# rogerbarton/optix-renderer

Hardware: AMD Instinct MI355X
Metric: Msamples/sec (whole node) + traversal HBM GB/s, cbox 1024x1024 256spp (higher is better)
Workload: dtype f32; 1 GPU; Cornell box (diffuse-only) 1024x1024, 16400 spp, path_mis; config=c2, width=1024, height=1024, spp=16400, mode=wavefront, traversal=ordered, pools=2, gpu_max_hw_queues=8, parallelism=single GPU

## Files before the change

### include/nori_hip.h

```cpp
#ifndef NORI_HIP_H
#define NORI_HIP_H

#include <stddef.h>
#include <stdint.h>

#ifdef __cplusplus
extern "C" {
#endif

#define NH_OK 0
#define NH_ERR_INVALID 1
#define NH_ERR_IO 2
#define NH_ERR_DEVICE 3
#define NH_ERR_UNSUPPORTED 4
#define NH_ERR_STATE 5


enum { NH_SHAPE_MESH = 0, NH_SHAPE_SPHERE = 1 };
enum { NH_BSDF_DIFFUSE = 0, NH_BSDF_MIRROR = 1, NH_BSDF_DIELECTRIC = 2, NH_BSDF_MICROFACET = 3, NH_BSDF_DISNEY = 4 };
enum { NH_EMITTER_AREA = 0, NH_EMITTER_POINT = 1, NH_EMITTER_ENVMAP = 2, NH_EMITTER_SPOT = 3,
       NH_EMITTER_DIRECTIONAL = 4 };
enum { NH_INTEGRATOR_PATH_MIS = 0, NH_INTEGRATOR_PATH_MATS = 1, NH_INTEGRATOR_DIRECT_EMS = 2,
       NH_INTEGRATOR_DIRECT_MATS = 3, NH_INTEGRATOR_DIRECT_MIS = 4, NH_INTEGRATOR_DIRECT = 5,
       NH_INTEGRATOR_NORMALS = 6,
// ... 103 lines not shown
typedef struct nh_envmap {
    int32_t width, height;
    const float *rgba;
    float radiance[3];
    float scale_u, scale_v;
    float offset_u, offset_v;
    int32_t spherical;
    int32_t constant;
    const float *cdf;
    float normalization;
    float rotation[9];
} nh_envmap;

enum { NH_DENOISER_NONE = 0, NH_DENOISER_SIMPLE = 1 };
typedef struct nh_denoiser {
    int32_t type;
    float sigma_d;
    float sigma_vr;
    int32_t range;
    int32_t amount;
} nh_denoiser;

enum { NH_SAMPLER_INDEPENDENT = 0, NH_SAMPLER_ADAPTIVE = 1 };

typedef struct nh_scene_desc {
    nh_camera camera;
    nh_filter filter;
    int32_t integrator;
    int32_t sample_count;
    uint32_t n_shapes;
    const nh_shape *shapes;
    uint32_t n_bsdfs;
    const nh_bsdf *bsdfs;
    uint32_t n_emitters;
    const nh_emitter *emitters;
    const float *emitter_cdf;
    int32_t envmap;
    uint32_t n_vertices;
    const float *V;
    const float *N;
    const float *UV;
    const float *T;
    const float *BT;
    uint32_t n_faces;
    const uint32_t *F;
    uint32_t n_area_cdf;
    const float *area_cdf;
    nh_envmap env;
    nh_denoiser denoiser;
    uint32_t n_textures;
    const nh_texture *textures;
    uint64_t n_texels;
    const float *texels;
    float normals_direction[3];
    const nh_emitter_ext *emitter_ext;
    uint32_t n_media;
    const nh_medium *media;
    const uint32_t *shape_medium;
    uint32_t ambient_medium;
    int32_t sampler;
    int32_t adaptive_initial_uniform;
} nh_scene_desc;


typedef struct nh_bvh_node {
    uint32_t word0;
    uint32_t word1;
    float bbox_min[3];
    float bbox_max[3];
} nh_bvh_node;

typedef struct nh_bvh_desc {
    uint32_t n_nodes;
    const nh_bvh_node *nodes;
    uint32_t n_indices;
    const uint32_t *indices;
    uint32_t n_shapes;
    const uint32_t *shape_offset;
    float bbox_min[3], bbox_max[3];
    uint32_t max_depth;
} nh_bvh_desc;


typedef struct nh_ray_soa {
    const float *ox, *oy, *oz;
    const float *dx, *dy, *dz;
    const float *mint, *maxt;
} nh_ray_soa;

typedef struct nh_hit_soa {
    uint8_t *hit;
    float *t, *u, *v;
    uint32_t *prim;
    uint32_t *shape;
} nh_hit_soa;


enum { NH_MODE_MEGAKERNEL = 0, NH_MODE_WAVEFRONT = 1 };
enum { NH_TRAVERSAL_REFERENCE = 0, NH_TRAVERSAL_ORDERED = 1, NH_TRAVERSAL_WIDE = 2 };

typedef struct nh_render_req {
    int32_t sample_begin;
    int32_t sample_end;
    uint64_t seed;
    int32_t n_blocks;
    const int32_t *blocks;
    int32_t mode;
    int32_t traversal;
    int32_t clear;
    int32_t collect_stats;
} nh_render_req;

#define NH_SMALL_TABLES_BYTES 4096

typedef struct nh_render_stats {
    double kernel_ms_path;
    double kernel_ms_splat;
    double kernel_ms_extend;
    double kernel_ms_shadow;
    double kernel_ms_shade;
    uint64_t launches_path, launches_splat, launches_extend, launches_shadow, launches_shade;
    uint64_t samples;
    uint64_t ray_queries;
    uint64_t nodes_visited;
    uint64_t boxes_tested;
    uint64_t prims_tested;
    uint64_t invalid_samples;
    uint64_t shadow_queries, shadow_nodes_visited, shadow_boxes_tested, shadow_prims_tested;
    uint64_t shade_state_bytes, extend_queue_bytes, shadow_queue_bytes, paths_shaded;
    double kernel_ms_tail;
    uint64_t launches_tail;
    uint64_t node_bytes;
    uint64_t tail_queries, tail_nodes_visited, tail_boxes_tested, tail_prims_tested;
    uint64_t tail_shadow_queries, tail_shadow_nodes_visited, tail_shadow_boxes_tested, tail_shadow_prims_tested;
    uint64_t lds_scene;
    uint64_t fused_bounce;
    uint64_t comm_inits;
    double kernel_ms_denoise;
    uint64_t launches_denoise;
    uint64_t tails_async;
    uint64_t pools_active;
    uint64_t trace_fused;
    uint64_t tail_cycles_body, tail_cycles_shadow, tail_cycles_closest, tail_cycles_head;
    uint64_t tail_bounces, tail_max_bounces;
    uint64_t tail_coop_cycles_body, tail_coop_cycles_shadow, tail_coop_cycles_closest, tail_coop_cycles_head;
    uint64_t tail_coop_bounces;
    uint64_t bounce_cycles_load, bounce_cycles_body, bounce_cycles_shadow, bounce_cycles_closest, bounce_cycles_head;
    uint64_t bounce_cycles_store, bounce_bounces;
    uint64_t bounce_traits;
    uint64_t primary_masks;
    uint64_t pair_kinds;
    uint64_t flat_trace;
    uint64_t shadow_masks;
} nh_render_stats;

typedef struct nh_scene nh_scene;
typedef struct nh_bvh nh_bvh;
typedef struct nh_ctx nh_ctx;

int nh_scene_load_xml(const char *path, nh_scene **out);
int nh_scene_load_xml_index(const char *path, int32_t index, nh_scene **out);
int nh_scene_get_desc(const nh_scene *scene, nh_scene_desc *out);
int nh_scene_set_resolution(nh_scene *scene, int32_t width, int32_t height);
int nh_scene_set_sample_count(nh_scene *scene, int32_t spp);
int nh_scene_set_sampler(nh_scene *scene, int32_t type, int32_t initial_uniform);
int nh_scene_set_bsdf(nh_scene *scene, uint32_t shape, const nh_bsdf *bsdf);
uint32_t nh_scene_add_texture(nh_scene *scene, const nh_texture *tex, const float *texels);
int nh_scene_set_normal_map(nh_scene *scene, uint32_t shape, uint32_t texture);
int nh_scene_set_lens_draw_order(nh_scene *scene, int32_t order);
int nh_texture_decode(const uint8_t *rgba8, uint64_t n, int32_t srgb, float *out);
int nh_scene_set_integrator(nh_scene *scene, int32_t integrator);
typedef struct nh_photon_params {
    int32_t photon_count;
    float photon_radius;
} nh_photon_params;
int nh_scene_get_photon_params(const nh_scene *scene, nh_photon_params *out);
int nh_scene_set_photon_params(nh_scene *scene, const nh_photon_params *params);
typedef struct nh_av_params {
    float length;
} nh_av_params;
int nh_scene_get_av_params(const nh_scene *scene, nh_av_params *out);
int nh_scene_set_av_params(nh_scene *scene, const nh_av_params *params);
int nh_photon_tables(float *cos_theta, float *sin_theta, float *cos_phi, float *sin_phi, float *exp_table);
void nh_scene_free(nh_scene *scene);
const char *nh_host_last_error(void);
int nh_debug_transform(const char *request, float *out, int32_t cap);

int nh_bvh_build(const nh_scene_desc *scene, int32_t n_threads, nh_bvh **out);
int nh_bvh_get_desc(const nh_bvh *bvh, nh_bvh_desc *out);
void nh_bvh_free(nh_bvh *bvh);

int nh_primary_masks(const nh_camera *camera, const float *records, int32_t n_records, const int32_t *blocks,
                     int32_t n_blocks, uint64_t *masks, int32_t *built);
int32_t nh_primary_mask_pad(int32_t width, int32_t height);

int nh_shadow_emitter_faces(const nh_scene_desc *scene, float *faces, int32_t cap_faces, int32_t *n_faces);
int nh_shadow_masks(const nh_camera *camera, const float *records, int32_t n_records, const float *emit_faces,
                    int32_t n_emit_faces, const int32_t *blocks, int32_t n_blocks, uint64_t *emitter_mask,
                    uint64_t *masks, int32_t *built);

int nh_pair_layout(const float *records, int32_t n_records, const int32_t *leaves, int32_t n_leaves, int32_t by_kind,
                   int32_t *slots, int32_t *leaf_pairs);

int nh_flat_image(const float *records, int32_t n_records, const int32_t *leaves, int32_t n_leaves, const float *boxes,
                  int32_t allowed, float *image, int32_t image_cap_f4, int32_t *n_f4, int32_t *box_equal);

int nh_framebuffer_to_rgb(const float *rgbw, int32_t width, int32_t height, int32_t border, float *rgb);
int nh_write_pfm(const char *path, const float *rgb, int32_t width, int32_t height);
int nh_image_load_png(const char *path, uint8_t *rgba, size_t cap, int32_t *width, int32_t *height);
int nh_write_exr(const char *path, const float *rgb, int32_t width, int32_t height);
int nh_rgb_to_ldr(const float *rgb, int32_t width, int32_t height, uint8_t *rgb8);
int nh_write_png(const char *path, const float *rgb, int32_t width, int32_t height);

int nh_get_device_count(int *n);
int nh_create(int device, nh_ctx **out);
void nh_destroy(nh_ctx *ctx);
int nh_upload_scene(nh_ctx *ctx, const nh_scene_desc *scene);
int nh_upload_bvh(nh_ctx *ctx, const nh_bvh_desc *bvh);
int nh_trace_rays(nh_ctx *ctx, const nh_ray_soa *rays, int32_t n, int32_t any_hit, int32_t traversal, nh_hit_soa *out);
#define NH_ADAPTIVE_MAX_SAMPLES 133948
#define NH_ADAPTIVE_STAGING_BYTES ((size_t)4 << 30)
int nh_render(nh_ctx *ctx, const nh_render_req *req);
typedef struct nh_adaptive_stats {
    uint64_t total_samples;
    uint64_t passes;
    uint64_t max_passes;
    uint64_t n_blocks;
} nh_adaptive_stats;
int nh_get_adaptive_stats(nh_ctx *ctx, nh_adaptive_stats *out);
int nh_get_adaptive_variance(nh_ctx *ctx, float *out, size_t n_floats);
int nh_synchronize(nh_ctx *ctx);
int nh_get_framebuffer(nh_ctx *ctx, float *rgbw, size_t n_floats);
int nh_framebuffer_device_ptr(nh_ctx *ctx, void **dptr, size_t *n_floats);
int nh_get_stats(nh_ctx *ctx, nh_render_stats *out);
int nh_reset_stats(nh_ctx *ctx);
int nh_reduce_framebuffers(nh_ctx **ctxs, int32_t n, int32_t root);
int nh_denoise(nh_ctx *ctx, const nh_denoiser *params);
int nh_denoise_image(nh_ctx *ctx, float *rgbw, int32_t width, int32_t height, int32_t border,
                     const nh_denoiser *params);
enum { NH_BSDF_QUERY_EVAL = 0, NH_BSDF_QUERY_SAMPLE = 1 };
int nh_bsdf_query(nh_ctx *ctx, const nh_bsdf *bsdf, const float *albedo, int32_t mode, int32_t n, const float *wi,
                  const float *wo, const float *sample, float *wo_out, float *value, float *pdf, int32_t *measure);
enum { NH_EMITTER_QUERY_SAMPLE = 0, NH_EMITTER_QUERY_EVAL = 1, NH_EMITTER_QUERY_PDF = 2,
       NH_EMITTER_QUERY_SAMPLE_PHOTON = 3 };
#define NH_EMITTER_QUERY_SAMPLE_STRIDE 16
#define NH_EMITTER_QUERY_PHOTON_STRIDE 12
#define NH_EMITTER_QUERY_IN_STRIDE 9
int nh_emitter_query(nh_ctx *ctx, uint32_t emitter, int32_t mode, int32_t n, const float *ref, const float *sample,
                     float *out);
enum { NH_MEDIUM_QUERY_FREE_PATH = 0, NH_MEDIUM_QUERY_TRANSMITTANCE = 1, NH_MEDIUM_QUERY_PHASE_SAMPLE = 2,
       NH_MEDIUM_QUERY_PHASE_PDF = 3 };
int nh_medium_query(nh_ctx *ctx, uint32_t medium, int32_t mode, int32_t n, const float *in, float *out);


enum { NH_TEST_TTEST = 0, NH_TEST_CHI2TEST = 1 };
typedef struct nh_test_desc {
    int32_t type;
    float significance_level;
    int32_t sample_count;
    uint32_t n_angles;
    const float *angles;
    uint32_t n_references;
    const float *references;
    uint32_t n_scenes;
    uint32_t n_bsdfs;
    const nh_bsdf *bsdfs;
} nh_test_desc;
typedef struct nh_test nh_test;
int nh_test_load_xml(const char *path, nh_test **out);
int nh_test_get_desc(const nh_test *test, nh_test_desc *out);
void nh_test_free(nh_test *test);

int nh_students_t_test(double mean, double variance, double reference, int32_t n, double alpha, int32_t num_tests,
                       int32_t *accepted, double *p_value);

#define NH_RADIANCE_QUERY_MAX (1 << 24)
int nh_radiance_query(nh_ctx *ctx, uint64_t seed, int32_t n, const int32_t *pixel, const int32_t *sample,
                      const float *pixel_sample, float *rgb, float *jitter);
int nh_ttest_scene(nh_ctx *ctx, uint64_t seed, int64_t first, int32_t n, double *mean, double *variance,
                   float *luminance);
int nh_ttest_bsdf(nh_ctx *ctx, const nh_bsdf *bsdf, const float *albedo, float angle_deg, uint64_t first_draw,
                  int32_t n, double *mean, double *variance, float *luminance);
typedef struct nh_test_result {
    double mean, variance, reference, p_value;
    int32_t accepted;
    int32_t sample_count;
    float angle;
    int32_t pad;
} nh_test_result;
int nh_test_run(int device, const char *path, uint64_t seed, nh_test_result *results, int32_t cap,
                int32_t *n_results);


#define NH_PHOTON_STREAM ((uint64_t)1 << 32)
#define NH_PHOTON_DEFAULT_BATCH (1 << 18)
int nh_photon_map_build(nh_ctx *ctx, const nh_photon_params *params, uint64_t seed, int32_t batch_paths);
typedef struct nh_photon_stats {
    int32_t stored;
    int32_t emitted;
    float radius;
    float cell_size;
    uint64_t occupied_cells;
} nh_photon_stats;
int nh_get_photon_stats(nh_ctx *ctx, nh_photon_stats *out);
int nh_get_photons(nh_ctx *ctx, int32_t first, int32_t n, float *position, float *direction, float *power,
                   uint8_t *bytes, int32_t *path, int32_t *bounce);
enum { NH_PHOTON_QUERY_CODEC = 0, NH_PHOTON_QUERY_GATHER = 1 };
int nh_photon_query(nh_ctx *ctx, int32_t mode, int32_t n, const float *in, uint8_t *bytes, int32_t *count, float *out);


int nh_set_av_params(nh_ctx *ctx, const nh_av_params *params);

const char *nh_last_error(const nh_ctx *ctx);

#ifdef __cplusplus
}
#endif
#endif
```

### optix-renderer_amd/csrc/nh_ctx.h

```cpp
#pragma once
#include <hip/hip_runtime.h>
#include <rccl/rccl.h>

#include <algorithm>
#include <cstdint>
#include <deque>
#include <memory>
#include <string>
#include <vector>

#include "nh_internal.h"
#include "nori_hip.h"

constexpr int kRing = 4;
constexpr int kPools = 4;
constexpr int kTails = 3;
constexpr int kTailCap = 65536;
#ifndef NH_DEFAULT_POOLS
#define NH_DEFAULT_POOLS 2
#endif

struct WfJob {
    uint64_t seq;
    int s0, rounds;
    uint64_t seed;
    bool ordered, stats;
    bool staged;
    bool jit;
};

struct WfPool {
    hipStream_t stream = nullptr;
    WfState wf{};
    std::vector<void *> bufs;
    size_t cap = 0;
    float *rec = nullptr;
    size_t rec_cap = 0;
    float2 *jit = nullptr;
    size_t jit_cap = 0;
    float4 *staging = nullptr;
    size_t staging_cap = 0;
    uint32_t *spill = nullptr;
    int spill_words = 0;
    unsigned *h_counts = nullptr;
    hipEvent_t copy_ev[kRing] = {};
    std::vector<hipEvent_t> events;
    hipEvent_t ev_begin = nullptr, ev_path = nullptr, ev_splat0 = nullptr, ev_splat = nullptr;
    hipEvent_t ev_handoff = nullptr;
    enum State { IDLE, ENQUEUE, COUNTS, SPLAT, FINISH } state = IDLE;
    WfJob job{};
    WfLaunch L{};
    bool persistent = false, wide = false, trace2 = false, tail = false, draining = false;
    bool fused = false, sorted = false;
    bool rr = false;
    bool trait = false;
    bool shade_sorted = false;
    int64_t tail_at = 0, drain_at = 0;
    int it = 0;
    std::vector<uint64_t> in_e, in_s;
};

struct CommSet {
    std::vector<uint64_t> ids;
    std::vector<int> devices;
    std::vector<ncclComm_t> comms;
    ~CommSet() {
        int cur = 0;
        const bool have = hipGetDevice(&cur) == hipSuccess;
        for (size_t i = 0; i < comms.size(); ++i) {
            (void)hipSetDevice(devices[i]);
            (void)ncclCommDestroy(comms[i]);
        }
        if (have) (void)hipSetDevice(cur);
    }
};

struct DeviceGuard {
    int dev = 0;
    bool ok = false;
    DeviceGuard() { ok = hipGetDevice(&dev) == hipSuccess; }
    ~DeviceGuard() {
        if (ok) (void)hipSetDevice(dev);
    }
};

struct PixelList {
    int *pixel_list = nullptr, *pixel_map = nullptr;
    int *block_ids = nullptr, *block_slot = nullptr;
    int *color_slots = nullptr;
    int n_blocks = 0, n_color0 = 0, n_list = 0;
    std::vector<int32_t> list_key;
    bool have_list = false;
    void release() {
        for (int *p : {pixel_list, pixel_map, block_ids, block_slot, color_slots}) (void)hipFree(p);
        *this = PixelList{};
    }
};

struct AdaptiveState {
    int n_blocks = 0, nbx = 0, nby = 0;
    int next_sample = -1;
    int4 *blocks = nullptr;
    int *block_rank = nullptr, *active_list = nullptr, *next = nullptr;
    AdBlock *state = nullptr;
    unsigned *counts = nullptr, *h_count = nullptr;
    int2 *pos = nullptr;
    float4 *rad = nullptr, *staging = nullptr;
    float2 *jit = nullptr;
    size_t slot_cap = 0;
    unsigned long long *stats = nullptr;
    std::vector<int4> h_blocks;
};

struct PhotonState {
    bool built = false;
    std::vector<void *> bufs;
    const float *tables = nullptr;
    std::vector<float> h_tables;
    float *pos = nullptr;
    uint2 *bytes = nullptr;
    uint32_t *path = nullptr;
    int *bounce = nullptr;
    nh_photon_stats stats{};
};

struct nh_ctx {
    uint64_t id = 0;
    std::shared_ptr<CommSet> comms;
    int device = 0;
    hipStream_t stream = nullptr;
    std::string err;
    std::vector<nh_shape> shapes;
    std::vector<float> V;
    std::vector<uint32_t> F;
    int width = 0, height = 0, border = 0, n_emitters = 0, integrator = 0;
    nh_filter filter{};
    nhd::DScene S{};
    nhd::DScene *d_scene = nullptr;
    nhd::Traversal tv{};
    std::vector<void *> scene_bufs, bvh_bufs;
    bool has_scene = false, has_bvh = false;
    int depth = 0;
    int depth_wide = 0;
    int wide_w = 4;
    int n_node_f4 = 0, n_leaves = 0, n_prim_f4 = 0;
    std::vector<uint32_t> bvh_indices, shape_offset;
    std::vector<int> shape_bsdf_type;
    std::vector<int> shape_bsdf_real;
    int n_bsdf_types = 0;
    bool disney = false;
    bool specular = false;
    bool textured = false;
    bool normal_mapped = false;
    bool diffuse_area = false;
    bool bsdfless = false, has_media = false;
    int sampler = 0, adaptive_initial_uniform = 0;
    AdaptiveState ad;
    PhotonState photon;
    bool av_set = false;
    AvLaunch av{};
    std::vector<void *> av_bufs;
    size_t av_cap = 0;
    int2 *av_spill = nullptr;
    int av_spill_depth = 0;
    std::vector<nhd::DShape> h_shapes;
    std::vector<nhd::DBsdf> h_bsdfs;
    std::vector<nhd::DEmitter> h_emitters;
    std::vector<float> h_area_cdf;
    int n_emit_faces = 0;
    float4 *small_image = nullptr;
    int small_tab[5] = {0, 0, 0, 0, 0};
    bool pair_kinds = false;
    float4 *small_image_ref = nullptr;
    const float4 *flat_image = nullptr;
    nh_camera camera{};
    std::vector<float> h_prims;
    unsigned long long *pmask = nullptr;
    bool pmask_known = false;
    std::vector<float> h_emit_tris;
    unsigned long long *smask = nullptr;
    float *fb = nullptr;
    size_t fb_floats = 0;
    float *rec = nullptr;
    size_t rec_cap = 0;
    int *block_rank = nullptr;
    int nbx = 0, nby = 0;
    PixelList px;
    float4 *staging = nullptr;
    size_t staging_cap = 0;
    unsigned long long *counters = nullptr;
    nh_render_stats stats{};
    WfPool pools[kPools + kTails];
    std::deque<WfJob> jobs;
    uint64_t job_seq = 0, splat_seq = 0;
    hipEvent_t fb_ev = nullptr;
    bool fb_ev_set = false;
    uint64_t stats_comm_inits = 0;
};

inline void drop_primary_masks(nh_ctx *c) {
    (void)hipFree(c->pmask);
    (void)hipFree(c->smask);
    c->pmask = nullptr;
    c->smask = nullptr;
    c->pmask_known = false;
}

#define NH_LAUNCH(c, fn) ((c)->disney ? nh_disney::nh::fn : nh::fn)

void pool_free(WfPool &p);
int pipeline_drain(nh_ctx *c);
int check_device(nh_ctx *c, const char *where);
int render_adaptive(nh_ctx *c, const nh_render_req *q);
void adaptive_release(nh_ctx *c);
void photon_release(nh_ctx *c, bool tables = false);
nhd::DDisney disney_record(const nh_bsdf &b);
void disney_set_record(nhd::DBsdf &o, const nhd::DDisney *rec);
int disney_upload(nh_ctx *c, std::vector<void *> &owner, const std::vector<nhd::DDisney> &recs,
                  const std::vector<float> &albedo, nhd::DDisney **out);

int query_bsdf_record(nh_ctx *c, std::vector<void *> &owner, const nh_bsdf *b, const float *albedo, nhd::DBsdf &o,
                      float alb[3]);

inline bool fail(nh_ctx *c, const std::string &m) {
    if (c) c->err = m;
    return false;
}

#define HIP_TRY(ctx, expr)                                                                               \
    do {                                                                                                 \
        hipError_t e_ = (expr);                                                                          \
        if (e_ != hipSuccess) {                                                                          \
            (ctx)->err = std::string(#expr) + ": " + hipGetErrorString(e_);                              \
            return NH_ERR_DEVICE;                                                                        \
        }                                                                                                \
    } while (0)

template <typename T>
int upload(nh_ctx *c, std::vector<void *> &owner, const T *src, size_t n, const T **dst) {
    void *p = nullptr;
    size_t bytes = (std::max<size_t>(n * sizeof(T), 16) + 15) / 16 * 16;
    HIP_TRY(c, hipMalloc(&p, bytes));
    owner.push_back(p);
    if (n) HIP_TRY(c, hipMemcpyAsync(p, src, n * sizeof(T), hipMemcpyHostToDevice, c->stream));
    *dst = reinterpret_cast<const T *>(p);
    return NH_OK;
}

inline void free_all(std::vector<void *> &v) {
    for (void *p : v) (void)hipFree(p);
    v.clear();
}
```

### optix-renderer_amd/csrc/nh_layout.h

```cpp
#pragma once

namespace nhd {

constexpr int kLensLo = 256, kLensHi = 65536;

constexpr int kPrimSphere = 1, kPrimLeafEnd = 2, kPrimMatShift = 2;
constexpr int kPrimIsolated = 16;

constexpr int kWideF4 = 8;
constexpr int kWideEmpty = (int)0x80000000;

constexpr int kPairF4 = 6;
constexpr int kFlatHeaderF4 = 6, kFlatMaxPairs = 16;
constexpr int kFlatLeftEq = 1, kFlatRightEq = 2;

constexpr int kMaxStack = 128;

}
```

### optix-renderer_amd/csrc/nh_pipeline.hip

```cpp
#include <cmath>
#include <cstdlib>
#include <cstring>
#include <thread>
#include <type_traits>

#include "../host/gpu_layout.h"
#include "nh_ctx.h"


constexpr size_t kWfBytesPerPath = 2 * (16 * 6 + 8 + 1) + 36;

static int pool_alloc(nh_ctx *c, WfPool &p, size_t n, size_t rec_n, size_t staging_f4, bool jit = false) {
    if (!p.stream) {
        if (!p.h_counts && hipHostMalloc(reinterpret_cast<void **>(&p.h_counts),
                                         (kRing * 2 * kCountGroup + kCountSlot) * sizeof(unsigned)) != hipSuccess) {
            p.h_counts = nullptr;
            return fail(c, "hipHostMalloc failed"), NH_ERR_DEVICE;
        }
        for (hipEvent_t &e : p.copy_ev)
            if (!e) HIP_TRY(c, hipEventCreateWithFlags(&e, hipEventDisableTiming));
        for (hipEvent_t *e : {&p.ev_begin, &p.ev_path, &p.ev_splat0, &p.ev_splat})
            if (!*e) HIP_TRY(c, hipEventCreate(e));
        if (!p.ev_handoff) HIP_TRY(c, hipEventCreateWithFlags(&p.ev_handoff, hipEventDisableTiming));
        HIP_TRY(c, hipStreamCreateWithFlags(&p.stream, hipStreamNonBlocking));
// ... 49 lines not shown

void pool_free(WfPool &p) {
    free_all(p.bufs);
    (void)hipFree(p.rec);
    (void)hipFree(p.jit);
    (void)hipFree(p.staging);
    (void)hipFree(p.spill);
    if (p.h_counts) (void)hipHostFree(p.h_counts);
    for (hipEvent_t e : p.events) (void)hipEventDestroy(e);
    for (hipEvent_t e : p.copy_ev)
        if (e) (void)hipEventDestroy(e);
    for (hipEvent_t e : {p.ev_begin, p.ev_path, p.ev_splat0, p.ev_splat, p.ev_handoff})
        if (e) (void)hipEventDestroy(e);
    if (p.stream) (void)hipStreamDestroy(p.stream);
    p = WfPool{};
}

static SplatLaunch make_splat(const nh_ctx *c, const float *rec, uint64_t seed, int s0, float4 *staging, int rounds,
                              bool staged) {
    SplatLaunch P{};
    P.staged = staged ? 1 : 0;
    P.fb = c->fb;
    P.width = c->width;
    P.height = c->height;
    P.border = c->border;
    P.reach = (int)std::floor(c->filter.radius + 0.5f);
    P.nbx = c->nbx;
    P.n_rounds = rounds;
    P.n_list = c->px.n_list;
    P.pixel_map = c->px.pixel_map;
    P.block_rank = c->block_rank;
    P.rec = rec;
    P.seed = seed;
    P.s0 = s0;
    P.radius = c->filter.radius;
    P.lookup = c->filter.lookup_factor;
    std::memcpy(P.table, c->filter.table, sizeof(P.table));
    P.blocks = c->px.block_ids;
    P.block_slot = c->px.block_slot;
    P.n_blocks = c->px.n_blocks;
    P.color_slots = c->px.color_slots;
    P.n_color0 = c->px.n_color0;
    P.staging = staging;
    return P;
}

static bool splat_staged(const nh_ctx *c) {
    return nh::splat_uses_staging(c->border, (int)std::floor(c->filter.radius + 0.5f));
}
static size_t block_px(const nh_ctx *c, bool staged) {
    if (!staged) return 0;
    return (size_t)(32 + 2 * c->border) * (size_t)stage_pitch(32 + 2 * c->border);
}

static int active_pools(const nh_ctx *c) {
    const char *np = std::getenv("NH_POOLS");
    const int def = c->specular ? NH_DEFAULT_POOLS + 1 : NH_DEFAULT_POOLS;
    return std::max(1, std::min(kPools, np ? std::atoi(np) : def));
}

static bool tail_async_enabled() {
    const char *e = std::getenv("NH_TAIL_ASYNC");
    return e && e[0] == '1';
}

static int pool_start(nh_ctx *c, WfPool &p, const WfJob &job) {
    WfJob j = job;
    j.staged = splat_staged(c);
    const char *jv = std::getenv("NH_SPLAT_JITTER");
    j.jit = jv && std::strcmp(jv, "stored") == 0;
    const int n_paths = j.rounds * c->px.n_list;
    const size_t staging_f4 = (size_t)j.rounds * c->px.n_blocks * block_px(c, j.staged);
    int rc = pool_alloc(c, p, (size_t)n_paths, (size_t)n_paths, staging_f4, j.jit);
    if (rc) return rc;
    for (int i = 0; i < active_pools(c); ++i) {
        WfPool &o = c->pools[i];
        if (&o == &p || o.state != WfPool::IDLE) continue;
        if ((rc = pool_alloc(c, o, (size_t)n_paths, (size_t)n_paths, staging_f4, j.jit))) return rc;
    }
    if (active_pools(c) > 1 && tail_async_enabled())
        for (int i = kPools; i < kPools + kTails; ++i) {
            WfPool &o = c->pools[i];
            if (o.state != WfPool::IDLE) continue;
            if ((rc = pool_alloc(c, o, (size_t)kTailCap, (size_t)n_paths, staging_f4, j.jit))) return rc;
        }
    p.job = j;
    WfLaunch &L = p.L;
    L = WfLaunch{};
    L.st = p.wf;
    L.n_paths = n_paths;
    L.n_list = c->px.n_list;
    L.s0 = j.s0;
    L.seed = j.seed;
    L.pixel_list = c->px.pixel_list;
    L.rec = p.rec;
    L.jit = j.jit ? p.jit : nullptr;
    L.counters = c->counters;
    const size_t scene_bytes = 16 * (size_t)(c->n_node_f4 + c->n_prim_f4) + 8 * (size_t)c->n_leaves;
    bool small = scene_bytes <= kSmallSceneBytes;
    if (const char *e = std::getenv("NH_LDS_SCENE")) small = small && e[0] != '0';
    if (small) {
        L.small_nodes = c->n_node_f4;
        L.small_leaves = c->n_leaves;
        L.small_prims = c->n_prim_f4;
        L.small_frames = c->n_prim_f4 / 3 <= kSmallFramesMaxPrims;
        if (const char *e = std::getenv("NH_LDS_FRAMES")) L.small_frames = L.small_frames && e[0] != '0';
        L.small_image = j.stats && c->small_image_ref ? c->small_image_ref : c->small_image;
        for (int i = 0; i < 5; ++i) L.small_tab[i] = c->small_tab[i];
    }
    const int per_chunk = 256;
    const int max_chunks = (n_paths + per_chunk - 1) / per_chunk;
    L.seg_cap = (max_chunks + kQueueShards - 1) / kQueueShards * per_chunk;
    p.persistent = c->depth > 20;
    if (const char *e = std::getenv("NH_PERSISTENT")) p.persistent = e[0] == '1';
    p.wide = p.persistent && j.ordered && c->tv.wnodes != nullptr;
    if (const char *e = std::getenv("NH_WIDE")) p.wide = p.wide && e[0] != '0';
    if (p.wide && !j.ordered) return fail(c, "wavefront pool: the wide traversal needs an ordered job"), NH_ERR_STATE;
    p.trace2 = p.wide && scene_bytes <= (size_t)256 << 20;
    if (const char *e = std::getenv("NH_TRACE2")) p.trace2 = p.wide && e[0] != '0';
    c->stats.trace_fused = p.trace2 ? 1 : 0;
    const int spill_words = p.wide ? 2 * c->depth_wide : (c->depth + 1) / 2 * 2;
    if (p.persistent && p.spill_words < spill_words) {
        HIP_TRY(c, hipStreamSynchronize(p.stream));
        (void)hipFree(p.spill);
        p.spill = nullptr;
        p.spill_words = 0;
        HIP_TRY(c, hipMalloc(&p.spill, (size_t)kPersistentBlocks * 128 * spill_words * sizeof(uint32_t)));
        p.spill_words = spill_words;
    }
    p.fused = small && !p.persistent && c->depth <= 16;
    if (const char *e = std::getenv("NH_FUSED")) p.fused = p.fused && e[0] != '0';
    p.sorted = p.fused && c->n_bsdf_types > 1;
    p.rr = p.fused;
    if (const char *e = std::getenv("NH_RR_AHEAD")) p.rr = p.fused && e[0] != '0';
    p.shade_sorted = false;
    if (const char *e = std::getenv("NH_SORT_SHADE")) p.shade_sorted = !p.fused && e[0] == '1';
    if (const char *e = std::getenv("NH_SORT")) p.sorted = p.fused && e[0] == '1';
    p.trait = p.rr && c->diffuse_area && c->small_tab[0] > 0 && j.ordered && !p.sorted;
    if (const char *e = std::getenv("NH_BOUNCE_TRAITS")) p.trait = p.trait && e[0] != '0';
    c->stats.bounce_traits = p.rr ? (p.trait ? 2 : 1) : 0;
    const char *pm = std::getenv("NH_PRIMARY_MASKS");
    const bool masks = p.rr && c->pmask && !j.stats && !(pm && pm[0] == '0');
    L.pmask = masks ? c->pmask : nullptr;
    L.pmask_nbx = c->nbx;
    c->stats.primary_masks = masks ? 1 : 0;
    const char *sm = std::getenv("NH_SHADOW_MASKS");
    const bool shadow = p.rr && c->smask && !j.stats && !(sm && (sm[0] == '0' || sm[0] == '1'));
    L.smask = shadow ? c->smask : nullptr;
    c->stats.shadow_masks = shadow ? 2 : 0;
    c->stats.pair_kinds = p.fused && c->pair_kinds && !j.stats ? 1 : 0;
    const bool flat = p.rr && c->flat_image && c->pair_kinds && !j.stats && !c->disney;
    L.flat = flat ? c->flat_image : nullptr;
    c->stats.flat_trace = flat ? 1 : 0;
    c->stats.fused_bounce = p.fused ? 1 : 0;
    c->stats.node_bytes = p.wide ? 16 * nhd::kWideF4 * (c->wide_w / 4) : 64;
    c->stats.lds_scene = small && !p.persistent && c->depth <= 16 ? 1 : 0;
    L.trav_spill = p.spill;
    L.spill_depth = p.spill_words;
    p.tail_at = p.fused ? std::min<int64_t>(std::max<int64_t>(n_paths / 1024, 8192), 16384)
                        : std::min<int64_t>(std::max<int64_t>(n_paths / 64, 8192), 262144);
    if (const char *e = std::getenv("NH_TAIL")) p.tail_at = std::atoll(e);
    p.drain_at = std::max<int64_t>(n_paths / 8, p.tail_at);
    HIP_TRY(c, hipEventRecord(p.ev_begin, p.stream));
    unsigned *h_init = p.h_counts + kRing * 2 * kCountGroup;
    std::memset(h_init, 0, kCountSlot * sizeof(unsigned));
    h_init[0] = (unsigned)n_paths;
    HIP_TRY(c, hipMemcpyAsync(p.wf.counts, h_init, kCountSlot * sizeof(unsigned), hipMemcpyHostToDevice, p.stream));
    p.in_e.assign(1, (uint64_t)n_paths);
    p.in_s.assign(1, 0);
    p.it = 0;
    p.tail = false;
    p.draining = false;
    p.state = WfPool::ENQUEUE;
    return NH_OK;
}

static void chunk_swap(WfPool &a, WfPool &b) {
    std::swap(a.h_counts, b.h_counts);
    std::swap(a.copy_ev, b.copy_ev);
    std::swap(a.events, b.events);
    std::swap(a.ev_begin, b.ev_begin);
    std::swap(a.ev_path, b.ev_path);
    std::swap(a.ev_splat0, b.ev_splat0);
    std::swap(a.ev_splat, b.ev_splat);
    std::swap(a.job, b.job);
    std::swap(a.L, b.L);
    std::swap(a.persistent, b.persistent);
    std::swap(a.wide, b.wide);
    std::swap(a.trace2, b.trace2);
    std::swap(a.tail, b.tail);
    std::swap(a.draining, b.draining);
    std::swap(a.fused, b.fused);
    std::swap(a.sorted, b.sorted);
    std::swap(a.rr, b.rr);
    std::swap(a.trait, b.trait);
    std::swap(a.shade_sorted, b.shade_sorted);
    std::swap(a.tail_at, b.tail_at);
    std::swap(a.drain_at, b.drain_at);
    std::swap(a.it, b.it);
    std::swap(a.in_e, b.in_e);
    std::swap(a.in_s, b.in_s);
    std::swap(a.rec, b.rec);
    std::swap(a.rec_cap, b.rec_cap);
    std::swap(a.jit, b.jit);
    std::swap(a.jit_cap, b.jit_cap);
    std::swap(a.staging, b.staging);
    std::swap(a.staging_cap, b.staging_cap);
}

static WfPool *free_tail_slot(nh_ctx *c, const WfPool &p, int bound) {
    if (!p.rr || bound > kTailCap || active_pools(c) < 2) return nullptr;
    if (!tail_async_enabled()) return nullptr;
    for (int i = kPools; i < kPools + kTails; ++i)
        if (c->pools[i].state == WfPool::IDLE) return &c->pools[i];
    return nullptr;
}

static int pool_handoff(nh_ctx *c, WfPool &p, WfPool &T, int bound, hipEvent_t *ev) {
    int rc = pool_alloc(c, T, (size_t)kTailCap, 0, 0);
    if (rc) return rc;
    HIP_TRY(c, hipMemsetAsync(T.wf.counts, 0, kCountSlot * sizeof(unsigned), p.stream));
    nh::launch_wf_pack_rr(p.L, T.wf.buf[0], T.wf.counts, bound, p.stream);
    HIP_TRY(c, hipGetLastError());
    HIP_TRY(c, hipEventRecord(p.ev_handoff, p.stream));
    chunk_swap(p, T);
    WfLaunch &L = T.L;
    L.st = T.wf;
    L.in_q = 0;
    L.cnt_in = T.wf.counts;
    HIP_TRY(c, hipStreamWaitEvent(T.stream, p.ev_handoff, 0));
    HIP_TRY(c, hipEventRecord(ev[1], T.stream));
    HIP_TRY(c, hipEventRecord(ev[2], T.stream));
    NH_LAUNCH(c, launch_wf_tail_rr)(c->d_scene, c->tv, L, T.job.ordered, T.job.stats, bound, c->specular,
                          !c->specular && !c->textured, c->normal_mapped, T.trait, T.stream);
    HIP_TRY(c, hipGetLastError());
    HIP_TRY(c, hipEventRecord(ev[3], T.stream));
    T.tail = true;
    T.draining = true;
    T.state = WfPool::SPLAT;
    p.state = WfPool::IDLE;
    c->stats.tails_async++;
    return NH_OK;
}

static bool count_kernel() {
    static const bool on = [] {
        const char *e = std::getenv("NH_COUNT_KERNEL");
        return !(e && e[0] == '0');
    }();
    return on;
}

static int count_service(nh_ctx *c, WfPool &p, unsigned *out, unsigned *in_slot, int it) {
    unsigned *h = p.h_counts + (size_t)(it % kRing) * 2 * kCountGroup;
    if (count_kernel()) {
        nh::launch_wf_counts(out, h, 2 * kCountGroup, in_slot, kCountSlot, p.stream);
        HIP_TRY(c, hipGetLastError());
    } else {
        HIP_TRY(c, hipMemcpyAsync(h, out, 2 * kCountGroup * sizeof(unsigned), hipMemcpyDeviceToHost, p.stream));
    }
    HIP_TRY(c, hipEventRecord(p.copy_ev[it % kRing], p.stream));
    return NH_OK;
}

static int pool_enqueue(nh_ctx *c, WfPool &p) {
    WfLaunch &L = p.L;
    const int it = p.it, in = it & 1;
    unsigned *slot[2] = {p.wf.counts, p.wf.counts + kCountSlot};
    L.in_q = in;
    L.first = it == 0;
    L.cam_rays = it == 0 && p.persistent && c->S.dof ? 1 : 0;
    L.cnt_in = slot[in];
    L.cnt_out = slot[in ^ 1];
    while ((size_t)(it + 1) * 4 > p.events.size()) {
        hipEvent_t e;
        HIP_TRY(c, hipEventCreate(&e));
        p.events.push_back(e);
    }
    hipEvent_t *ev = &p.events[(size_t)it * 4];
    const int bound = (int)p.in_e[it == 0 ? 0 : it - 1];
    const bool ordered = p.job.ordered, stats = p.job.stats;
    if (it == 0 || !count_kernel()) HIP_TRY(c, hipMemsetAsync(slot[in ^ 1], 0, kCountSlot * sizeof(unsigned), p.stream));
    HIP_TRY(c, hipEventRecord(ev[0], p.stream));
    if (p.fused) {
        if (it > 0 && (int64_t)bound <= p.tail_at)
            if (WfPool *T = free_tail_slot(c, p, bound)) return pool_handoff(c, p, *T, bound, ev);
        HIP_TRY(c, hipEventRecord(ev[1], p.stream));
        HIP_TRY(c, hipEventRecord(ev[2], p.stream));
        if (it > 0 && (int64_t)bound <= p.tail_at) {
            if (p.rr)
                NH_LAUNCH(c, launch_wf_tail_rr)(c->d_scene, c->tv, L, ordered, stats, bound, c->specular,
                                                !c->specular && !c->textured, c->normal_mapped, p.trait, p.stream);
            else NH_LAUNCH(c, launch_wf_tail)(c->d_scene, c->tv, L, ordered, stats, false, bound, c->depth, p.stream);
            HIP_TRY(c, hipGetLastError());
            HIP_TRY(c, hipEventRecord(ev[3], p.stream));
            p.tail = true;
            p.draining = true;
            p.state = WfPool::SPLAT;
            return NH_OK;
        }
        if (p.rr) NH_LAUNCH(c, launch_wf_bounce_rr)(c->d_scene, c->tv, L, ordered, stats, p.sorted,
                                                    !c->specular && !c->textured, c->normal_mapped, p.trait, bound,
                                                    p.stream);
        else NH_LAUNCH(c, launch_wf_bounce)(c->d_scene, c->tv, L, ordered, stats, p.sorted, bound, p.stream);
        HIP_TRY(c, hipGetLastError());
        HIP_TRY(c, hipEventRecord(ev[3], p.stream));
// ... 309 lines not shown
    if (blocks.empty())
        for (int i = 0; i < c->nbx * c->nby; ++i) blocks.push_back(i);
    std::vector<uint64_t> m;
    if (!nh::primary_masks(c->camera, reinterpret_cast<const nh::f4 *>(c->h_prims.data()), (int)(c->h_prims.size() / 12),
                           blocks.data(), (int)blocks.size(), m))
        return NH_OK;
    std::vector<unsigned long long> grid((size_t)c->nbx * c->nby, 0ull);
    for (size_t i = 0; i < blocks.size(); ++i) grid[(size_t)blocks[i]] = m[i];
    unsigned long long *d = nullptr;
    HIP_TRY(c, hipMalloc(&d, std::max<size_t>(grid.size(), 1) * sizeof(unsigned long long)));
    const hipError_t e = hipMemcpy(d, grid.data(), grid.size() * sizeof(unsigned long long), hipMemcpyHostToDevice);
    if (e != hipSuccess) {
        (void)hipFree(d);
        HIP_TRY(c, e);
    }
    c->pmask = d;
    const int n_faces = (int)(c->h_emit_tris.size() / 9);
    const nh::f4 *recs = reinterpret_cast<const nh::f4 *>(c->h_prims.data());
    const int n_recs = (int)(c->h_prims.size() / 12);
    if (n_faces == 0 ||
        !nh::shadow_block_masks(c->camera, recs, n_recs, c->h_emit_tris.data(), n_faces, blocks.data(), (int)blocks.size(), m))
        return NH_OK;
    for (size_t i = 0; i < blocks.size(); ++i) grid[(size_t)blocks[i]] = m[i];
    HIP_TRY(c, hipMalloc(&d, std::max<size_t>(grid.size(), 1) * sizeof(unsigned long long)));
    const hipError_t e2 = hipMemcpy(d, grid.data(), grid.size() * sizeof(unsigned long long), hipMemcpyHostToDevice);
    if (e2 != hipSuccess) {
        (void)hipFree(d);
        HIP_TRY(c, e2);
    }
    c->smask = d;
    return NH_OK;
}

constexpr size_t kAvBytesPerPath = 94;

static bool av_wide(const nh_ctx *c, const nh_render_req *q) {
    return q->traversal != NH_TRAVERSAL_REFERENCE && c->depth > 20 && c->tv.wnodes != nullptr;
}
static size_t av_bytes_per_path(const nh_ctx *c, const nh_render_req *q) {
    return kAvBytesPerPath + (av_wide(c, q) ? (size_t)c->depth_wide * sizeof(int2) : 0);
}

static int av_reserve(nh_ctx *c, size_t paths, bool wide) {
    const int spill_depth = wide ? c->depth_wide : 0;
    if (c->av_cap >= paths && c->av_spill_depth >= spill_depth) return NH_OK;
    free_all(c->av_bufs);
    c->av_cap = 0;
    c->av_spill_depth = 0;
    c->av_spill = nullptr;
    AvLaunch &L = c->av;
    L = AvLaunch{};
    const auto get = [&](auto **p, size_t n) -> int {
        void *d = nullptr;
        HIP_TRY(c, hipMalloc(&d, std::max<size_t>(n, 1) * sizeof(**p)));
        c->av_bufs.push_back(d);
        *p = static_cast<std::remove_reference_t<decltype(*p)>>(d);
        return NH_OK;
    };
    int rc = NH_OK;
    for (int i = 0; i < 8 && !rc; ++i)
        if (!(rc = get(&L.ray[i], paths))) rc = get(&L.q_ray[i], paths);
    if (rc || (rc = get(&L.hit.hit, paths)) || (rc = get(&L.hit.t, paths)) || (rc = get(&L.hit.u, paths)) ||
        (rc = get(&L.hit.v, paths)) || (rc = get(&L.hit.k, paths)) || (rc = get(&L.rng, paths)) ||
        (rc = get(&L.q_path, paths)) || (rc = get(&L.q_hit, paths)) || (rc = get(&L.q_count, 1)) ||
        (spill_depth && (rc = get(&c->av_spill, paths * (size_t)spill_depth)))) {
        free_all(c->av_bufs);
        return rc;
    }
    c->av_cap = paths;
    c->av_spill_depth = spill_depth;
    return NH_OK;
}

static int av_chunk(nh_ctx *c, const nh_render_req *q, const PathLaunch &P) {
    AvLaunch L = c->av;
    L.n_paths = P.n_paths;
    L.n_list = P.n_list;
    L.s0 = P.s0;
    L.seed = P.seed;
    L.pixel_list = P.pixel_list;
    L.rec = P.rec;
    const bool wide = av_wide(c, q), ordered = q->traversal != NH_TRAVERSAL_REFERENCE, stats = q->collect_stats != 0;
    const auto batch = [&](float *const r[8], const HitBatch &hb, int n, bool any) {
        const RayBatch rb{r[0], r[1], r[2], r[3], r[4], r[5], r[6], r[7]};
        unsigned long long *ctr = c->counters + (any ? kStatAny : 0);
        if (wide) nh::launch_trace_wide(c->d_scene, c->tv, rb, hb, n, any, true, stats, c->av_spill, c->av_spill_depth, ctr,
                                        c->stream, c->wide_w);
        else nh::launch_trace(c->d_scene, c->tv, rb, hb, n, any, ordered, stats, c->depth, ctr, c->stream);
    };
    HIP_TRY(c, hipMemsetAsync(L.q_count, 0, sizeof(unsigned), c->stream));
    nh::launch_av_primary(c->d_scene, L, c->stream);
    batch(L.ray, L.hit, L.n_paths, false);
    nh::launch_av_shade(c->d_scene, c->tv, L, c->stream);
    HIP_TRY(c, hipGetLastError());
    int n_queue = L.n_paths;
    if (stats) {
        unsigned n = 0;
        HIP_TRY(c, hipMemcpyAsync(&n, L.q_count, sizeof(n), hipMemcpyDeviceToHost, c->stream));
        HIP_TRY(c, hipStreamSynchronize(c->stream));
        n_queue = (int)n;
    }
    HitBatch occl{};
    occl.hit = L.q_hit;
    batch(L.q_ray, occl, n_queue, true);
    nh::launch_av_resolve(L, n_queue, c->stream);
    return NH_OK;
}

extern "C" {

int nh_render(nh_ctx *c, const nh_render_req *q) {
    if (!c || !q) return NH_ERR_INVALID;
    if (!c->has_scene || !c->has_bvh) return fail(c, "nh_render: scene and BVH must be uploaded"), NH_ERR_STATE;
    if (q->sample_end < q->sample_begin || q->sample_begin < 0) return fail(c, "invalid sample range"), NH_ERR_INVALID;
    if (c->S.dof && q->sample_end > nhd::kLensLo * nhd::kLensHi)
        return fail(c, "depth of field: sample rounds beyond 2^24"), NH_ERR_UNSUPPORTED;
    if ((c->integrator == NH_INTEGRATOR_PATH_MIS || c->integrator == NH_INTEGRATOR_DIRECT_MIS) && c->n_emitters == 0)
        return fail(c, "No Emitter in scene!"), NH_ERR_INVALID;
    if (q->mode != NH_MODE_MEGAKERNEL && q->mode != NH_MODE_WAVEFRONT) return fail(c, "unknown render mode"), NH_ERR_INVALID;
    const bool volumetric = c->integrator == NH_INTEGRATOR_PATH_VOL_MATS || c->integrator == NH_INTEGRATOR_PATH_VOL_MIS;
    if (!volumetric && (c->bsdfless || c->has_media))
        return fail(c, "the scene has a participating medium or a shape without a BSDF: only the path_vol_mats and "
                       "path_vol_mis integrators render it"), NH_ERR_UNSUPPORTED;
    if (c->integrator == NH_INTEGRATOR_PATH_VOL_MIS && c->n_emitters == 0)
        return fail(c, "No Emitter in scene!"), NH_ERR_INVALID;
    const bool photon = c->integrator == NH_INTEGRATOR_PHOTONMAPPER;
    if (photon && !c->photon.built)
        return fail(c, "nh_render: the photon mapper needs a photon map (nh_photon_map_build)"), NH_ERR_STATE;
    if (photon && c->sampler == NH_SAMPLER_ADAPTIVE)
        return fail(c, "photonmapper: the adaptive sampler is not supported"), NH_ERR_UNSUPPORTED;
    if (c->integrator == NH_INTEGRATOR_AV && !c->av_set)
        return fail(c, "nh_render: the av integrator needs its length (nh_set_av_params)"), NH_ERR_STATE;
    if (c->integrator == NH_INTEGRATOR_ENVMAPTESTER && c->S.envmap < 0)
        return fail(c, "This integrator requires an env map."), NH_ERR_INVALID;
    const bool av_split = q->mode == NH_MODE_WAVEFRONT && c->integrator == NH_INTEGRATOR_AV;
    const bool wavefront = q->mode == NH_MODE_WAVEFRONT && c->integrator <= NH_INTEGRATOR_PATH_MATS;
    if (q->traversal < NH_TRAVERSAL_REFERENCE || q->traversal > NH_TRAVERSAL_WIDE)
        return fail(c, "unknown traversal"), NH_ERR_INVALID;
    if (c->border > 4) return fail(c, "reconstruction filters wider than border 4 are not supported"), NH_ERR_UNSUPPORTED;
    HIP_TRY(c, hipSetDevice(c->device));
    int rc = NH_OK;
    if (!wavefront || q->collect_stats || q->clear || c->sampler == NH_SAMPLER_ADAPTIVE) rc = pipeline_drain(c);
    if (rc) return rc;
    if (c->sampler == NH_SAMPLER_ADAPTIVE) return render_adaptive(c, q);
    rc = ensure_pixel_list(c, q);
    if (rc) return rc;
    if (wavefront && (rc = ensure_primary_masks(c))) return rc;
    c->stats.node_bytes = 64;
    if (av_split && av_wide(c, q)) c->stats.node_bytes = 16 * nhd::kWideF4 * (c->wide_w / 4);
    c->stats.primary_masks = 0;
    c->stats.shadow_masks = 0;
    c->stats.pair_kinds = 0;
    c->stats.flat_trace = 0;
    c->stats.trace_fused = 0;
    c->stats.lds_scene = 0;
    c->stats.fused_bounce = 0;
    if (q->clear) {
        HIP_TRY(c, hipMemsetAsync(c->fb, 0, c->fb_floats * sizeof(float), c->stream));
        HIP_TRY(c, hipEventRecord(c->fb_ev, c->stream));
        c->fb_ev_set = true;
    }
    const int rounds = q->sample_end - q->sample_begin;
    if (rounds == 0 || c->px.n_list == 0) return NH_OK;
    if (q->collect_stats)
        HIP_TRY(c, hipMemsetAsync(c->counters, 0, kStatShards * kStatStride * sizeof(unsigned long long), c->stream));
    const size_t per_round = (size_t)c->px.n_list;
    const char *jv = std::getenv("NH_SPLAT_JITTER");
    const size_t rec_bytes = kRecFloats * 4 + (wavefront && jv && std::strcmp(jv, "stored") == 0 ? 8 : 0);
    const size_t per_round_bytes = per_round * rec_bytes + (size_t)c->px.n_blocks * block_px(c, splat_staged(c)) * 16 +
                                   (wavefront ? per_round * kWfBytesPerPath : 0) +
                                   (av_split ? per_round * av_bytes_per_path(c, q) : 0);
    size_t budget = wavefront ? (size_t)24 << 30 : (size_t)1 << 30;
    if (const char *e = std::getenv(wavefront ? "NH_WF_BUDGET_MB" : "NH_RECORD_BUDGET_MB"))
        budget = (size_t)std::max(1L, std::atol(e)) << 20;
    if (wavefront) {
        size_t free_b = 0, total_b = 0;
        if (hipMemGetInfo(&free_b, &total_b) == hipSuccess) {
            size_t held = 0;
            for (const WfPool &p : c->pools)
                held += p.cap * kWfBytesPerPath + p.rec_cap * kRecFloats * 4 + p.jit_cap * 8 + p.staging_cap * sizeof(float4);
            const int shares = active_pools(c) + (active_pools(c) > 1 && tail_async_enabled() ? kTails : 0);
            const size_t avail = (size_t)((double)(free_b + held) * 0.85) / (size_t)shares;
            budget = std::min(budget, std::max(avail, per_round_bytes));
        }
    }
    int chunk = (int)std::max<size_t>(1, std::min<size_t>((size_t)rounds, budget / per_round_bytes));
    while ((size_t)chunk * per_round > (size_t)0x7fffffff) chunk = std::max(1, chunk / 2);
    if (wavefront) {
        if (per_round > ((size_t)1 << 26))
            return fail(c, "wavefront mode renders at most 2^26 pixels per context"), NH_ERR_UNSUPPORTED;
        chunk = std::min(chunk, (int)(((size_t)1 << 26) / per_round));
    }

    if (wavefront) {
        HIP_TRY(c, hipStreamSynchronize(c->stream));
        for (int s = q->sample_begin; s < q->sample_end; s += chunk)
            c->jobs.push_back(WfJob{c->job_seq++, s, std::min(chunk, q->sample_end - s), q->seed,
                                    q->traversal != NH_TRAVERSAL_REFERENCE, q->collect_stats != 0});
        rc = q->collect_stats ? pipeline_drain(c) : pipeline_run(c, false);
        if (rc) return rc;
        if (int e = check_device(c, "nh_render")) return e;
    } else {
        if (c->rec_cap < (size_t)chunk * per_round) {
            (void)hipFree(c->rec);
            c->rec = nullptr;
            c->rec_cap = 0;
            const size_t cap = (size_t)chunk * per_round;
            HIP_TRY(c, hipMalloc(&c->rec, cap * kRecFloats * sizeof(float)));
            c->rec_cap = cap;
        }
        if (av_split && (rc = av_reserve(c, (size_t)chunk * per_round, av_wide(c, q)))) return rc;
        const bool staged = splat_staged(c);
        if (c->staging_cap < (size_t)chunk * c->px.n_blocks * block_px(c, staged)) {
            (void)hipFree(c->staging);
            c->staging = nullptr;
            c->staging_cap = 0;
            const size_t cap = (size_t)chunk * c->px.n_blocks * block_px(c, staged);
            HIP_TRY(c, hipMalloc(&c->staging, cap * sizeof(float4)));
            c->staging_cap = cap;
        }
        struct Ev {
            hipEvent_t a, b, d;
        };
        std::vector<Ev> evs;
        for (int s = q->sample_begin; s < q->sample_end; s += chunk) {
            const int k = std::min(chunk, q->sample_end - s);
            PathLaunch L{};
            L.n_paths = k * c->px.n_list;
            L.n_list = c->px.n_list;
            L.s0 = s;
            L.seed = q->seed;
            L.pixel_list = c->px.pixel_list;
            L.rec = c->rec;
            L.counters = c->counters;
            Ev ev;
            HIP_TRY(c, hipEventCreate(&ev.a));
            HIP_TRY(c, hipEventCreate(&ev.b));
            HIP_TRY(c, hipEventCreate(&ev.d));
            HIP_TRY(c, hipEventRecord(ev.a, c->stream));
            if (av_split) {
                if ((rc = av_chunk(c, q, L))) return rc;
            } else if (photon)
                nh_disney::nh::launch_photon_path(c->d_scene, c->tv, L, q->collect_stats != 0, c->depth, c->stream);
            else if (volumetric)
                nh_disney::nh::launch_vol_path(c->d_scene, c->tv, L, c->integrator == NH_INTEGRATOR_PATH_VOL_MIS,
                                               q->collect_stats != 0, c->depth, c->stream);
            else
                NH_LAUNCH(c, launch_path)(c->d_scene, c->tv, L, q->traversal != NH_TRAVERSAL_REFERENCE, q->collect_stats != 0,
                            c->depth, c->integrator == NH_INTEGRATOR_PATH_MIS && !c->normal_mapped, c->stream);
            HIP_TRY(c, hipGetLastError());
            HIP_TRY(c, hipEventRecord(ev.b, c->stream));
            if (q->collect_stats) nh::launch_count_invalid(c->rec, (size_t)L.n_paths, c->counters, c->stream);
            nh::launch_splat(make_splat(c, c->rec, q->seed, s, c->staging, k, staged), c->stream);
            HIP_TRY(c, hipGetLastError());
            HIP_TRY(c, hipEventRecord(ev.d, c->stream));
            evs.push_back(ev);
        }
        HIP_TRY(c, hipStreamSynchronize(c->stream));
        for (auto &ev : evs) {
            float a = 0, b = 0;
            (void)hipEventElapsedTime(&a, ev.a, ev.b);
            (void)hipEventElapsedTime(&b, ev.b, ev.d);
            c->stats.kernel_ms_path += a;
            c->stats.kernel_ms_splat += b;
            c->stats.launches_path++;
            c->stats.launches_splat++;
            (void)hipEventDestroy(ev.a);
            (void)hipEventDestroy(ev.b);
            (void)hipEventDestroy(ev.d);
        }
        c->stats.samples += (uint64_t)rounds * (uint64_t)c->px.n_list;
    }
    if (q->collect_stats) {
        unsigned long long hs[kStatShards * kStatStride], h[kStatStride] = {};
        HIP_TRY(c, hipMemcpy(hs, c->counters, sizeof(hs), hipMemcpyDeviceToHost));
        for (int sh = 0; sh < kStatShards; ++sh)
            for (int j = 0; j < kStatStride; ++j) h[j] += hs[sh * kStatStride + j];
        h[kStatTailClk + 5] = 0;
        for (int sh = 0; sh < kStatShards; ++sh)
            h[kStatTailClk + 5] = std::max(h[kStatTailClk + 5], hs[sh * kStatStride + kStatTailClk + 5]);
        c->stats.tail_cycles_body += h[kStatTailClk];
        c->stats.tail_cycles_shadow += h[kStatTailClk + 1];
        c->stats.tail_cycles_closest += h[kStatTailClk + 2];
        c->stats.tail_cycles_head += h[kStatTailClk + 3];
        c->stats.tail_bounces += h[kStatTailClk + 4];
        c->stats.tail_max_bounces = std::max<uint64_t>(c->stats.tail_max_bounces, h[kStatTailClk + 5]);
        c->stats.tail_coop_cycles_body += h[kStatTailCoopClk];
        c->stats.tail_coop_cycles_shadow += h[kStatTailCoopClk + 1];
        c->stats.tail_coop_cycles_closest += h[kStatTailCoopClk + 2];
        c->stats.tail_coop_cycles_head += h[kStatTailCoopClk + 3];
        c->stats.tail_coop_bounces += h[kStatTailCoopClk + 4];
        c->stats.bounce_cycles_load += h[kStatBounceClk];
        c->stats.bounce_cycles_body += h[kStatBounceClk + 1];
        c->stats.bounce_cycles_shadow += h[kStatBounceClk + 2];
        c->stats.bounce_cycles_closest += h[kStatBounceClk + 3];
        c->stats.bounce_cycles_head += h[kStatBounceClk + 4];
        c->stats.bounce_cycles_store += h[kStatBounceClk + 5];
        c->stats.bounce_bounces += h[kStatBounceClk + 6];
        const unsigned long long *cl = h, *an = h + kStatAny, *tc = h + kStatTail, *ta = h + kStatTailAny;
        c->stats.ray_queries += cl[0] + an[0] + tc[0] + ta[0];
        c->stats.nodes_visited += cl[1] + an[1] + tc[1] + ta[1];
        c->stats.boxes_tested += cl[2] + an[2] + tc[2] + ta[2];
        c->stats.prims_tested += cl[3] + an[3] + tc[3] + ta[3];
        c->stats.invalid_samples += h[4];
        c->stats.shadow_queries += an[0] + ta[0];
        c->stats.shadow_nodes_visited += an[1] + ta[1];
// ... 16 lines not shown
```

### optix-renderer_amd/csrc/nh_traverse.h

```cpp
#pragma once
#include "nh_device.h"
#include "nh_flat_combine.h"

namespace nhd {

struct Hit {
    float t, u, v;
    int k;
};

struct TravStats {
    uint32_t nodes, boxes, prims;
};

NHD bool box_test(float mnx, float mny, float mnz, float mxx, float mxy, float mxz, F3 o, F3 d, F3 r, float mint,
                  float maxt, float &near_out) {
    float near_t = -INFINITY, far_t = INFINITY;
    if (d.x == 0) {
        if (o.x < mnx || o.x > mxx) return false;
    } else {
        float t1 = (mnx - o.x) * r.x, t2 = (mxx - o.x) * r.x;
        if (t1 > t2) { float tmp = t1; t1 = t2; t2 = tmp; }
        near_t = e_max(t1, near_t);
        far_t = e_min(t2, far_t);
// ... 411 lines not shown
}

NHD void node_box_tests(const float *nf, F3 o, F3 d, F3 r, float mint, float maxt, bool fin, bool &hl, bool &hr,
                        float &nl, float &nr) {
    const float l0 = nf[0], l1 = nf[1], l2 = nf[2], l3 = nf[3], l4 = nf[4], l5 = nf[5];
    const float r0 = nf[6], r1 = nf[7], r2 = nf[8], r3 = nf[9], r4 = nf[10], r5 = nf[11];
    if (fin) {
        box_test_finite_pair(f2{l0, r0}, f2{l1, r1}, f2{l2, r2}, f2{l3, r3}, f2{l4, r4}, f2{l5, r5}, o.x, o.y, o.z, r.x,
                             r.y, r.z, mint, maxt, hl, hr, nl, nr);
    } else {
        hl = box_test(l0, l1, l2, l3, l4, l5, o, d, r, mint, maxt, nl);
        hr = box_test(r0, r1, r2, r3, r4, r5, o, d, r, mint, maxt, nr);
    }
}

template <int DEPTH, bool ORDERED, bool ANY, bool STATS, bool PAIRS = false, int G = 1, bool RCP = false,
          bool MASKED = false>
NHD bool trace(const Traversal &tv, const DScene &S, F3 o, F3 d, float mint, float maxt, Hit &best, uint32_t *stk,
               int stride, TravStats &st, unsigned long long cand = ~0ull) {
    if (mint == kEps) mint = e_max(mint, mint * e_max(fabsf(o.x), e_max(fabsf(o.y), fabsf(o.z))));
    const bool lead = G == 1 || (threadIdx.x & (G - 1)) == 0;
    best.k = -1;
    best.t = INFINITY;
    if (S.root_kind == 0 || maxt < mint) return false;
    const F3 r = RCP ? f3(dir_rcp(d.x), dir_rcp(d.y), dir_rcp(d.z)) : f3(1.0f / d.x, 1.0f / d.y, 1.0f / d.z);
    const bool fin = isfinite(r.x) & isfinite(r.y) & isfinite(r.z);
    bool found = false;
    float near_t;
    if (STATS && lead) st.boxes++;
    if (fin ? !box_test_finite(S.root_min[0], S.root_min[1], S.root_min[2], S.root_max[0], S.root_max[1],
                               S.root_max[2], o, r, mint, maxt, near_t)
            : !box_test(S.root_min[0], S.root_min[1], S.root_min[2], S.root_max[0], S.root_max[1], S.root_max[2], o,
                        d, r, mint, maxt, near_t))
        return false;
    if (S.root_kind == 2) {
        bool any = leaf_any<ANY, STATS, PAIRS, G, MASKED>(tv, 0, o, d, mint, maxt, best, found, st, cand);
        return ANY ? any : found;
    }
    int sp = 0;
    int cur = 0;
    for (;;) {
        while (cur >= 0) {
            const float *nf = node_f(tv, cur);
            const int ref_l = node_ref(nf, 0), ref_r = node_ref(nf, 1);
            if (STATS && lead) { st.nodes++; st.boxes += 2; }
            float nl, nr;
            bool hl, hr;
            node_box_tests(nf, o, d, r, mint, maxt, fin, hl, hr, nl, nr);
            int next;
            if (hl && hr) {
                const bool right_first = ORDERED && nr < nl;
                stk[sp * stride] = ((uint32_t)cur << 1) | (right_first ? 0u : 1u);
                ++sp;
                next = right_first ? ref_r : ref_l;
            } else if (hl) {
                next = ref_l;
            } else if (hr) {
                next = ref_r;
            } else {
                break;
            }
            if (next >= 0) {
                cur = next;
                continue;
            }
            if (leaf_any<ANY, STATS, PAIRS, G, MASKED>(tv, ~next, o, d, mint, maxt, best, found, st, cand)) return true;
            break;
        }
        cur = -1;
        while (sp > 0) {
            --sp;
            const uint32_t e = stk[sp * stride];
            const int parent = (int)(e >> 1), side = (int)(e & 1u);
            const float *nf = node_f(tv, parent);
            if (STATS && lead) st.boxes++;
            if (!child_box_test(nf, side, o, d, r, mint, maxt, near_t, fin)) continue;
            const int ref = node_ref(nf, side);
            if (ref >= 0) {
                cur = ref;
                break;
            }
            if (leaf_any<ANY, STATS, PAIRS, G, MASKED>(tv, ~ref, o, d, mint, maxt, best, found, st, cand)) return true;
        }
        if (cur < 0) break;
    }
    (void)DEPTH;
    return ANY ? false : found;
}

template <bool ANY, bool MASKED>
NHD bool flat_leaf(const float4 *__restrict__ pp, int n_tri, int n_sph, F3 o, F3 d, float mint, float maxt, Hit &best,
                   bool &found, unsigned long long cand) {
    bool any = false;
    for (int i = 0; i < n_tri; ++i, pp += kPairF4) {
        const float4 q5 = pp[5];
        const int k0 = __float_as_int(q5.z), k1 = __float_as_int(q5.w);
        if constexpr (MASKED)
            if (!(((cand >> (k0 & 63)) | (cand >> (k1 & 63))) & 1ull)) continue;
        const float4 q0 = pp[0], q1 = pp[1], q2 = pp[2], q3 = pp[3], q4 = pp[4];
        const P3 p0{f2{q0.x, q0.y}, f2{q0.z, q0.w}, f2{q1.x, q1.y}};
        const P3 e1{f2{q2.x, q2.y}, f2{q2.z, q2.w}, f2{q3.x, q3.y}};
        const P3 e2{f2{q3.z, q3.w}, f2{q4.x, q4.y}, f2{q4.z, q4.w}};
        f2 pt, pu, pv;
        bool ok0, ok1;
        tri_test_pair_e(p0, e1, e2, o, d, mint, pt, pu, pv, ok0, ok1);
        if (ANY) {
            any = any || (ok0 && pt.x <= maxt) || (ok1 && pt.y <= maxt);
            continue;
        }
        accept_hit(ok0 && pt.x <= maxt, pt.x, pu.x, pv.x, k0, maxt, best, found);
        accept_hit(ok1 && pt.y <= maxt, pt.y, pu.y, pv.y, k1, maxt, best, found);
    }
    for (int i = 0; i < n_sph; ++i, pp += kPairF4) {
        const float4 q5 = pp[5];
        const int k0 = __float_as_int(q5.z), k1 = __float_as_int(q5.w);
        if constexpr (MASKED)
            if (!(((cand >> (k0 & 63)) | (cand >> (k1 & 63))) & 1ull)) continue;
        const float4 q0 = pp[0], q1 = pp[1];
        f2 tmin, tmax;
        bool ok0, ok1;
        sphere_test_pair(f2{q0.x, q0.y}, f2{q0.z, q0.w}, f2{q1.x, q1.y}, f2{q1.z, q1.w}, o, d, tmin, tmax, ok0, ok1);
        if (!(ok0 | ok1)) continue;
        float t0, t1;
        const bool h0 = sphere_in_range(tmin.x, tmax.x, mint, maxt, t0) && ok0;
        if (ANY) {
            any = any || h0 || (sphere_in_range(tmin.y, tmax.y, mint, maxt, t1) && ok1);
            continue;
        }
        accept_hit(h0, t0, 0.f, 0.f, k0, maxt, best, found);
        const bool h1 = sphere_in_range(tmin.y, tmax.y, mint, maxt, t1) && ok1;
        accept_hit(h1, t1, 0.f, 0.f, k1, maxt, best, found);
    }
    return any;
}

template <bool ORDERED, bool ANY, bool RCP, bool MASKED = false>
NHD bool trace_flat(const float4 *__restrict__ fl, const DScene &S, F3 o, F3 d, float mint, float maxt, Hit &best,
                    unsigned long long cand = ~0ull) {
    if (mint == kEps) mint = e_max(mint, mint * e_max(fabsf(o.x), e_max(fabsf(o.y), fabsf(o.z))));
    best.k = -1;
    best.t = INFINITY;
    if (S.root_kind == 0 || maxt < mint) return false;
    const F3 r = RCP ? f3(dir_rcp(d.x), dir_rcp(d.y), dir_rcp(d.z)) : f3(1.0f / d.x, 1.0f / d.y, 1.0f / d.z);
    const bool fin = isfinite(r.x) & isfinite(r.y) & isfinite(r.z);
    const float4 h0 = fl[0], h1 = fl[1], h2 = fl[2], h3 = fl[3], h4 = fl[4], h5 = fl[5];
    const auto box = [&](float4 mn, float4 mx, float &near_t) {
        return fin ? box_test_finite(mn.x, mn.y, mn.z, mx.x, mx.y, mx.z, o, r, mint, maxt, near_t)
                   : box_test(mn.x, mn.y, mn.z, mx.x, mx.y, mx.z, o, d, r, mint, maxt, near_t);
    };
    float near_root;
    if (!box(h0, h1, near_root)) return false;
    const int eq = __float_as_int(h0.w);
    const bool two = __float_as_int(h1.w) == 2;
    bool hl = true, hr = false;
    float nl = near_root, nr = near_root;
    if (!(eq & kFlatLeftEq)) hl = box(h2, h3, nl);
    if (two) {
        hr = true;
        if (!(eq & kFlatRightEq)) hr = box(h4, h5, nr);
    }
    const int cl = __float_as_int(h2.w), cr = __float_as_int(h4.w);
    const float4 *pl = fl + kFlatHeaderF4, *pr = pl + kPairF4 * ((cl & 0xffff) + (cl >> 16));
    Hit bl{INFINITY, 0.f, 0.f, -1}, br{INFINITY, 0.f, 0.f, -1};
    bool fl_found = false, fr_found = false, any_l = false, any_r = false;
    if (hl) any_l = flat_leaf<ANY, MASKED>(pl, cl & 0xffff, cl >> 16, o, d, mint, maxt, bl, fl_found, cand);
    if constexpr (ANY) {
        if (hr && !any_l) any_r = flat_leaf<ANY, MASKED>(pr, cr & 0xffff, cr >> 16, o, d, mint, maxt, br, fr_found, cand);
        return flat_combine_any(hl, hr, any_l, any_r);
    } else {
        const bool left_first = hl && !(hr && ORDERED && nr < nl);
        const float maxt_l = fl_found ? bl.t : maxt;
        if (hr && !(left_first && !(nr <= maxt_l)))
            flat_leaf<ANY, MASKED>(pr, cr & 0xffff, cr >> 16, o, d, mint, maxt, br, fr_found, cand);
        FlatBest out;
        flat_combine<ORDERED>(hl, hr, nl, nr, maxt, FlatBest{bl.t, bl.u, bl.v, bl.k, fl_found},
                              FlatBest{br.t, br.u, br.v, br.k, fr_found}, out);
        best.t = out.found ? out.t : INFINITY;
        best.u = out.u;
        best.v = out.v;
        best.k = out.k;
        return out.found;
    }
}

template <bool STATS, int G = 1>
NHD bool iso_sphere_hit(const Traversal &tv, int k_prev, F3 o, F3 d, float mint, float maxt, Hit &best,
                        TravStats &st) {
    if (k_prev < 0) return false;
    const float4 c = tv.prims[3 * k_prev + 2];
    if (!(__float_as_int(c.w) & kPrimIsolated)) return false;
    if (mint == kEps) mint = e_max(mint, mint * e_max(fabsf(o.x), e_max(fabsf(o.y), fabsf(o.z))));
    if (maxt < mint) return false;
    const float4 a = tv.prims[3 * k_prev];
    const float lim = a.w + tv.prims[3 * k_prev + 1].x;
    if (!(fabsf(o.x - a.x) <= lim && fabsf(o.y - a.y) <= lim && fabsf(o.z - a.z) <= lim)) return false;
    float t;
    if (!sphere_test(a, o, d, mint, maxt, t) || !(t >= 2.f * mint)) return false;
    best.t = t;
    best.u = 0.f;
    best.v = 0.f;
    best.k = k_prev;
    if (STATS && (G == 1 || (threadIdx.x & (G - 1)) == 0)) st.prims++;
    return true;
}

template <int DEPTH, bool ORDERED, bool STATS, bool PAIRS = false, int G = 1, bool ISO = true, bool RCP = false>
NHD bool trace_next(const Traversal &tv, const DScene &S, int k_prev, F3 o, F3 d, float mint, float maxt, Hit &best,
                    uint32_t *stk, int stride, TravStats &st) {
#ifndef NH_AB_NO_ISO
    if (ISO && S.iso_spheres && S.root_kind != 0 && iso_sphere_hit<STATS, G>(tv, k_prev, o, d, mint, maxt, best, st))
        return true;
#endif
    return trace<DEPTH, ORDERED, false, STATS, PAIRS, G, RCP>(tv, S, o, d, mint, maxt, best, stk, stride, st);
}
template <bool ORDERED, bool ISO = true, bool RCP = false>
NHD bool trace_next_flat(const float4 *__restrict__ fl, const Traversal &tv, const DScene &S, int k_prev, F3 o, F3 d,
                         float mint, float maxt, Hit &best) {
#ifndef NH_AB_NO_ISO
    TravStats none{0, 0, 0};
    if (ISO && S.iso_spheres && S.root_kind != 0 && iso_sphere_hit<false, 1>(tv, k_prev, o, d, mint, maxt, best, none))
        return true;
#endif
    return trace_flat<ORDERED, false, RCP>(fl, S, o, d, mint, maxt, best);
}



template <int K>
struct RingStack {
    static_assert((K & (K - 1)) == 0, "K must be a power of two");
    uint32_t *lds;
    int stride;
    uint32_t *glob;
    NHD void push(int i, uint32_t e) {
        uint32_t *slot = lds + (i & (K - 1)) * stride;
        if (i >= K) glob[i - K] = *slot;
        *slot = e;
    }
    NHD uint32_t pop(int i) {
        uint32_t *slot = lds + (i & (K - 1)) * stride;
        const uint32_t e = *slot;
        if (i >= K) *slot = glob[i - K];
        return e;
    }
};

template <bool ORDERED, bool ANY, bool STATS, class Stack>
struct Tracer {
    F3 o, d, r;
    float mint, maxt;
    int cur;
    int k, kend;
    int sp;
    bool found, done;
    bool fin;
    Hit best;

    NHD void begin(const DScene &S, const Traversal &tv, F3 o_, F3 d_, float mint_, float maxt_, TravStats &st) {
        o = o_;
        d = d_;
        mint = mint_;
        maxt = maxt_;
        if (mint == kEps) mint = e_max(mint, mint * e_max(fabsf(o.x), e_max(fabsf(o.y), fabsf(o.z))));
        best.k = -1;
        best.t = INFINITY;
        found = false;
        done = true;
        sp = 0;
        cur = -1;
        k = kend = 0;
        if (S.root_kind == 0 || maxt < mint) return;
        r = f3(1.0f / d.x, 1.0f / d.y, 1.0f / d.z);
        fin = isfinite(r.x) & isfinite(r.y) & isfinite(r.z);
        float near_t;
        if (STATS) st.boxes++;
        if (fin ? !box_test_finite(S.root_min[0], S.root_min[1], S.root_min[2], S.root_max[0], S.root_max[1],
                                   S.root_max[2], o, r, mint, maxt, near_t)
                : !box_test(S.root_min[0], S.root_min[1], S.root_min[2], S.root_max[0], S.root_max[1], S.root_max[2],
                            o, d, r, mint, maxt, near_t))
            return;
        done = false;
        if (S.root_kind == 2) {
            const int2 lf = tv.leaves[0];
            k = lf.x;
            kend = lf.x + lf.y;
        } else {
            cur = 0;
        }
    }

    NHD void step(const Traversal &tv, Stack &stk, TravStats &st) {
        if (k < kend) {
            const float4 a = tv.prims[3 * k], b = tv.prims[3 * k + 1], c = tv.prims[3 * k + 2];
            if (STATS) st.prims++;
            float t, u = 0.f, v = 0.f;
            const bool hit = prim_is_tri(c) ? tri_test(a, b, c, o, d, mint, maxt, t, u, v)
                                                        : sphere_test(a, o, d, mint, maxt, t);
            if (hit) {
                if (ANY) {
                    found = true;
                    done = true;
                    return;
                }
                if (t < maxt || k > best.k) {
                    found = true;
                    maxt = t;
                    best.t = t;
                    best.u = u;
                    best.v = v;
                    best.k = k;
                }
            }
            ++k;
            return;
        }
// ... 477 lines not shown
```

### optix-renderer_amd/csrc/nh_upload.hip

```cpp
#include <cmath>
#include <cstdlib>
#include <cstring>

#include "../host/gpu_layout.h"
#include "nh_ctx.h"

using nhd::DBsdf;
using nhd::DEmitter;
using nhd::DShape;

static_assert(sizeof(nh::f4) == sizeof(float4) && alignof(float4) % alignof(nh::f4) == 0, "nh::f4 is float4's layout");
static_assert(sizeof(nh::i2) == sizeof(int2) && alignof(int2) % alignof(nh::i2) == 0, "nh::i2 is int2's layout");
static_assert(sizeof(nh::u64x2) == sizeof(ulonglong2) && alignof(ulonglong2) % alignof(nh::u64x2) == 0,
              "nh::u64x2 is ulonglong2's layout");
static_assert((int)nhd::BSDF_DIELECTRIC == (int)NH_BSDF_DIELECTRIC, "the isolated-sphere marking reads NH_BSDF_*");

nhd::DDisney disney_record(const nh_bsdf &b) {
    nhd::DDisney o;
    std::memset(&o, 0, sizeof(o));
    o.metallic = b.metallic; o.subsurface = b.subsurface; o.specular = b.specular; o.roughness = b.roughness;
    o.specular_tint = b.specular_tint; o.anisotropic = b.anisotropic; o.sheen = b.sheen; o.sheen_tint = b.sheen_tint;
    o.clearcoat = b.clearcoat; o.clearcoat_gloss = b.clearcoat_gloss;
    return o;
}
// ... 213 lines not shown
        const uint4 *tri = nullptr;
        if ((rc = upload(c, c->scene_bufs, ef_tri.data(), ef_tri.size(), &tri))) return rc;
        float4 *faces = nullptr;
        HIP_TRY(c, hipMalloc(&faces, 3 * ef_tri.size() * sizeof(float4)));
        c->scene_bufs.push_back(faces);
        const int n = (int)ef_tri.size();
        hipLaunchKernelGGL(emit_face_kernel, dim3((n + 255) / 256), dim3(256), 0, c->stream, S.V, tri, n, faces);
        HIP_TRY(c, hipGetLastError());
        S.emit_faces = faces;
    }
    if ((rc = upload(c, c->scene_bufs, d->area_cdf, (size_t)d->n_area_cdf, &S.area_cdf))) return rc;
    if (!dt.empty() && (rc = upload(c, c->scene_bufs, dt.data(), dt.size(), &S.texs))) return rc;
    if (d->n_texels) {
        const float *tx = nullptr;
        if ((rc = upload(c, c->scene_bufs, d->texels, 4 * (size_t)d->n_texels, &tx))) return rc;
        S.texels = reinterpret_cast<const float4 *>(tx);
    }
    S.envmap = d->envmap;
    if (d->envmap >= 0) {
        const nh_envmap &e = d->env;
        const size_t texels = (size_t)e.width * (size_t)e.height;
        const float *rgba = nullptr;
        if ((rc = upload(c, c->scene_bufs, e.rgba, 4 * texels, &rgba))) return rc;
        S.env_rgba = reinterpret_cast<const float4 *>(rgba);
        if ((rc = upload(c, c->scene_bufs, e.cdf, texels + 1, &S.env_cdf))) return rc;
        S.env_guide = nullptr;
        S.env_guide_bits = 0;
        bool monotone = true;
        for (size_t i = 0; i <= texels && monotone; ++i)
            monotone = !std::isnan(e.cdf[i]) && (i == 0 || !(e.cdf[i] < e.cdf[i - 1]));
        if (monotone && texels >= 64 && !(std::getenv("NH_ENV_GUIDE") && std::getenv("NH_ENV_GUIDE")[0] == '0')) {
            int bits = 0;
            while (bits < 20 && ((size_t)1 << (bits + 2)) < texels) ++bits;
            const size_t M = (size_t)1 << bits;
            std::vector<int> guide(M + 1);
            size_t i = 0;
            for (size_t j = 0; j <= M; ++j) {
                const float t = (float)((double)j / (double)M);
                while (i <= texels && e.cdf[i] < t) ++i;
                guide[j] = (int)i;
            }
            const int *g = nullptr;
            if ((rc = upload(c, c->scene_bufs, guide.data(), guide.size(), &g))) return rc;
            HIP_TRY(c, hipStreamSynchronize(c->stream));
            S.env_guide = g;
            S.env_guide_bits = bits;
        }
        S.env_w = e.width;
        S.env_h = e.height;
        S.env_spherical = e.spherical;
        std::memcpy(S.env_rot, e.rotation, sizeof(S.env_rot));
        S.env_constant = e.constant;
        S.env_norm = e.normalization;
        S.env_su = e.scale_u;
        S.env_sv = e.scale_v;
        S.env_ou = e.offset_u;
        S.env_ov = e.offset_v;
        S.env_r = e.radiance[0];
        S.env_g = e.radiance[1];
        S.env_b = e.radiance[2];
    }
    S.n_emitters = (int)d->n_emitters;
    S.nee_finite = nh::nee_finite(d) ? 1 : 0;
    if (d->integrator < NH_INTEGRATOR_PATH_MIS || d->integrator > NH_INTEGRATOR_ENVMAPTESTER)
        return fail(c, "unknown integrator"), NH_ERR_INVALID;
    S.integrator = d->integrator;
    S.av_length = 0.f;
    for (int i = 0; i < 3; ++i) S.ndir[i] = d->normals_direction[i];
    std::memcpy(S.s2c, d->camera.sample_to_camera, sizeof(S.s2c));
    std::memcpy(S.c2w, d->camera.camera_to_world, sizeof(S.c2w));
    {
        float ow[4];
        const float z = 0.0f;
        for (int i = 0; i < 4; ++i) {
            float acc = S.c2w[4 * i] * z;
            acc = acc + S.c2w[4 * i + 1] * z;
            acc = acc + S.c2w[4 * i + 2] * z;
            acc = acc + S.c2w[4 * i + 3] * 1.0f;
            ow[i] = acc;
        }
        for (int i = 0; i < 3; ++i) S.cam_o[i] = ow[i] / ow[3];
    }
    S.inv_w = d->camera.inv_output_size[0];
    S.inv_h = d->camera.inv_output_size[1];
    S.near_clip = d->camera.near_clip;
    S.far_clip = d->camera.far_clip;
    S.width = d->camera.width;
    S.height = d->camera.height;
    S.dof = d->camera.lens_radius > 1e-4f ? 1 : 0;
    S.lens_radius = d->camera.lens_radius;
    S.focal_distance = d->camera.focal_distance;
    S.lens_rtl = d->camera.lens_draw_order == NH_LENS_DRAWS_RTL ? 1 : 0;
    S.lens_pix = S.lens_lo = nullptr;
    S.lens_hi = nullptr;
    if (S.dof) {
        const nh::LensTables lt = nh::lens_tables(S.width, S.height);
        const nh::u64x2 *pix = nullptr, *lo = nullptr;
        if ((rc = upload(c, c->scene_bufs, lt.pix.data(), lt.pix.size(), &pix))) return rc;
        if ((rc = upload(c, c->scene_bufs, lt.lo.data(), lt.lo.size(), &lo))) return rc;
        if ((rc = upload(c, c->scene_bufs, lt.hi.data(), lt.hi.size(), &S.lens_hi))) return rc;
        S.lens_pix = reinterpret_cast<const ulonglong2 *>(pix);
        S.lens_lo = reinterpret_cast<const ulonglong2 *>(lo);
        HIP_TRY(c, hipStreamSynchronize(c->stream));
    }
    S.filter_radius = d->filter.radius;
    S.lookup = d->filter.lookup_factor;
    S.border = d->filter.border;
    std::memcpy(S.table, d->filter.table, sizeof(S.table));

    c->shapes.assign(d->shapes, d->shapes + d->n_shapes);
    c->shape_bsdf_type.clear();
    c->shape_bsdf_real.clear();
    unsigned types = 0;
    for (uint32_t i = 0; i < d->n_shapes; ++i) {
        const int t = d->shapes[i].bsdf < 0 ? NH_BSDF_DIFFUSE : d->bsdfs[d->shapes[i].bsdf].type;
        c->shape_bsdf_real.push_back(t);
        types |= 1u << t;
    }
    int disney_key = 0;
    for (int k : {NH_BSDF_MICROFACET, NH_BSDF_MIRROR, NH_BSDF_DIELECTRIC, NH_BSDF_DIFFUSE})
        if (!(types & (1u << k))) {
            disney_key = k;
            break;
        }
    for (int t : c->shape_bsdf_real) c->shape_bsdf_type.push_back(t == NH_BSDF_DISNEY ? disney_key : t);
    c->disney = (types & (1u << NH_BSDF_DISNEY)) != 0;
    c->disney = c->disney || !dx.empty();
    c->n_bsdf_types = __builtin_popcount(types);
    c->specular = (types & ((1u << NH_BSDF_MIRROR) | (1u << NH_BSDF_DIELECTRIC))) != 0;
    c->textured = false;
    for (uint32_t i = 0; i < d->n_bsdfs; ++i) c->textured = c->textured || d->bsdfs[i].albedo_texture != 0;
    c->normal_mapped = false;
    for (uint32_t i = 0; i < d->n_shapes; ++i) c->normal_mapped = c->normal_mapped || d->shapes[i].normal_map != 0;
    c->textured = c->textured || c->normal_mapped;
    c->diffuse_area = S.integrator == NH_INTEGRATOR_PATH_MIS && !c->textured && !S.dof && d->envmap < 0 &&
                      d->n_emitters > 0;
    for (uint32_t i = 0; i < d->n_bsdfs; ++i) c->diffuse_area = c->diffuse_area && d->bsdfs[i].type == NH_BSDF_DIFFUSE;
    for (uint32_t i = 0; i < d->n_emitters; ++i) {
        const nh_emitter &e = d->emitters[i];
        c->diffuse_area = c->diffuse_area && e.type == NH_EMITTER_AREA && e.shape >= 0 &&
                          (uint32_t)e.shape < d->n_shapes && ds[e.shape].ef_off >= 0;
    }
    for (uint32_t i = 0; i < d->n_shapes; ++i)
        c->diffuse_area = c->diffuse_area && d->shapes[i].emitter < (int32_t)d->n_emitters;
    c->h_shapes = ds;
    c->h_bsdfs = db;
    c->h_emitters = de;
    c->h_area_cdf.assign(d->area_cdf, d->area_cdf + d->n_area_cdf);
    c->n_emit_faces = (int)ef_tri.size();
    c->h_emit_tris = nh::shadow_emitter_faces(*d);
    if (c->h_emit_tris.size() != 9 * ef_tri.size()) c->h_emit_tris.clear();
    c->small_image = c->small_image_ref = nullptr;
    c->flat_image = nullptr;
    c->pair_kinds = false;
    c->V.assign(d->V, d->V + 3 * nv);
    c->F.assign(d->F, d->F + 3 * (size_t)d->n_faces);
    c->width = d->camera.width;
    c->height = d->camera.height;
    c->border = d->filter.border;
    c->filter = d->filter;
    c->n_emitters = (int)d->n_emitters;
    c->integrator = S.integrator;
    if (d->sampler != NH_SAMPLER_INDEPENDENT && d->sampler != NH_SAMPLER_ADAPTIVE)
        return fail(c, "unknown sampler"), NH_ERR_INVALID;
    c->sampler = d->sampler;
    c->adaptive_initial_uniform = std::max(1, (int)d->adaptive_initial_uniform);
    adaptive_release(c);
    photon_release(c);
    c->av_set = false;

    (void)hipFree(c->fb);
    c->fb = nullptr;
    c->fb_floats = 4 * (size_t)(c->width + 2 * c->border) * (size_t)(c->height + 2 * c->border);
    HIP_TRY(c, hipMalloc(&c->fb, c->fb_floats * sizeof(float)));
    HIP_TRY(c, hipMemsetAsync(c->fb, 0, c->fb_floats * sizeof(float), c->stream));
    auto rank = nh::spiral_rank(c->width, c->height, 32, c->nbx, c->nby);
    (void)hipFree(c->block_rank);
    HIP_TRY(c, hipMalloc(&c->block_rank, rank.size() * sizeof(int)));
    HIP_TRY(c, hipMemcpyAsync(c->block_rank, rank.data(), rank.size() * sizeof(int), hipMemcpyHostToDevice, c->stream));
    HIP_TRY(c, hipStreamSynchronize(c->stream));
    c->has_scene = true;
    return NH_OK;
}

static int build_small_image(nh_ctx *c, const nh::GpuBvh &g) {
    c->small_image = c->small_image_ref = nullptr;
    c->flat_image = nullptr;
    c->pair_kinds = false;
    for (int &v : c->small_tab) v = 0;
    const size_t scene_bytes = 16 * (size_t)(c->n_node_f4 + c->n_prim_f4) + 8 * (size_t)c->n_leaves;
    if (scene_bytes > kSmallSceneBytes) return NH_OK;
    const int n = c->n_prim_f4 / 3;
    const int leaves_f4 = (c->n_leaves + 1) / 2;
    const int pairs_off = c->n_node_f4 + c->n_prim_f4 + leaves_f4;
    const bool frames = n <= kSmallFramesMaxPrims;
    std::vector<float4> tab;
    if (c->diffuse_area) {
        std::vector<nhd::DShape> sh = c->h_shapes;
        std::vector<float> cdf;
        for (const nhd::DEmitter &e : c->h_emitters) {
            nhd::DShape &s = sh[e.shape];
            if ((size_t)s.pdf_off + s.n_faces + 1 > c->h_area_cdf.size()) return fail(c, "area CDF out of range"), NH_ERR_INVALID;
            const int off = (int)cdf.size();
            cdf.insert(cdf.end(), c->h_area_cdf.begin() + s.pdf_off, c->h_area_cdf.begin() + s.pdf_off + s.n_faces + 1);
            s.pdf_off = off;
        }
        cdf.resize((cdf.size() + 3) / 4 * 4, 0.f);
        const size_t bytes = sh.size() * sizeof(nhd::DShape) + c->h_bsdfs.size() * sizeof(nhd::DBsdf) +
                             c->h_emitters.size() * sizeof(nhd::DEmitter) + cdf.size() * sizeof(float) +
                             3 * (size_t)c->n_emit_faces * sizeof(float4);
        if (bytes <= kSmallTablesBytes) {
            static_assert(sizeof(nhd::DShape) % 16 == 0 && sizeof(nhd::DBsdf) % 16 == 0 && sizeof(nhd::DEmitter) % 16 == 0,
                          "table records are whole float4s");
            c->small_tab[0] = (int)(sh.size() * sizeof(nhd::DShape) / 16);
            c->small_tab[1] = (int)(c->h_bsdfs.size() * sizeof(nhd::DBsdf) / 16);
            c->small_tab[2] = (int)(c->h_emitters.size() * sizeof(nhd::DEmitter) / 16);
            c->small_tab[3] = (int)(cdf.size() / 4);
            c->small_tab[4] = 3 * c->n_emit_faces;
            tab.resize((size_t)c->small_tab[0] + c->small_tab[1] + c->small_tab[2] + c->small_tab[3]);
            char *w = reinterpret_cast<char *>(tab.data());
            std::memcpy(w, sh.data(), sh.size() * sizeof(nhd::DShape));
            w += sh.size() * sizeof(nhd::DShape);
            std::memcpy(w, c->h_bsdfs.data(), c->h_bsdfs.size() * sizeof(nhd::DBsdf));
            w += c->h_bsdfs.size() * sizeof(nhd::DBsdf);
            std::memcpy(w, c->h_emitters.data(), c->h_emitters.size() * sizeof(nhd::DEmitter));
            w += c->h_emitters.size() * sizeof(nhd::DEmitter);
            std::memcpy(w, cdf.data(), cdf.size() * sizeof(float));
        }
    }
    const int tab_f4 = (int)tab.size() + c->small_tab[4];
    const int pleaves_off = pairs_off + nhd::kPairF4 * n, tab_off = pleaves_off + leaves_f4;
    const int frames_off = tab_off + tab_f4;
    const size_t total = (size_t)frames_off + (frames ? 3 * (size_t)n : 0);
    const auto d2d = [&](float4 *dst, const void *src, size_t bytes) {
        return bytes ? hipMemcpyAsync(dst, src, bytes, hipMemcpyDeviceToDevice, c->stream) : hipSuccess;
    };
    const char *pk = std::getenv("NH_PAIR_KINDS");
    c->pair_kinds = n > 0 && !(pk && pk[0] == '0');
    for (int pass = 0; pass < (c->pair_kinds ? 2 : 1); ++pass) {
        const bool by_kind = c->pair_kinds && pass == 0;
        const nh::PairLayout pl = nh::pair_layout(g.leaves.data(), c->n_leaves, g.prims.data(), n, by_kind);
        float4 *img = nullptr;
        HIP_TRY(c, hipMalloc(&img, std::max<size_t>(total, 1) * sizeof(float4)));
        c->bvh_bufs.push_back(img);
        HIP_TRY(c, hipMemsetAsync(img, 0, std::max<size_t>(total, 1) * sizeof(float4), c->stream));
        HIP_TRY(c, d2d(img, c->tv.nodes, 16 * (size_t)c->n_node_f4));
        HIP_TRY(c, d2d(img + c->n_node_f4, c->tv.prims, 16 * (size_t)c->n_prim_f4));
        HIP_TRY(c, d2d(img + c->n_node_f4 + c->n_prim_f4, c->tv.leaves, 8 * (size_t)c->n_leaves));
        if (n > 0) {
            const nh::i2 *slots = nullptr;
            if (int rc = upload(c, c->bvh_bufs, pl.slots.data(), pl.slots.size(), &slots)) return rc;
            nh::launch_small_image(c->tv, c->n_prim_f4, reinterpret_cast<const int2 *>(slots), pairs_off,
                                   frames ? frames_off : -1, img, c->stream);
            HIP_TRY(c, hipGetLastError());
        }
        if (c->n_leaves > 0)
            HIP_TRY(c, hipMemcpyAsync(img + pleaves_off, pl.leaves.data(), 8 * (size_t)c->n_leaves, hipMemcpyHostToDevice,
                                      c->stream));
        if (!tab.empty()) {
            float4 *t = img + tab_off;
            HIP_TRY(c, hipMemcpyAsync(t, tab.data(), tab.size() * sizeof(float4), hipMemcpyHostToDevice, c->stream));
            HIP_TRY(c, d2d(t + tab.size(), c->S.emit_faces, 16 * (size_t)c->small_tab[4]));
        }
        HIP_TRY(c, hipStreamSynchronize(c->stream));
        (pass == 0 ? c->small_image : c->small_image_ref) = img;
    }
    const bool one_leaf = g.root_kind == 2 && c->n_leaves == 1;
    bool two_leaves = g.root_kind == 1 && c->n_node_f4 == 4 && c->n_leaves == 2;
    if (two_leaves) {
        int refs[2];
        std::memcpy(refs, &g.nodes[3].x, sizeof(refs));
        two_leaves = refs[0] == ~0 && refs[1] == ~1;
    }
    if (c->pair_kinds && (one_leaf || two_leaves)) {
        float boxes[18];
        for (int i = 0; i < 3; ++i) {
            boxes[i] = g.root_min[i];
            boxes[3 + i] = g.root_max[i];
        }
        if (two_leaves) {
            const nh::f4 n0 = g.nodes[0], n1 = g.nodes[1], n2 = g.nodes[2];
            const float lr[12] = {n0.x, n0.y, n0.z, n0.w, n1.x, n1.y, n1.z, n1.w, n2.x, n2.y, n2.z, n2.w};
            std::memcpy(boxes + 6, lr, sizeof(lr));
        } else {
            std::memcpy(boxes + 6, boxes, 6 * sizeof(float));
            std::memcpy(boxes + 12, boxes, 6 * sizeof(float));
        }
        const nh::PairLayout pl = nh::pair_layout(g.leaves.data(), c->n_leaves, g.prims.data(), n, true);
        const nh::FlatImage fi = nh::flat_image(boxes, g.leaves.data(), c->n_leaves, g.prims.data(), n, pl, nh::flat_trace_knob());
        if (fi.flat) {
            const nh::f4 *dev = nullptr;
            if (int rc = upload(c, c->bvh_bufs, fi.data.data(), fi.data.size(), &dev)) return rc;
            HIP_TRY(c, hipStreamSynchronize(c->stream));
            c->flat_image = reinterpret_cast<const float4 *>(dev);
        }
    }
    return NH_OK;
}

int nh_set_av_params(nh_ctx *c, const nh_av_params *params) {
    if (!c) return NH_ERR_INVALID;
    if (!params || std::isnan(params->length)) return fail(c, "nh_set_av_params: invalid av parameters"), NH_ERR_INVALID;
    if (!c->has_scene) return fail(c, "nh_set_av_params: no scene uploaded"), NH_ERR_STATE;
    HIP_TRY(c, hipSetDevice(c->device));
    if (int rc = pipeline_drain(c)) return rc;
    HIP_TRY(c, hipStreamSynchronize(c->stream));
    c->S.av_length = params->length;
    if (c->d_scene && c->has_bvh)
        HIP_TRY(c, hipMemcpy(reinterpret_cast<char *>(c->d_scene) + offsetof(nhd::DScene, av_length), &c->S.av_length,
                             sizeof(float), hipMemcpyHostToDevice));
    c->av_set = true;
    return NH_OK;
}

int nh_upload_bvh(nh_ctx *c, const nh_bvh_desc *b) {
    if (!c || !b) return NH_ERR_INVALID;
    if (!c->has_scene) return fail(c, "nh_upload_bvh: upload the scene first"), NH_ERR_STATE;
    HIP_TRY(c, hipSetDevice(c->device));
    if (int rc_ = pipeline_drain(c)) return rc_;
    HIP_TRY(c, hipStreamSynchronize(c->stream));
    free_all(c->bvh_bufs);
    c->has_bvh = false;
    photon_release(c);
    c->wide_w = std::getenv("NH_WIDE8") && std::getenv("NH_WIDE8")[0] == '1' ? 8 : 4;
    int top_k = nh::tree_top_nodes() * 4 / c->wide_w;
    if (const char *e = std::getenv("NH_TREE_TOP")) top_k = std::min(std::max(0, std::atoi(e)), top_k);
    nh::GpuBvh g;
    if (int rc_ = nh::build_gpu_bvh(*b, c->shapes, c->V, c->F, c->shape_bsdf_type, c->shape_bsdf_real, c->wide_w, top_k,
                                    g, c->err))
        return rc_;
    nhd::DScene &S = c->S;
    S.root_kind = g.root_kind;
    for (int i = 0; i < 3; ++i) { S.root_min[i] = g.root_min[i]; S.root_max[i] = g.root_max[i]; }
    S.iso_spheres = g.iso_spheres;
    c->tv.n_top = g.n_top;
    int rc;
    c->n_node_f4 = (int)g.nodes.size();
    c->n_leaves = (int)g.leaves.size();
    c->n_prim_f4 = (int)g.prims.size() - 3;
    drop_primary_masks(c);
    c->h_prims.clear();
    if (c->n_prim_f4 > 0 && c->n_prim_f4 / 3 <= 64)
        c->h_prims.assign(&g.prims[0].x, &g.prims[0].x + 4 * (size_t)c->n_prim_f4);
    const nh::f4 *nodes = nullptr, *prims = nullptr, *wide = nullptr;
    const nh::i2 *leaves = nullptr;
    if ((rc = upload(c, c->bvh_bufs, g.nodes.data(), g.nodes.size(), &nodes))) return rc;
    if ((rc = upload(c, c->bvh_bufs, g.leaves.data(), g.leaves.size(), &leaves))) return rc;
    if ((rc = upload(c, c->bvh_bufs, g.prims.data(), g.prims.size(), &prims))) return rc;
    if (!g.wide.empty() && (rc = upload(c, c->bvh_bufs, g.wide.data(), g.wide.size(), &wide))) return rc;
    c->tv.nodes = reinterpret_cast<const float4 *>(nodes);
    c->tv.leaves = reinterpret_cast<const int2 *>(leaves);
    c->tv.prims = reinterpret_cast<const float4 *>(prims);
    c->tv.wnodes = reinterpret_cast<const float4 *>(wide);
    c->depth_wide = g.depth_wide;
    S.nodes = c->tv.nodes;
    S.prims = c->tv.prims;
    c->bvh_indices.assign(b->indices, b->indices + b->n_indices);
    c->shape_offset = g.shape_offset;
    c->depth = (int)g.tree_depth + 2;
    if (!c->d_scene) HIP_TRY(c, hipMalloc(&c->d_scene, sizeof(nhd::DScene)));
    HIP_TRY(c, hipMemcpyAsync(c->d_scene, &c->S, sizeof(nhd::DScene), hipMemcpyHostToDevice, c->stream));
    if ((rc = build_small_image(c, g))) return rc;
    HIP_TRY(c, hipStreamSynchronize(c->stream));
    c->has_bvh = true;
    return NH_OK;
}

}
```

### optix-renderer_amd/host/gpu_layout.cpp

```cpp
#include "gpu_layout.h"

#include <algorithm>
#include <cmath>
#include <cstdlib>
#include <cstring>
#include <functional>

#include "../csrc/nh_layout.h"
#include "nh_host.h"

namespace nh {

namespace {
using float4 = f4;
using int2 = i2;
struct int4 {
    int x, y, z, w;
};
inline float4 make_float4(float x, float y, float z, float w) { return float4{x, y, z, w}; }
inline int2 make_int2(int x, int y) { return int2{x, y}; }
inline int4 make_int4(int x, int y, int z, int w) { return int4{x, y, z, w}; }
inline u64x2 make_ulonglong2(uint64_t x, uint64_t y) { return u64x2{x, y}; }
}

// ... 374 lines not shown
}

int build_gpu_bvh(const nh_bvh_desc &desc, const std::vector<nh_shape> &shapes, const std::vector<float> &V,
                  const std::vector<uint32_t> &F, const std::vector<int> &shape_mat_key,
                  const std::vector<int> &shape_bsdf_real, int wide_w, int top_k, GpuBvh &S, std::string &err) {
    const nh_bvh_desc *b = &desc;
    auto fail = [&](const std::string &m) {
        err = m;
        return false;
    };
    S = GpuBvh{};
    std::vector<uint32_t> &off = S.shape_offset;
    off.assign(1, 0u);
    for (auto &s : shapes) off.push_back(off.back() + (s.type == NH_SHAPE_MESH ? s.n_faces : 1u));
    if (b->n_indices != off.back()) return fail("BVH primitive count does not match the scene"), NH_ERR_INVALID;
    if (b->n_indices > 0 && b->n_nodes == 0) return fail("empty BVH for a non-empty scene"), NH_ERR_INVALID;

    std::vector<float4> &nodes = S.nodes;
    std::vector<int2> &leaves = S.leaves;
    uint32_t &tree_depth = S.tree_depth;
    if (b->n_nodes == 0) {
        S.root_kind = 0;
    } else {
        const nh_bvh_node *N = b->nodes;
        for (int i = 0; i < 3; ++i) { S.root_min[i] = N[0].bbox_min[i]; S.root_max[i] = N[0].bbox_max[i]; }
        if (N[0].word0 & 1u) {
            S.root_kind = 2;
            leaves.push_back(make_int2((int)N[0].word1, (int)(N[0].word0 >> 1)));
        } else {
            S.root_kind = 1;
            std::vector<int> gid(b->n_nodes, -1);
            std::vector<uint32_t> order;
            std::vector<std::pair<uint32_t, uint32_t>> st{{0u, 0u}};
            while (!st.empty()) {
                const uint32_t i = st.back().first, lvl = st.back().second;
                st.pop_back();
                tree_depth = std::max(tree_depth, lvl);
                if (N[i].word0 & 1u) continue;
                if (gid[i] >= 0) return fail("corrupt BVH: node reached twice"), NH_ERR_INVALID;
                gid[i] = (int)order.size();
                order.push_back(i);
                if (N[i].word1 >= b->n_nodes || i + 1 >= b->n_nodes)
                    return fail("corrupt BVH child index"), NH_ERR_INVALID;
                st.push_back({N[i].word1, lvl + 1});
                st.push_back({i + 1, lvl + 1});
            }
            nodes.resize(4 * order.size());
            auto child_ref = [&](uint32_t ch) -> int {
                if (N[ch].word0 & 1u) {
                    leaves.push_back(make_int2((int)N[ch].word1, (int)(N[ch].word0 >> 1)));
                    return ~(int)(leaves.size() - 1);
                }
                return gid[ch];
            };
            for (size_t g = 0; g < order.size(); ++g) {
                uint32_t i = order[g];
                const nh_bvh_node &L = N[i + 1], &R = N[N[i].word1];
                int lr = child_ref(i + 1), rr = child_ref(N[i].word1);
                nodes[4 * g] = make_float4(L.bbox_min[0], L.bbox_min[1], L.bbox_min[2], L.bbox_max[0]);
                nodes[4 * g + 1] = make_float4(L.bbox_max[1], L.bbox_max[2], R.bbox_min[0], R.bbox_min[1]);
                nodes[4 * g + 2] = make_float4(R.bbox_min[2], R.bbox_max[0], R.bbox_max[1], R.bbox_max[2]);
                int4 r4 = make_int4(lr, rr, 0, 0);
                std::memcpy(&nodes[4 * g + 3], &r4, sizeof(int4));
            }
        }
    }
    std::vector<float4> &prims = S.prims;
    prims.resize(3 * (size_t)b->n_indices);
    for (uint32_t k = 0; k < b->n_indices; ++k) {
        uint32_t g = b->indices[k];
        if (g >= off.back()) return fail("BVH index out of range"), NH_ERR_INVALID;
        uint32_t s = (uint32_t)(std::upper_bound(off.begin(), off.end(), g) - off.begin()) - 1;
        uint32_t local = g - off[s];
        const nh_shape &sh = shapes[s];
        float4 *p = &prims[3 * (size_t)k];
        int si = (int)s, one = 1, zero = 0;
        float fs, f1, f0;
        std::memcpy(&fs, &si, 4);
        std::memcpy(&f1, &one, 4);
        std::memcpy(&f0, &zero, 4);
        const int mat = shape_mat_key[s] << nhd::kPrimMatShift;
        if (sh.type == NH_SHAPE_SPHERE) {
            const int flags = 1 | mat;
            std::memcpy(&f1, &flags, 4);
            p[0] = make_float4(sh.center[0], sh.center[1], sh.center[2], sh.radius);
            p[1] = make_float4(0, 0, 0, fs);
            p[2] = make_float4(0, 0, 0, f1);
        } else {
            std::memcpy(&f0, &mat, 4);
            const uint32_t *f = &F[3 * ((size_t)sh.f_offset + local)];
            const float *p0 = &V[3 * ((size_t)sh.v_offset + f[0])], *p1 = &V[3 * ((size_t)sh.v_offset + f[1])],
                        *p2 = &V[3 * ((size_t)sh.v_offset + f[2])];
            int li = (int)local;
            float fl;
            std::memcpy(&fl, &li, 4);
            p[0] = make_float4(p0[0], p0[1], p0[2], fl);
            p[1] = make_float4(p1[0], p1[1], p1[2], fs);
            p[2] = make_float4(p2[0], p2[1], p2[2], f0);
        }
    }
    S.iso_spheres = mark_isolated_spheres(prims, nodes, leaves, S.root_kind, shape_bsdf_real);
    for (const int2 &lf : leaves)
        if (lf.y > 0) {
            float4 &w = prims[3 * ((size_t)lf.x + lf.y - 1) + 2];
            int bits;
            std::memcpy(&bits, &w.w, 4);
            bits |= nhd::kPrimLeafEnd;
            std::memcpy(&w.w, &bits, 4);
        }
    if (tree_depth + 2 > (uint32_t)nhd::kMaxStack)
        return fail("BVH deeper than " + std::to_string(nhd::kMaxStack - 2) + " levels is not supported"), NH_ERR_UNSUPPORTED;
    int depth4 = 0;
    S.wide = collapse_wide(nodes, leaves, depth4, wide_w);
    S.n_top = S.root_kind == 1 ? number_top_first(S.wide, S.root_min, S.root_max, top_k, wide_w) : 0;
    S.depth_wide = (wide_w - 1) * depth4 + 1;
    prims.resize(prims.size() + 3, make_float4(0.f, 0.f, 0.f, 0.f));
    return NH_OK;
}

PairLayout pair_layout(const i2 *leaves, int n_leaves, const f4 *prims, int n_records, bool by_kind) {
    PairLayout out;
    out.slots.assign((size_t)n_records, make_int2(-1, -1));
    out.leaves.resize((size_t)n_leaves);
    if (!by_kind) {
        for (int p = 0; p < n_records; ++p) out.slots[(size_t)p] = make_int2(p, p + 1 < n_records ? p + 1 : -1);
        for (int l = 0; l < n_leaves; ++l) out.leaves[(size_t)l] = make_int2(leaves[l].x, 0);
        return out;
    }
    std::vector<int> kind[2];
    for (int l = 0; l < n_leaves; ++l) {
        const int2 lf = leaves[l];
        kind[0].clear();
        kind[1].clear();
        for (int k = lf.x; k < lf.x + lf.y; ++k) {
            int bits;
            std::memcpy(&bits, &prims[3 * (size_t)k + 2].w, 4);
            kind[bits & nhd::kPrimSphere ? 1 : 0].push_back(k);
        }
        int p = lf.x;
        for (const std::vector<int> &v : kind)
            for (size_t i = 0; i < v.size(); i += 2) out.slots[(size_t)p++] = make_int2(v[i], i + 1 < v.size() ? v[i + 1] : -1);
        const int n_tri = ((int)kind[0].size() + 1) / 2, n_sph = ((int)kind[1].size() + 1) / 2;
        out.leaves[(size_t)l] = make_int2(lf.x, n_tri | (n_sph << 16));
    }
    return out;
}

bool flat_trace_knob() {
    const char *e = std::getenv("NH_FLAT_TRACE");
    return !(e && e[0] == '0');
}

FlatImage flat_image(const float boxes[18], const i2 *leaves, int n_leaves, const f4 *prims, int n_records,
                     const PairLayout &pl, bool allowed) {
    FlatImage out;
    if (!allowed || n_leaves < 1 || n_leaves > 2 || n_records < 1 || (int)pl.leaves.size() != n_leaves) return out;
    int n_pairs = 0;
    for (int l = 0; l < n_leaves; ++l) {
        const int2 p = pl.leaves[(size_t)l];
        if (p.y == 0 && leaves[l].y > 0) return out;
        n_pairs += (p.y & 0xffff) + (p.y >> 16);
    }
    if (n_pairs < 1 || n_pairs > nhd::kFlatMaxPairs) return out;
    const auto same_bits = [](const float *a, const float *b) { return std::memcmp(a, b, 6 * sizeof(float)) == 0; };
    const auto as_float = [](int v) {
        float f;
        std::memcpy(&f, &v, 4);
        return f;
    };
    const float *root = boxes, *lb = n_leaves == 2 ? boxes + 6 : boxes, *rb = n_leaves == 2 ? boxes + 12 : boxes;
    out.box_equal = n_leaves == 1 ? nhd::kFlatLeftEq
                                  : (same_bits(lb, root) ? nhd::kFlatLeftEq : 0) | (same_bits(rb, root) ? nhd::kFlatRightEq : 0);
    out.data.reserve((size_t)nhd::kFlatHeaderF4 + (size_t)nhd::kPairF4 * n_pairs);
    out.data.push_back(make_float4(root[0], root[1], root[2], as_float(out.box_equal)));
    out.data.push_back(make_float4(root[3], root[4], root[5], as_float(n_leaves)));
    out.data.push_back(make_float4(lb[0], lb[1], lb[2], as_float(pl.leaves[0].y)));
    out.data.push_back(make_float4(lb[3], lb[4], lb[5], 0.f));
    out.data.push_back(make_float4(rb[0], rb[1], rb[2], as_float(n_leaves == 2 ? pl.leaves[1].y : 0)));
    out.data.push_back(make_float4(rb[3], rb[4], rb[5], 0.f));
    for (int l = 0; l < n_leaves; ++l) {
        const int2 p = pl.leaves[(size_t)l];
        for (int i = 0, n = (p.y & 0xffff) + (p.y >> 16); i < n; ++i) {
            const int2 s = pl.slots[(size_t)(p.x + i)];
            const int k = s.x, k1 = s.y < 0 ? k : s.y;
            if (k < 0 || k >= n_records || k1 >= n_records) return FlatImage{};
            const float4 a = prims[3 * (size_t)k], b = prims[3 * (size_t)k + 1], c = prims[3 * (size_t)k + 2];
            const float4 a1 = prims[3 * (size_t)k1], b1 = prims[3 * (size_t)k1 + 1], c1 = prims[3 * (size_t)k1 + 2];
            out.data.push_back(make_float4(a.x, a1.x, a.y, a1.y));
            out.data.push_back(make_float4(a.z, a1.z, a.w, a1.w));
            out.data.push_back(make_float4(b.x - a.x, b1.x - a1.x, b.y - a.y, b1.y - a1.y));
            out.data.push_back(make_float4(b.z - a.z, b1.z - a1.z, c.x - a.x, c1.x - a1.x));
            out.data.push_back(make_float4(c.y - a.y, c1.y - a1.y, c.z - a.z, c1.z - a1.z));
            out.data.push_back(make_float4(c.w, c1.w, as_float(k), as_float(k1)));
        }
    }
    out.flat = true;
    return out;
}

}

extern "C" {

int nh_flat_image(const float *records, int32_t n_records, const int32_t *leaves, int32_t n_leaves, const float *boxes,
                  int32_t allowed, float *image, int32_t image_cap_f4, int32_t *n_f4, int32_t *box_equal) {
    bool ok = n_records >= 0 && n_leaves >= 0 && (n_records == 0 || records) && (n_leaves == 0 || leaves) && boxes &&
              n_f4 && box_equal && image_cap_f4 >= 0 && (image_cap_f4 == 0 || image);
    std::vector<char> used((size_t)std::max(n_records, 0), 0);
    for (int l = 0; ok && l < n_leaves; ++l) {
        const int64_t s = leaves[2 * l], n = leaves[2 * l + 1];
        ok = s >= 0 && n >= 0 && n < 65535 && s + n <= n_records;
        for (int64_t k = s; ok && k < s + n; ++k) {
            ok = !used[(size_t)k];
            used[(size_t)k] = 1;
        }
    }
    if (!ok) {
        nh::set_host_error("nh_flat_image: invalid argument");
        return NH_ERR_INVALID;
    }
    const nh::i2 *lv = reinterpret_cast<const nh::i2 *>(leaves);
    const nh::f4 *rec = reinterpret_cast<const nh::f4 *>(records);
    const nh::PairLayout pl = nh::pair_layout(lv, n_leaves, rec, n_records, true);
    const nh::FlatImage fi = nh::flat_image(boxes, lv, n_leaves, rec, n_records, pl, allowed != 0 && nh::flat_trace_knob());
    *n_f4 = fi.flat ? (int32_t)fi.data.size() : 0;
    *box_equal = fi.box_equal;
    if (fi.flat) {
        if ((size_t)image_cap_f4 < fi.data.size()) {
            nh::set_host_error("nh_flat_image: image buffer too small");
            return NH_ERR_INVALID;
        }
        std::memcpy(image, fi.data.data(), fi.data.size() * sizeof(nh::f4));
    }
    return NH_OK;
}

int nh_pair_layout(const float *records, int32_t n_records, const int32_t *leaves, int32_t n_leaves, int32_t by_kind,
                   int32_t *slots, int32_t *leaf_pairs) {
    bool ok = n_records >= 0 && n_leaves >= 0 && (n_records == 0 || (records && slots)) &&
              (n_leaves == 0 || (leaves && leaf_pairs));
    std::vector<char> used((size_t)std::max(n_records, 0), 0);
    for (int l = 0; ok && l < n_leaves; ++l) {
        const int64_t s = leaves[2 * l], n = leaves[2 * l + 1];
        ok = s >= 0 && n >= 0 && n < 65535 && s + n <= n_records;
        for (int64_t k = s; ok && k < s + n; ++k) {
            ok = !used[(size_t)k];
            used[(size_t)k] = 1;
        }
    }
    if (!ok) {
        nh::set_host_error("nh_pair_layout: invalid argument");
        return NH_ERR_INVALID;
    }
    static_assert(sizeof(nh::f4) == 4 * sizeof(float) && sizeof(nh::i2) == 2 * sizeof(int32_t), "plain arrays");
    const nh::PairLayout pl = nh::pair_layout(reinterpret_cast<const nh::i2 *>(leaves), n_leaves,
                                              reinterpret_cast<const nh::f4 *>(records), n_records, by_kind != 0);
    if (n_records > 0) std::memcpy(slots, pl.slots.data(), (size_t)n_records * sizeof(nh::i2));
    for (int l = 0; l < n_leaves; ++l) {
        leaf_pairs[3 * l] = pl.leaves[(size_t)l].x;
        leaf_pairs[3 * l + 1] = pl.leaves[(size_t)l].y & 0xffff;
        leaf_pairs[3 * l + 2] = pl.leaves[(size_t)l].y >> 16;
    }
    return NH_OK;
}

}
```

### optix-renderer_amd/host/gpu_layout.h

```cpp
#pragma once
#include <cstdint>
#include <string>
#include <vector>

#include "nori_hip.h"

namespace nh {

struct f4 {
    float x, y, z, w;
};
struct i2 {
    int x, y;
};
struct u64x2 {
    uint64_t x, y;
};

struct GpuBvh {
    std::vector<f4> nodes;
    std::vector<i2> leaves;
    std::vector<f4> prims;
    std::vector<f4> wide;
    std::vector<uint32_t> shape_offset;
    int root_kind = 0;
    float root_min[3] = {0.f, 0.f, 0.f}, root_max[3] = {0.f, 0.f, 0.f};
    uint32_t tree_depth = 0;
    int depth_wide = 1;
    int n_top = 0;
    int iso_spheres = 0;
};

int build_gpu_bvh(const nh_bvh_desc &b, const std::vector<nh_shape> &shapes, const std::vector<float> &V,
                  const std::vector<uint32_t> &F, const std::vector<int> &shape_mat_key,
                  const std::vector<int> &shape_bsdf_real, int wide_w, int top_k, GpuBvh &out, std::string &err);

std::vector<f4> collapse_wide(const std::vector<f4> &nodes, const std::vector<i2> &leaves, int &depth_out, int W = 4);
int number_top_first(std::vector<f4> &wide, const float root_min[3], const float root_max[3], int K, int W = 4);

std::vector<int> spiral_rank(int w, int h, int bs, int &nbx, int &nby);
std::vector<uint32_t> serial_ray_index(int w, int h, int bs);

struct LensTables {
    std::vector<u64x2> pix, lo;
    std::vector<uint64_t> hi;
};
LensTables lens_tables(int w, int h);

bool nee_finite(const nh_scene_desc *d);

bool primary_masks(const nh_camera &cam, const f4 *prims, int n_records, const int32_t *blocks, int n_blocks,
                   std::vector<uint64_t> &masks);
int primary_mask_pad(int width, int height);
bool primary_mask_in_front(const nh_camera &cam, const f4 *prims, int n_records, std::vector<char> &in_front);

uint64_t shadow_emitter_mask(const f4 *prims, int n_records, const float *emit_faces, int n_faces);
std::vector<float> shadow_emitter_faces(const nh_scene_desc &d);
bool shadow_block_masks(const nh_camera &cam, const f4 *prims, int n_records, const float *emit_faces, int n_faces,
                        const int32_t *blocks, int n_blocks, std::vector<uint64_t> &masks);

struct PairLayout {
    std::vector<i2> slots, leaves;
};
PairLayout pair_layout(const i2 *leaves, int n_leaves, const f4 *prims, int n_records, bool by_kind);

struct FlatImage {
    bool flat = false;
    int box_equal = 0;
    std::vector<f4> data;
};
FlatImage flat_image(const float boxes[18], const i2 *leaves, int n_leaves, const f4 *prims, int n_records,
                     const PairLayout &pl, bool allowed);
bool flat_trace_knob();

}
```

### optix-renderer_amd/host/shadow_masks.cpp

```cpp
#include <algorithm>
#include <cmath>
#include <cstring>

#include "gpu_layout.h"
#include "nh_host.h"

#include "../csrc/nh_layout.h"

namespace nh {

namespace {

struct V3 {
    double x, y, z;
};
V3 operator-(V3 a, V3 b) { return V3{a.x - b.x, a.y - b.y, a.z - b.z}; }
V3 operator+(V3 a, V3 b) { return V3{a.x + b.x, a.y + b.y, a.z + b.z}; }
V3 operator*(double s, V3 a) { return V3{s * a.x, s * a.y, s * a.z}; }
double dot(V3 a, V3 b) { return a.x * b.x + a.y * b.y + a.z * b.z; }
V3 cross(V3 a, V3 b) { return V3{a.y * b.z - a.z * b.y, a.z * b.x - a.x * b.z, a.x * b.y - a.y * b.x}; }
double norm(V3 a) { return std::sqrt(dot(a, a)); }

const double kU = std::ldexp(1.0, -24);

struct AABB {
    V3 lo{INFINITY, INFINITY, INFINITY}, hi{-INFINITY, -INFINITY, -INFINITY};
    void add(V3 p) {
        lo = V3{std::min(lo.x, p.x), std::min(lo.y, p.y), std::min(lo.z, p.z)};
        hi = V3{std::max(hi.x, p.x), std::max(hi.y, p.y), std::max(hi.z, p.z)};
    }
    bool empty() const { return !(lo.x <= hi.x); }
    bool meets(const AABB &o, double g) const {
        return lo.x - g <= o.hi.x && o.lo.x <= hi.x + g && lo.y - g <= o.hi.y && o.lo.y <= hi.y + g &&
               lo.z - g <= o.hi.z && o.lo.z <= hi.z + g;
    }
};

struct Face {
    V3 p[3], n;
};

struct Record {
    bool sphere;
    V3 p[3];
    double r;
    V3 n;
    double sin_t;
    double len;
    double rho;
    double grown;
    AABB box;
};

double sphere_grown(double r, double far_d) {
    const double g = r + 1e-3 * r + 64.0 * kU * far_d * far_d / std::max(r, 1e-300);
    return 1.5 * g;
}

struct Analysis {
    bool ok = false;
    std::vector<Face> faces;
    std::vector<Record> rec;
    AABB scene, emit;
    double eps_o = 0, eta = 0, d_e = 0, m = 0;
    uint64_t emitter_word = ~(uint64_t)0;
};

Analysis analyse(const f4 *prims, int n_records, const float *emit_faces, int n_faces) {
    Analysis A;
    if (n_records <= 0 || n_records > 64 || n_faces <= 0 || !emit_faces) return A;
    double min_sin = 1.0, max_abs = 0.0;
    for (int f = 0; f < n_faces; ++f) {
        Face F;
        for (int j = 0; j < 3; ++j) {
            F.p[j] = V3{emit_faces[9 * f + 3 * j], emit_faces[9 * f + 3 * j + 1], emit_faces[9 * f + 3 * j + 2]};
            A.emit.add(F.p[j]);
            max_abs = std::max({max_abs, std::fabs(F.p[j].x), std::fabs(F.p[j].y), std::fabs(F.p[j].z)});
        }
        const V3 e1 = F.p[1] - F.p[0], e2 = F.p[2] - F.p[0], c = cross(e1, e2);
        const double a2 = norm(c), l = norm(e1) * norm(e2);
        if (!(a2 > 0.0) || !std::isfinite(a2) || !(l > 0.0)) return A;
        min_sin = std::min(min_sin, a2 / l);
        F.n = (1.0 / a2) * c;
        A.faces.push_back(F);
    }
    if (!(min_sin >= 1.0 / 16)) return A;
    A.rec.resize((size_t)n_records);
    for (int k = 0; k < n_records; ++k) {
        const f4 a = prims[3 * k], b = prims[3 * k + 1], c = prims[3 * k + 2];
        int bits;
        std::memcpy(&bits, &c.w, sizeof(bits));
        Record &R = A.rec[(size_t)k];
        R.sphere = (bits & nhd::kPrimSphere) != 0;
        R.p[0] = V3{a.x, a.y, a.z};
        R.rho = INFINITY;
        if (R.sphere) {
            R.r = std::fabs((double)a.w);
            R.box.add(V3{a.x - R.r, a.y - R.r, a.z - R.r});
            R.box.add(V3{a.x + R.r, a.y + R.r, a.z + R.r});
        } else {
            R.p[1] = V3{b.x, b.y, b.z};
            R.p[2] = V3{c.x, c.y, c.z};
            for (int j = 0; j < 3; ++j) R.box.add(R.p[j]);
        }
        A.scene.add(R.box.lo);
        A.scene.add(R.box.hi);
    }
    if (!std::isfinite(A.scene.lo.x + A.scene.lo.y + A.scene.lo.z + A.scene.hi.x + A.scene.hi.y + A.scene.hi.z)) return A;
    const V3 ext = A.scene.hi - A.scene.lo;
    A.m = 1e-4 * std::max({ext.x, ext.y, ext.z});
    for (const Face &F : A.faces)
        for (int j = 0; j < 3; ++j)
            for (int i = 0; i < 8; ++i) {
                const V3 q{i & 1 ? A.scene.hi.x : A.scene.lo.x, i & 2 ? A.scene.hi.y : A.scene.lo.y,
                           i & 4 ? A.scene.hi.z : A.scene.lo.z};
                A.d_e = std::max(A.d_e, norm(q - F.p[j]));
            }
    A.eps_o = 8.0 * kU * max_abs;
    A.eta = 32.0 * kU / min_sin;
    for (Record &R : A.rec) {
        if (R.sphere) {
            double far_d = 0;
            for (const Face &F : A.faces)
                for (int j = 0; j < 3; ++j) far_d = std::max(far_d, norm(F.p[j] - R.p[0]) + R.r);
            R.grown = sphere_grown(R.r, far_d);
            R.rho = R.grown - R.r;
            continue;
        }
        const V3 e1 = R.p[1] - R.p[0], e2 = R.p[2] - R.p[0], c = cross(e1, e2);
        const double a2 = norm(c), l1 = norm(e1), l2 = norm(e2);
        R.n = V3{0, 0, 0};
        R.sin_t = 0;
        R.len = std::max(l1, l2);
        if (!(a2 > 0.0) || !(l1 * l2 > 0.0)) continue;
        R.n = (1.0 / a2) * c;
        R.sin_t = a2 / (l1 * l2);
        double s = INFINITY, reach = 0;
        int side = 0;
        bool one_side = true;
        for (const Face &F : A.faces)
            for (int j = 0; j < 3; ++j) {
                const double h = dot(R.n, F.p[j] - R.p[0]);
                const int sg = h > 0 ? 1 : h < 0 ? -1 : 0;
                if (sg == 0 || (side && sg != side)) one_side = false;
                side = sg;
                s = std::min(s, std::fabs(h));
                for (int i = 0; i < 3; ++i) reach = std::max(reach, norm(F.p[j] - R.p[i]));
            }
        s -= A.eps_o;
        if (!one_side || !(s > 0.0) || !(32.0 * kU * reach <= s * R.sin_t)) continue;
        R.rho = 64.0 * kU * (reach + R.len + A.d_e) * A.d_e / (s * R.sin_t);
    }
    A.ok = true;
    uint64_t word = n_records < 64 ? ~(uint64_t)0 << n_records : 0;
    for (int k = 0; k < n_records; ++k) {
        const Record &R = A.rec[(size_t)k];
        bool behind = std::isfinite(R.rho);
        const double delta = A.eps_o + 1.01 * A.d_e * A.eta + (R.sphere ? 0.0 : R.rho);
        for (size_t f = 0; f < A.faces.size() && behind; ++f) {
            const Face &F = A.faces[f];
            if (R.sphere) {
                for (int i = 0; i < 8 && behind; ++i) {
                    const V3 q{R.p[0].x + (i & 1 ? R.grown : -R.grown), R.p[0].y + (i & 2 ? R.grown : -R.grown),
                               R.p[0].z + (i & 4 ? R.grown : -R.grown)};
                    behind = dot(F.n, q - F.p[0]) <= -delta;
                }
            } else {
                for (int j = 0; j < 3 && behind; ++j) behind = dot(F.n, R.p[j] - F.p[0]) <= -delta;
            }
        }
        if (!behind) word |= (uint64_t)1 << k;
    }
    A.emitter_word = word;
    return A;
}

void clip(const std::vector<V3> &in, V3 org, V3 n, std::vector<V3> &out) {
    out.clear();
    const size_t k = in.size();
    for (size_t i = 0; i < k; ++i) {
        const V3 a = in[i], b = in[(i + 1) % k];
        const double da = dot(n, a - org), db = dot(n, b - org);
        if (da >= 0) out.push_back(a);
        if ((da >= 0) != (db >= 0)) out.push_back(a + (da / (da - db)) * (b - a));
    }
}

}

std::vector<float> shadow_emitter_faces(const nh_scene_desc &d) {
    std::vector<float> out;
    if (d.n_emitters == 0) return out;
    for (uint32_t i = 0; i < d.n_emitters; ++i) {
        const nh_emitter &e = d.emitters[i];
        if (e.type != NH_EMITTER_AREA || e.shape < 0 || (uint32_t)e.shape >= d.n_shapes) return out;
        const nh_shape &s = d.shapes[e.shape];
        if (s.type != NH_SHAPE_MESH || s.has_normals || s.emitter < 0) return out;
    }
    for (uint32_t i = 0; i < d.n_shapes; ++i) {
        const nh_shape &s = d.shapes[i];
        if (s.emitter < 0) continue;
        if (s.type != NH_SHAPE_MESH || s.has_normals || (uint64_t)s.f_offset + s.n_faces > d.n_faces) return {};
        for (uint32_t f = 0; f < s.n_faces; ++f)
            for (int j = 0; j < 3; ++j) {
                const uint64_t v = (uint64_t)s.v_offset + d.F[3 * ((size_t)s.f_offset + f) + j];
                if (v >= d.n_vertices) return {};
                out.insert(out.end(), d.V + 3 * v, d.V + 3 * v + 3);
            }
    }
    return out;
}

uint64_t shadow_emitter_mask(const f4 *prims, int n_records, const float *emit_faces, int n_faces) {
    return analyse(prims, n_records, emit_faces, n_faces).emitter_word;
}

bool shadow_block_masks(const nh_camera &cam, const f4 *prims, int n_records, const float *emit_faces, int n_faces,
                        const int32_t *blocks, int n_blocks, std::vector<uint64_t> &masks) {
    masks.clear();
    std::vector<uint64_t> pm;
    std::vector<char> in_front;
    if (!primary_masks(cam, prims, n_records, blocks, n_blocks, pm) ||
        !primary_mask_in_front(cam, prims, n_records, in_front))
        return false;
    const Analysis A = analyse(prims, n_records, emit_faces, n_faces);
    masks.assign((size_t)std::max(n_blocks, 0), 0);
    bool all_in_front = true;
    for (char c : in_front) all_in_front = all_in_front && c;
    const int nbx = (cam.width + 31) / 32, nby = (cam.height + 31) / 32;
    const double pad = primary_mask_pad(cam.width, cam.height);
    const float *cw = cam.camera_to_world;
    const V3 org{(double)cw[3] / cw[15], (double)cw[7] / cw[15], (double)cw[11] / cw[15]};
    const auto direction = [&](double x, double y, V3 &d) {
        const float *m = cam.sample_to_camera;
        const double sx = x / cam.width, sy = y / cam.height;
        double r[4];
        for (int i = 0; i < 4; ++i) r[i] = m[4 * i] * sx + m[4 * i + 1] * sy + m[4 * i + 3];
        const V3 l{r[0] / r[3], r[1] / r[3], r[2] / r[3]};
        d = V3{cw[0] * l.x + cw[1] * l.y + cw[2] * l.z, cw[4] * l.x + cw[5] * l.y + cw[6] * l.z,
               cw[8] * l.x + cw[9] * l.y + cw[10] * l.z};
        const double len = norm(d);
        if (!(len > 0.0) || !std::isfinite(len)) return false;
        d = (1.0 / len) * d;
        return true;
    };
    std::vector<V3> poly, tmp;
    for (int i = 0; i < n_blocks; ++i) {
        const uint64_t p = pm[(size_t)i];
        if (!p) continue;
        masks[(size_t)i] = A.emitter_word;
        const int bid = blocks[i];
        if (!A.ok || !all_in_front || bid < 0 || bid >= nbx * nby) continue;
        const int bx = bid % nbx, by = bid / nbx;
        const double x0 = 32.0 * bx - pad, x1 = std::min(32.0 * bx + 32.0, (double)cam.width) + pad;
        const double y0 = 32.0 * by - pad, y1 = std::min(32.0 * by + 32.0, (double)cam.height) + pad;
        V3 d[4], mid;
        if (!direction(x0, y0, d[0]) || !direction(x1, y0, d[1]) || !direction(x1, y1, d[2]) ||
            !direction(x0, y1, d[3]) || !direction(0.5 * (x0 + x1), 0.5 * (y0 + y1), mid))
            continue;
        V3 pn[4];
        bool planes_ok = true;
        double cone_cos = 1.0;
        for (int e = 0; e < 4; ++e) {
            pn[e] = cross(d[e], d[(e + 1) & 3]);
            const double s = dot(pn[e], mid);
            if (s < 0) pn[e] = -1.0 * pn[e];
            planes_ok = planes_ok && s != 0.0;
            for (int j = 0; j < 4; ++j) cone_cos = std::min(cone_cos, dot(d[e], d[j]));
        }
        if (!planes_ok || !(cone_cos > 0.5)) continue;
        AABB region;
        double w = 0;
        bool grazing = false;
        for (int k = 0; k < n_records && !grazing; ++k) {
            if (!((p >> k) & 1)) continue;
            const Record &R = A.rec[(size_t)k];
            if (R.sphere) {
                double dist = norm(R.p[0] - org);
                const double G = sphere_grown(R.r, dist + R.r), reach = std::sqrt(3.0) * G;
                const double t0 = std::max(dist - reach, 0.0), t1 = (dist + reach) / cone_cos;
                AABB fr, sb;
                for (int e = 0; e < 4; ++e) {
                    fr.add(org + t0 * d[e]);
                    fr.add(org + t1 * d[e]);
                }
                sb.add(V3{R.p[0].x - G, R.p[0].y - G, R.p[0].z - G});
                sb.add(V3{R.p[0].x + G, R.p[0].y + G, R.p[0].z + G});
                if (!fr.meets(sb, 0.0)) continue;
                region.add(V3{std::max(fr.lo.x, sb.lo.x), std::max(fr.lo.y, sb.lo.y), std::max(fr.lo.z, sb.lo.z)});
                region.add(V3{std::min(fr.hi.x, sb.hi.x), std::min(fr.hi.y, sb.hi.y), std::min(fr.hi.z, sb.hi.z)});
                continue;
            }
            double c_min = INFINITY, reach = 0;
            int side = 0;
            for (int e = 0; e < 4; ++e) {
                const double c = dot(R.n, d[e]);
                const int sg = c > 0 ? 1 : c < 0 ? -1 : 0;
                if (sg == 0 || (side && sg != side)) grazing = true;
                side = sg;
                c_min = std::min(c_min, std::fabs(c));
            }
            for (int j = 0; j < 3; ++j) reach = std::max(reach, norm(R.p[j] - org));
            if (grazing || !(R.sin_t > 0.0)) {
                grazing = true;
                break;
            }
            w = std::max(w, 64.0 * kU * (reach + R.len) / (R.sin_t * c_min));
            poly.assign(R.p, R.p + 3);
            for (int e = 0; e < 4 && !poly.empty(); ++e) {
                clip(poly, org, pn[e], tmp);
                poly.swap(tmp);
            }
            for (const V3 &q : poly) region.add(q);
        }
        if (grazing || !std::isfinite(w)) continue;
        AABB target = A.emit;
        if (!region.empty()) {
            target.add(region.lo);
            target.add(region.hi);
        }
        uint64_t keep = 0;
        for (int k = 0; k < n_records; ++k) {
            const Record &R = A.rec[(size_t)k];
            if (!std::isfinite(R.rho) || R.box.meets(target, A.m + A.eps_o + w + R.rho)) keep |= (uint64_t)1 << k;
        }
        if (n_records < 64) keep |= ~(uint64_t)0 << n_records;
        masks[(size_t)i] = keep & A.emitter_word;
    }
    return true;
}

}

extern "C" {

int nh_shadow_emitter_faces(const nh_scene_desc *scene, float *faces, int32_t cap_faces, int32_t *n_faces) {
    if (!scene || !n_faces || cap_faces < 0 || (cap_faces > 0 && !faces)) {
        nh::set_host_error("nh_shadow_emitter_faces: invalid argument");
        return NH_ERR_INVALID;
    }
    const std::vector<float> f = nh::shadow_emitter_faces(*scene);
    *n_faces = (int32_t)(f.size() / 9);
    if (*n_faces > cap_faces) {
        nh::set_host_error("nh_shadow_emitter_faces: more faces than the caller has room for");
        return NH_ERR_INVALID;
    }
    if (!f.empty()) std::memcpy(faces, f.data(), f.size() * sizeof(float));
    return NH_OK;
}

int nh_shadow_masks(const nh_camera *camera, const float *records, int32_t n_records, const float *emit_faces,
                    int32_t n_emit_faces, const int32_t *blocks, int32_t n_blocks, uint64_t *emitter_mask,
                    uint64_t *masks, int32_t *built) {
    if (!camera || !built || !emitter_mask || n_records < 0 || n_blocks < 0 || (n_records > 0 && !records) ||
        (n_emit_faces > 0 && !emit_faces) || (n_blocks > 0 && (!blocks || !masks))) {
        nh::set_host_error("nh_shadow_masks: invalid argument");
        return NH_ERR_INVALID;
    }
    const nh::f4 *prims = reinterpret_cast<const nh::f4 *>(records);
    *emitter_mask = nh::shadow_emitter_mask(prims, n_records, emit_faces, n_emit_faces);
    std::vector<uint64_t> m;
    *built = nh::shadow_block_masks(*camera, prims, n_records, emit_faces, n_emit_faces, blocks, n_blocks, m) ? 1 : 0;
    if (*built && n_blocks > 0) std::memcpy(masks, m.data(), (size_t)n_blocks * sizeof(uint64_t));
    return NH_OK;
}

}
```

### optix-renderer_amd/nori_hip.py

```python
from __future__ import annotations

import ctypes as C
import os

import numpy as np

_HERE = os.path.dirname(os.path.abspath(__file__))
LIB_PATH = os.environ.get("NH_LIB_PATH") or os.path.join(_HERE, "lib", "libnori_hip.so")

from nh_env import raise_hw_queues

if not os.path.exists(LIB_PATH):
    raise ImportError(f"nori_hip: HIP library not built ({LIB_PATH}); run `make` or __graft_entry__.build()")
_lib = C.CDLL(LIB_PATH)

NH_OK = 0
SHAPE_MESH, SHAPE_SPHERE = 0, 1
BSDF_DIFFUSE, BSDF_MIRROR, BSDF_DIELECTRIC, BSDF_MICROFACET = 0, 1, 2, 3
BSDF_DISNEY = 4
BSDF_QUERY_EVAL, BSDF_QUERY_SAMPLE = 0, 1
EMITTER_AREA, EMITTER_POINT, EMITTER_ENVMAP = 0, 1, 2
EMITTER_SPOT, EMITTER_DIRECTIONAL = 3, 4
EMITTER_QUERY_SAMPLE, EMITTER_QUERY_EVAL, EMITTER_QUERY_PDF = 0, 1, 2
EMITTER_QUERY_SAMPLE_STRIDE, EMITTER_QUERY_IN_STRIDE = 16, 9
# ... 12 lines not shown
ADAPTIVE_MAX_SAMPLES = 133948
LENS_DRAWS_LTR, LENS_DRAWS_RTL = 0, 1

_f = C.c_float
_i32 = C.c_int32
_u32 = C.c_uint32
_fp = C.POINTER(C.c_float)
_u32p = C.POINTER(C.c_uint32)


class nh_shape(C.Structure):
    _fields_ = [("type", _i32), ("bsdf", _i32), ("emitter", _i32), ("v_offset", _u32), ("n_vertices", _u32),
                ("f_offset", _u32), ("n_faces", _u32), ("has_normals", _i32), ("has_uvs", _i32),
                ("center", _f * 3), ("radius", _f), ("bbox_min", _f * 3), ("bbox_max", _f * 3),
                ("pdf_offset", _u32), ("pdf_normalization", _f), ("normal_map", _u32)]


DISNEY_PARAMS = ("metallic", "subsurface", "specular", "roughness", "specular_tint", "anisotropic", "sheen",
                 "sheen_tint", "clearcoat", "clearcoat_gloss")
DISNEY_DEFAULTS = dict(zip(DISNEY_PARAMS, (0.0, 0.0, 0.5, 0.5, 0.0, 0.0, 0.0, 0.5, 0.0, 1.0)))


class nh_bsdf(C.Structure):
    _fields_ = [("type", _i32), ("albedo", _f * 3), ("alpha", _f), ("int_ior", _f), ("ext_ior", _f),
                ("kd", _f * 3), ("ks", _f), ("albedo_texture", _u32)] + [(n, _f) for n in DISNEY_PARAMS]


TEXTURE_CONSTANT, TEXTURE_CHECKERBOARD, TEXTURE_PNG = 0, 1, 2


class nh_texture(C.Structure):
    _fields_ = [("type", _i32), ("value1", _f * 3), ("value2", _f * 3), ("delta", _f * 2), ("scale", _f * 2),
                ("width", _i32), ("height", _i32), ("texel_offset", C.c_uint64), ("scale_u", _f), ("scale_v", _f),
                ("offset_u", _f), ("offset_v", _f), ("spherical", _i32), ("rotation", _f * 9), ("linear", _i32),
                ("intensity", _f), ("pad", _i32)]


class nh_emitter(C.Structure):
    _fields_ = [("type", _i32), ("shape", _i32), ("radiance", _f * 3), ("light_prob", _f),
                ("position", _f * 3), ("pad", _f)]


class nh_emitter_ext(C.Structure):
    _fields_ = [("direction", _f * 3), ("cos_total_width", _f), ("frame_s", _f * 3), ("cos_falloff_start", _f),
                ("frame_t", _f * 3), ("cos_theta_max", _f), ("frame_n", _f * 3), ("pad", _f)]


class nh_medium(C.Structure):
    _fields_ = [("type", _i32), ("mu_a", _f * 3), ("mu_s", _f * 3), ("mu_t", _f * 3), ("density", _f),
                ("phase", _i32), ("g", _f)]


class nh_camera(C.Structure):
    _fields_ = [("width", _i32), ("height", _i32), ("sample_to_camera", _f * 16), ("camera_to_world", _f * 16),
                ("inv_output_size", _f * 2), ("near_clip", _f), ("far_clip", _f), ("lens_radius", _f),
                ("focal_distance", _f), ("lens_draw_order", _i32)]


class nh_filter(C.Structure):
    _fields_ = [("radius", _f), ("border", _i32), ("lookup_factor", _f), ("table", _f * 33)]


class nh_envmap(C.Structure):
    _fields_ = [("width", _i32), ("height", _i32), ("rgba", _fp), ("radiance", _f * 3), ("scale_u", _f),
                ("scale_v", _f), ("offset_u", _f), ("offset_v", _f), ("spherical", _i32), ("constant", _i32),
                ("cdf", _fp), ("normalization", _f), ("rotation", _f * 9)]


class nh_denoiser(C.Structure):
    _fields_ = [("type", _i32), ("sigma_d", _f), ("sigma_vr", _f), ("range", _i32), ("amount", _i32)]


def simple_denoiser(sigma_d: float = 0.0, sigma_vr: float = 0.6, range: int = 1, amount: int = 1) -> nh_denoiser:
    eps = np.float32(1e-4)

    def clampf(v, lo, hi):
        v = np.float32(v)
        return float(lo if v < lo else (hi if v > hi else v))
    d = nh_denoiser()
    d.type = DENOISER_SIMPLE
    d.sigma_d = clampf(sigma_d, eps, np.float32(10))
    d.sigma_vr = clampf(sigma_vr, eps, np.float32(10))
    d.range = int(min(max(range, 0), 50))
    d.amount = int(min(max(amount, 1), 10))
    return d


class nh_scene_desc(C.Structure):
    _fields_ = [("camera", nh_camera), ("filter", nh_filter), ("integrator", _i32), ("sample_count", _i32),
                ("n_shapes", _u32), ("shapes", C.POINTER(nh_shape)), ("n_bsdfs", _u32),
                ("bsdfs", C.POINTER(nh_bsdf)), ("n_emitters", _u32), ("emitters", C.POINTER(nh_emitter)),
                ("emitter_cdf", _fp), ("envmap", _i32), ("n_vertices", _u32), ("V", _fp), ("N", _fp),
                ("UV", _fp), ("T", _fp), ("BT", _fp), ("n_faces", _u32), ("F", _u32p), ("n_area_cdf", _u32),
                ("area_cdf", _fp), ("env", nh_envmap), ("denoiser", nh_denoiser), ("n_textures", _u32),
                ("textures", C.POINTER(nh_texture)), ("n_texels", C.c_uint64), ("texels", _fp),
                ("normals_direction", _f * 3), ("emitter_ext", C.POINTER(nh_emitter_ext)),
                ("n_media", _u32), ("media", C.POINTER(nh_medium)), ("shape_medium", _u32p),
                ("ambient_medium", _u32), ("sampler", _i32), ("adaptive_initial_uniform", _i32)]


class nh_bvh_node(C.Structure):
    _fields_ = [("word0", _u32), ("word1", _u32), ("bbox_min", _f * 3), ("bbox_max", _f * 3)]


class nh_bvh_desc(C.Structure):
    _fields_ = [("n_nodes", _u32), ("nodes", C.POINTER(nh_bvh_node)), ("n_indices", _u32), ("indices", _u32p),
                ("n_shapes", _u32), ("shape_offset", _u32p), ("bbox_min", _f * 3), ("bbox_max", _f * 3),
                ("max_depth", _u32)]


class nh_ray_soa(C.Structure):
    _fields_ = [(n, _fp) for n in ("ox", "oy", "oz", "dx", "dy", "dz", "mint", "maxt")]


class nh_hit_soa(C.Structure):
    _fields_ = [("hit", C.POINTER(C.c_uint8)), ("t", _fp), ("u", _fp), ("v", _fp), ("prim", _u32p),
                ("shape", _u32p)]


class nh_render_req(C.Structure):
    _fields_ = [("sample_begin", _i32), ("sample_end", _i32), ("seed", C.c_uint64), ("n_blocks", _i32),
                ("blocks", C.POINTER(_i32)), ("mode", _i32), ("traversal", _i32), ("clear", _i32),
                ("collect_stats", _i32)]


class nh_adaptive_stats(C.Structure):
    _fields_ = [("total_samples", C.c_uint64), ("passes", C.c_uint64), ("max_passes", C.c_uint64),
                ("n_blocks", C.c_uint64)]


class nh_render_stats(C.Structure):
    _fields_ = [("kernel_ms_path", C.c_double), ("kernel_ms_splat", C.c_double), ("kernel_ms_extend", C.c_double),
                ("kernel_ms_shadow", C.c_double), ("kernel_ms_shade", C.c_double), ("launches_path", C.c_uint64),
                ("launches_splat", C.c_uint64), ("launches_extend", C.c_uint64), ("launches_shadow", C.c_uint64),
                ("launches_shade", C.c_uint64), ("samples", C.c_uint64), ("ray_queries", C.c_uint64),
                ("nodes_visited", C.c_uint64), ("boxes_tested", C.c_uint64), ("prims_tested", C.c_uint64),
                ("invalid_samples", C.c_uint64), ("shadow_queries", C.c_uint64),
                ("shadow_nodes_visited", C.c_uint64), ("shadow_boxes_tested", C.c_uint64),
                ("shadow_prims_tested", C.c_uint64), ("shade_state_bytes", C.c_uint64),
                ("extend_queue_bytes", C.c_uint64), ("shadow_queue_bytes", C.c_uint64),
                ("paths_shaded", C.c_uint64), ("kernel_ms_tail", C.c_double), ("launches_tail", C.c_uint64),
                ("node_bytes", C.c_uint64)] + [
        (n, C.c_uint64) for n in ("tail_queries", "tail_nodes_visited", "tail_boxes_tested", "tail_prims_tested",
                                  "tail_shadow_queries", "tail_shadow_nodes_visited", "tail_shadow_boxes_tested",
                                  "tail_shadow_prims_tested", "lds_scene", "fused_bounce", "comm_inits")] + [
        ("kernel_ms_denoise", C.c_double), ("launches_denoise", C.c_uint64), ("tails_async", C.c_uint64),
        ("pools_active", C.c_uint64), ("trace_fused", C.c_uint64)] + [
        (n, C.c_uint64) for n in ("tail_cycles_body", "tail_cycles_shadow", "tail_cycles_closest", "tail_cycles_head",
                                  "tail_bounces", "tail_max_bounces", "tail_coop_cycles_body",
                                  "tail_coop_cycles_shadow", "tail_coop_cycles_closest", "tail_coop_cycles_head",
                                  "tail_coop_bounces", "bounce_cycles_load", "bounce_cycles_body",
                                  "bounce_cycles_shadow", "bounce_cycles_closest", "bounce_cycles_head",
                                  "bounce_cycles_store", "bounce_bounces", "bounce_traits", "primary_masks",
                                  "pair_kinds", "flat_trace", "shadow_masks")]


def _sig(name, res, *args):
    fn = getattr(_lib, name)
    fn.restype = res
    fn.argtypes = list(args)
    return fn


_vp = C.c_void_p
_sig("nh_scene_load_xml", _i32, C.c_char_p, C.POINTER(_vp))
_sig("nh_scene_load_xml_index", _i32, C.c_char_p, _i32, C.POINTER(_vp))
_sig("nh_scene_get_desc", _i32, _vp, C.POINTER(nh_scene_desc))
_sig("nh_scene_set_resolution", _i32, _vp, _i32, _i32)
_sig("nh_scene_set_sample_count", _i32, _vp, _i32)
_sig("nh_scene_set_sampler", _i32, _vp, _i32, _i32)
_sig("nh_scene_set_bsdf", _i32, _vp, _u32, C.POINTER(nh_bsdf))
_sig("nh_scene_set_integrator", _i32, _vp, _i32)
_sig("nh_scene_add_texture", _u32, _vp, C.POINTER(nh_texture), _fp)
_sig("nh_scene_set_normal_map", _i32, _vp, _u32, _u32)
_sig("nh_scene_set_lens_draw_order", _i32, _vp, _i32)
_sig("nh_texture_decode", _i32, C.POINTER(C.c_uint8), C.c_uint64, _i32, _fp)
_sig("nh_scene_free", None, _vp)
_sig("nh_host_last_error", C.c_char_p)
_sig("nh_debug_transform", _i32, C.c_char_p, _fp, _i32)
_sig("nh_bvh_build", _i32, C.POINTER(nh_scene_desc), _i32, C.POINTER(_vp))
_sig("nh_bvh_get_desc", _i32, _vp, C.POINTER(nh_bvh_desc))
_sig("nh_bvh_free", None, _vp)
_sig("nh_primary_masks", _i32, C.POINTER(nh_camera), _fp, _i32, C.POINTER(_i32), _i32, C.POINTER(C.c_uint64),
     C.POINTER(_i32))
_sig("nh_primary_mask_pad", _i32, _i32, _i32)
_sig("nh_shadow_emitter_faces", _i32, C.POINTER(nh_scene_desc), _fp, _i32, C.POINTER(_i32))
_sig("nh_shadow_masks", _i32, C.POINTER(nh_camera), _fp, _i32, _fp, _i32, C.POINTER(_i32), _i32, C.POINTER(C.c_uint64),
     C.POINTER(C.c_uint64), C.POINTER(_i32))
_sig("nh_pair_layout", _i32, _fp, _i32, C.POINTER(_i32), _i32, _i32, C.POINTER(_i32), C.POINTER(_i32))
_sig("nh_flat_image", _i32, _fp, _i32, C.POINTER(_i32), _i32, _fp, _i32, _fp, _i32, C.POINTER(_i32), C.POINTER(_i32))
_sig("nh_framebuffer_to_rgb", _i32, _fp, _i32, _i32, _i32, _fp)
_sig("nh_write_pfm", _i32, C.c_char_p, _fp, _i32, _i32)
_sig("nh_image_load_png", _i32, C.c_char_p, C.POINTER(C.c_uint8), C.c_size_t, C.POINTER(_i32), C.POINTER(_i32))
_sig("nh_write_exr", _i32, C.c_char_p, _fp, _i32, _i32)
_sig("nh_write_png", _i32, C.c_char_p, _fp, _i32, _i32)
_sig("nh_rgb_to_ldr", _i32, _fp, _i32, _i32, C.POINTER(C.c_uint8))
_sig("nh_get_device_count", _i32, C.POINTER(C.c_int))
_sig("nh_create", _i32, C.c_int, C.POINTER(_vp))
_sig("nh_destroy", None, _vp)
_sig("nh_upload_scene", _i32, _vp, C.POINTER(nh_scene_desc))
_sig("nh_upload_bvh", _i32, _vp, C.POINTER(nh_bvh_desc))
_sig("nh_trace_rays", _i32, _vp, C.POINTER(nh_ray_soa), _i32, _i32, _i32, C.POINTER(nh_hit_soa))
_sig("nh_render", _i32, _vp, C.POINTER(nh_render_req))
_sig("nh_synchronize", _i32, _vp)
_sig("nh_get_framebuffer", _i32, _vp, _fp, C.c_size_t)
_sig("nh_framebuffer_device_ptr", _i32, _vp, C.POINTER(_vp), C.POINTER(C.c_size_t))
_sig("nh_get_stats", _i32, _vp, C.POINTER(nh_render_stats))
_sig("nh_reset_stats", _i32, _vp)
_sig("nh_get_adaptive_stats", _i32, _vp, C.POINTER(nh_adaptive_stats))
_sig("nh_get_adaptive_variance", _i32, _vp, _fp, C.c_size_t)
_sig("nh_reduce_framebuffers", _i32, C.POINTER(_vp), _i32, _i32)
_sig("nh_denoise", _i32, _vp, C.POINTER(nh_denoiser))
_sig("nh_denoise_image", _i32, _vp, _fp, _i32, _i32, _i32, C.POINTER(nh_denoiser))
_sig("nh_bsdf_query", _i32, _vp, C.POINTER(nh_bsdf), _fp, _i32, _i32, _fp, _fp, _fp, _fp, _fp, _fp, C.POINTER(_i32))
_sig("nh_emitter_query", _i32, _vp, _u32, _i32, _i32, _fp, _fp, _fp)
_sig("nh_medium_query", _i32, _vp, _u32, _i32, _i32, _fp, _fp)
_sig("nh_last_error", C.c_char_p, _vp)


class nh_test_desc(C.Structure):
    _fields_ = [("type", _i32), ("significance_level", _f), ("sample_count", _i32), ("n_angles", _u32),
                ("angles", _fp), ("n_references", _u32), ("references", _fp), ("n_scenes", _u32), ("n_bsdfs", _u32),
                ("bsdfs", C.POINTER(nh_bsdf))]


class nh_test_result(C.Structure):
    _fields_ = [("mean", C.c_double), ("variance", C.c_double), ("reference", C.c_double), ("p_value", C.c_double),
                ("accepted", _i32), ("sample_count", _i32), ("angle", _f), ("pad", _i32)]


TEST_TTEST, TEST_CHI2TEST = 0, 1
RADIANCE_QUERY_MAX = 1 << 24
_dp = C.POINTER(C.c_double)
_i32p = C.POINTER(_i32)
_sig("nh_test_load_xml", _i32, C.c_char_p, C.POINTER(_vp))
_sig("nh_test_get_desc", _i32, _vp, C.POINTER(nh_test_desc))
_sig("nh_test_free", None, _vp)
_sig("nh_students_t_test", _i32, C.c_double, C.c_double, C.c_double, _i32, C.c_double, _i32, _i32p, _dp)
_sig("nh_radiance_query", _i32, _vp, C.c_uint64, _i32, _i32p, _i32p, _fp, _fp, _fp)
_sig("nh_ttest_scene", _i32, _vp, C.c_uint64, C.c_int64, _i32, _dp, _dp, _fp)
_sig("nh_ttest_bsdf", _i32, _vp, C.POINTER(nh_bsdf), _fp, _f, C.c_uint64, _i32, _dp, _dp, _fp)
_sig("nh_test_run", _i32, C.c_int, C.c_char_p, C.c_uint64, C.POINTER(nh_test_result), _i32, _i32p)


INTEGRATOR_PHOTONMAPPER = 9
EMITTER_QUERY_SAMPLE_PHOTON, EMITTER_QUERY_PHOTON_STRIDE = 3, 12
PHOTON_QUERY_CODEC, PHOTON_QUERY_GATHER = 0, 1
PHOTON_STREAM = 1 << 32
PHOTON_DEFAULT_BATCH = 1 << 18


class nh_photon_params(C.Structure):
    _fields_ = [("photon_count", _i32), ("photon_radius", _f)]


class nh_photon_stats(C.Structure):
    _fields_ = [("stored", _i32), ("emitted", _i32), ("radius", _f), ("cell_size", _f),
                ("occupied_cells", C.c_uint64)]


_u8p = C.POINTER(C.c_uint8)
_sig("nh_scene_get_photon_params", _i32, _vp, C.POINTER(nh_photon_params))
_sig("nh_scene_set_photon_params", _i32, _vp, C.POINTER(nh_photon_params))
_sig("nh_photon_tables", _i32, _fp, _fp, _fp, _fp, _fp)
_sig("nh_photon_map_build", _i32, _vp, C.POINTER(nh_photon_params), C.c_uint64, _i32)
_sig("nh_get_photon_stats", _i32, _vp, C.POINTER(nh_photon_stats))
_sig("nh_get_photons", _i32, _vp, _i32, _i32, _fp, _fp, _fp, _u8p, _i32p, _i32p)
_sig("nh_photon_query", _i32, _vp, _i32, _i32, _fp, _u8p, _i32p, _fp)


INTEGRATOR_AV, INTEGRATOR_ENVMAPTESTER = 10, 11


class nh_av_params(C.Structure):
    _fields_ = [("length", _f)]


_sig("nh_scene_get_av_params", _i32, _vp, C.POINTER(nh_av_params))
_sig("nh_scene_set_av_params", _i32, _vp, C.POINTER(nh_av_params))
_sig("nh_set_av_params", _i32, _vp, C.POINTER(nh_av_params))


def photon_tables() -> dict:
    t = {k: np.zeros(256, np.float32) for k in ("cos_theta", "sin_theta", "cos_phi", "sin_phi", "exp")}
    _host_check(_lib.nh_photon_tables(*[_fptr(t[k]) for k in ("cos_theta", "sin_theta", "cos_phi", "sin_phi", "exp")]),
                "photon_tables")
    return t


lib = _lib
_hip_used = False


def configure_runtime(min_hw_queues: int = 8) -> int:
    if _hip_used:
        raise RuntimeError("configure_runtime: the HIP runtime is already initialised in this process")
    return raise_hw_queues(min_hw_queues)


class NoriError(RuntimeError):
    pass


def _fptr(a):
    return a.ctypes.data_as(_fp)


def _host_check(rc, what):
    if rc != NH_OK:
        raise NoriError(f"{what}: {_lib.nh_host_last_error().decode()}")


class Scene:

    def __init__(self, path: str, index: int = 0):
        h = _vp()
        _host_check(_lib.nh_scene_load_xml_index(path.encode(), index, C.byref(h)), f"load {path}")
        self._h = h
        self.path = path

    def __del__(self):
        if getattr(self, "_h", None):
            _lib.nh_scene_free(self._h)
            self._h = None

    @property
    def desc(self) -> nh_scene_desc:
        d = nh_scene_desc()
        _host_check(_lib.nh_scene_get_desc(self._h, C.byref(d)), "get_desc")
        return d

    def set_resolution(self, w: int, h: int):
        _host_check(_lib.nh_scene_set_resolution(self._h, w, h), "set_resolution")

    def set_sample_count(self, spp: int):
        _host_check(_lib.nh_scene_set_sample_count(self._h, spp), "set_sample_count")

    def set_sampler(self, type: int, initial_uniform: int = 2):
        _host_check(_lib.nh_scene_set_sampler(self._h, type, initial_uniform), "set_sampler")

    def set_integrator(self, integ: int):
        _host_check(_lib.nh_scene_set_integrator(self._h, integ), "set_integrator")

# ... 343 lines not shown
        out = np.array(rgbw, dtype=np.float32, order="C", copy=True)
        h, w = out.shape[0] - 2 * border, out.shape[1] - 2 * border
        self._check(_lib.nh_denoise_image(self._h, _fptr(out), w, h, border, C.byref(params)), "denoise_image")
        return out

    def bsdf_query(self, bsdf: nh_bsdf, wi: np.ndarray, wo: np.ndarray = None, sample: np.ndarray = None,
                   albedo=None) -> dict:
        if (wo is None) == (sample is None):
            raise ValueError("bsdf_query: give either wo (eval) or sample (sample)")
        wi = np.ascontiguousarray(wi, dtype=np.float32).reshape(-1, 3)
        n = len(wi)
        out = {"value": np.zeros((n, 3), np.float32), "pdf": np.zeros(n, np.float32)}
        alb = None if albedo is None else np.ascontiguousarray(albedo, dtype=np.float32).reshape(3)
        if wo is not None:
            wo = np.ascontiguousarray(wo, dtype=np.float32).reshape(n, 3)
            rc = _lib.nh_bsdf_query(self._h, C.byref(bsdf), None if alb is None else _fptr(alb), BSDF_QUERY_EVAL, n,
                                    _fptr(wi), _fptr(wo), None, None, _fptr(out["value"]), _fptr(out["pdf"]), None)
        else:
            sample = np.ascontiguousarray(sample, dtype=np.float32).reshape(n, 2)
            out["wo"] = np.zeros((n, 3), np.float32)
            out["measure"] = np.zeros(n, np.int32)
            rc = _lib.nh_bsdf_query(self._h, C.byref(bsdf), None if alb is None else _fptr(alb), BSDF_QUERY_SAMPLE, n,
                                    _fptr(wi), None, _fptr(sample), _fptr(out["wo"]), _fptr(out["value"]),
                                    _fptr(out["pdf"]), out["measure"].ctypes.data_as(C.POINTER(_i32)))
        self._check(rc, "bsdf_query")
        return out

    def emitter_query(self, emitter: int, ref: np.ndarray, sample: np.ndarray = None, wi: np.ndarray = None,
                      p: np.ndarray = None, n: np.ndarray = None, mode: int = None) -> dict:
        if (sample is None) == (wi is None):
            raise ValueError("emitter_query: give either sample (sample) or wi (eval and pdf)")
        ref = np.ascontiguousarray(ref, dtype=np.float32).reshape(-1, 3)
        m = len(ref)

        def call(md, inp, out):
            self._check(_lib.nh_emitter_query(self._h, emitter, md, m, _fptr(ref), _fptr(inp), _fptr(out)),
                        "emitter_query")
            return out
        if sample is not None:
            sample = np.ascontiguousarray(sample, dtype=np.float32).reshape(m, 2)
            o = call(EMITTER_QUERY_SAMPLE, sample, np.zeros((m, EMITTER_QUERY_SAMPLE_STRIDE), np.float32))
            return {"value": o[:, 0:3].copy(), "wi": o[:, 3:6].copy(), "pdf": o[:, 6].copy(), "o": o[:, 7:10].copy(),
                    "d": o[:, 10:13].copy(), "mint": o[:, 13].copy(), "maxt": o[:, 14].copy()}
        inp = np.zeros((m, EMITTER_QUERY_IN_STRIDE), np.float32)
        inp[:, 0:3] = np.asarray(wi, np.float32).reshape(m, 3)
        if p is not None:
            inp[:, 3:6] = np.asarray(p, np.float32).reshape(m, 3)
        if n is not None:
            inp[:, 6:9] = np.asarray(n, np.float32).reshape(m, 3)
        out = {}
        if mode in (None, EMITTER_QUERY_EVAL):
            out["value"] = call(EMITTER_QUERY_EVAL, inp, np.zeros((m, 3), np.float32))
        if mode in (None, EMITTER_QUERY_PDF):
            out["pdf"] = call(EMITTER_QUERY_PDF, inp, np.zeros(m, np.float32))
        return out

    def medium_query(self, medium: int, mode: int, inp: np.ndarray) -> np.ndarray:
        n_in, n_out = {MEDIUM_QUERY_FREE_PATH: (2, 2), MEDIUM_QUERY_TRANSMITTANCE: (6, 3),
                       MEDIUM_QUERY_PHASE_SAMPLE: (2, 4), MEDIUM_QUERY_PHASE_PDF: (3, 1)}[mode]
        inp = np.ascontiguousarray(inp, dtype=np.float32).reshape(-1, n_in)
        out = np.zeros((len(inp), n_out), np.float32)
        self._check(_lib.nh_medium_query(self._h, medium, mode, len(inp), _fptr(inp), _fptr(out)), "medium_query")
        return out[:, 0] if n_out == 1 else out

    def radiance_query(self, pixel, sample, seed: int = 0, pixel_sample=None) -> dict:
        pixel = np.ascontiguousarray(pixel, dtype=np.int32).ravel()
        sample = np.ascontiguousarray(np.broadcast_to(np.asarray(sample, dtype=np.int32), pixel.shape))
        n = len(pixel)
        ps = None if pixel_sample is None else np.ascontiguousarray(pixel_sample, dtype=np.float32).reshape(n, 2)
        out = {"rgb": np.zeros((n, 3), np.float32), "jitter": np.zeros((n, 2), np.float32)}
        self._check(_lib.nh_radiance_query(self._h, seed, n, pixel.ctypes.data_as(_i32p), sample.ctypes.data_as(_i32p),
                                           None if ps is None else _fptr(ps), _fptr(out["rgb"]), _fptr(out["jitter"])),
                    "radiance_query")
        return out

    def ttest_scene(self, n: int, seed: int = 0, first: int = 0, luminance: bool = False):
        m, v = C.c_double(0.0), C.c_double(0.0)
        lum = np.zeros(max(n, 0), np.float32) if luminance else None
        self._check(_lib.nh_ttest_scene(self._h, seed, first, n, C.byref(m), C.byref(v),
                                        None if lum is None else _fptr(lum)), "ttest_scene")
        return (m.value, v.value, lum) if luminance else (m.value, v.value)

    def ttest_bsdf(self, bsdf: nh_bsdf, angle_deg: float, n: int, first_draw: int = 0, albedo=None,
                   luminance: bool = False):
        m, v = C.c_double(0.0), C.c_double(0.0)
        lum = np.zeros(max(n, 0), np.float32) if luminance else None
        alb = None if albedo is None else np.ascontiguousarray(albedo, dtype=np.float32).reshape(3)
        self._check(_lib.nh_ttest_bsdf(self._h, C.byref(bsdf), None if alb is None else _fptr(alb), angle_deg, first_draw,
                                       n, C.byref(m), C.byref(v), None if lum is None else _fptr(lum)), "ttest_bsdf")
        return (m.value, v.value, lum) if luminance else (m.value, v.value)

    def trace(self, o: np.ndarray, d: np.ndarray, mint: np.ndarray, maxt: np.ndarray, any_hit=False,
              traversal: int = TRAVERSAL_REFERENCE) -> dict:
        n = len(o)
        cols = [np.ascontiguousarray(x, dtype=np.float32) for x in (o[:, 0], o[:, 1], o[:, 2], d[:, 0], d[:, 1],
                                                                     d[:, 2], mint, maxt)]
        r = nh_ray_soa(*[_fptr(c) for c in cols])
        res = {"hit": np.zeros(n, np.uint8), "t": np.zeros(n, np.float32), "u": np.zeros(n, np.float32),
               "v": np.zeros(n, np.float32), "prim": np.zeros(n, np.uint32), "shape": np.zeros(n, np.uint32)}
        h = nh_hit_soa(res["hit"].ctypes.data_as(C.POINTER(C.c_uint8)), _fptr(res["t"]), _fptr(res["u"]),
                       _fptr(res["v"]), res["prim"].ctypes.data_as(_u32p), res["shape"].ctypes.data_as(_u32p))
        self._check(_lib.nh_trace_rays(self._h, C.byref(r), n, int(any_hit), traversal, C.byref(h)), "trace_rays")
        return res


def tile_shard(width: int, height: int, world: int, rank: int) -> list:
    nbx, nby = (width + 31) // 32, (height + 31) // 32
    return [b for b in range(nbx * nby) if b % world == rank]


def primary_mask_pad(width: int, height: int) -> int:
    return int(_lib.nh_primary_mask_pad(width, height))


def primary_masks(camera: nh_camera, records: np.ndarray, blocks):
    rec = np.ascontiguousarray(records, dtype=np.float32).reshape(-1, 12)
    blk = np.ascontiguousarray(blocks, dtype=np.int32).ravel()
    out = np.zeros(len(blk), np.uint64)
    built = _i32(0)
    _host_check(_lib.nh_primary_masks(C.byref(camera), _fptr(rec), len(rec), blk.ctypes.data_as(C.POINTER(_i32)),
                                      len(blk), out.ctypes.data_as(C.POINTER(C.c_uint64)), C.byref(built)),
                "primary_masks")
    return out if built.value else None


def shadow_emitter_faces(desc: nh_scene_desc):
    out, n = np.zeros((max(int(desc.n_faces), 1), 9), np.float32), _i32(0)
    _host_check(_lib.nh_shadow_emitter_faces(C.byref(desc), _fptr(out), len(out), C.byref(n)), "shadow_emitter_faces")
    return out[:n.value].copy()


def shadow_masks(camera: nh_camera, records: np.ndarray, emit_faces, blocks):
    rec = np.ascontiguousarray(records, dtype=np.float32).reshape(-1, 12)
    blk = np.ascontiguousarray(blocks, dtype=np.int32).ravel()
    ef = np.zeros((0, 9), np.float32) if emit_faces is None else np.ascontiguousarray(emit_faces, np.float32).reshape(-1, 9)
    out = np.zeros(len(blk), np.uint64)
    word, built = C.c_uint64(0), _i32(0)
    _host_check(_lib.nh_shadow_masks(C.byref(camera), _fptr(rec), len(rec), _fptr(ef), len(ef),
                                     blk.ctypes.data_as(C.POINTER(_i32)), len(blk), C.byref(word),
                                     out.ctypes.data_as(C.POINTER(C.c_uint64)), C.byref(built)), "shadow_masks")
    return int(word.value), (out if built.value else None)


def pair_layout(records: np.ndarray, leaves, by_kind: bool = True):
    rec = np.ascontiguousarray(records, dtype=np.float32).reshape(-1, 12)
    lv = np.ascontiguousarray(leaves, dtype=np.int32).reshape(-1, 2)
    slots, lp = np.zeros((len(rec), 2), np.int32), np.zeros((len(lv), 3), np.int32)
    ip = C.POINTER(_i32)
    _host_check(_lib.nh_pair_layout(_fptr(rec), len(rec), lv.ctypes.data_as(ip), len(lv), 1 if by_kind else 0,
                                    slots.ctypes.data_as(ip), lp.ctypes.data_as(ip)), "pair_layout")
    return slots, lp


def flat_image(records: np.ndarray, leaves, boxes, allowed: bool = True):
    rec = np.ascontiguousarray(records, dtype=np.float32).reshape(-1, 12)
    lv = np.ascontiguousarray(leaves, dtype=np.int32).reshape(-1, 2)
    bx = np.ascontiguousarray(boxes, dtype=np.float32).ravel()
    assert bx.size == 18
    cap = 6 + 6 * 16
    img, n, eq = np.zeros((cap, 4), np.float32), _i32(0), _i32(0)
    _host_check(_lib.nh_flat_image(_fptr(rec), len(rec), lv.ctypes.data_as(C.POINTER(_i32)), len(lv), _fptr(bx),
                                   1 if allowed else 0, _fptr(img), cap, C.byref(n), C.byref(eq)), "flat_image")
    return (img[:n.value].copy() if n.value else None), int(eq.value)


def reduce_framebuffers(ctxs, root: int = 0):
    arr = (_vp * len(ctxs))(*[c._h for c in ctxs])
    rc = _lib.nh_reduce_framebuffers(arr, len(ctxs), root)
    if rc != NH_OK:
        raise NoriError(f"nh_reduce_framebuffers failed ({rc})")


def to_rgb(rgbw: np.ndarray, border: int) -> np.ndarray:
    h, w = rgbw.shape[0] - 2 * border, rgbw.shape[1] - 2 * border
    src = np.ascontiguousarray(rgbw, dtype=np.float32)
    out = np.zeros((h, w, 3), np.float32)
    rc = _lib.nh_framebuffer_to_rgb(_fptr(src), w, h, border, _fptr(out))
    if rc != NH_OK:
        raise NoriError("framebuffer_to_rgb failed")
    return out


def write_exr(path: str, rgb: np.ndarray):
    rgb = np.ascontiguousarray(rgb, dtype=np.float32)
    _host_check(_lib.nh_write_exr(path.encode(), _fptr(rgb), rgb.shape[1], rgb.shape[0]), "write_exr")


def write_png(path: str, rgb: np.ndarray):
    rgb = np.ascontiguousarray(rgb, dtype=np.float32)
    _host_check(_lib.nh_write_png(path.encode(), _fptr(rgb), rgb.shape[1], rgb.shape[0]), "write_png")


def rgb_to_ldr(rgb: np.ndarray) -> np.ndarray:
    rgb = np.ascontiguousarray(rgb, dtype=np.float32)
    out = np.empty(rgb.shape[:2] + (3,), np.uint8)
    _host_check(_lib.nh_rgb_to_ldr(_fptr(rgb), rgb.shape[1], rgb.shape[0],
                                   out.ctypes.data_as(C.POINTER(C.c_uint8))), "rgb_to_ldr")
    return out


def write_pfm(path: str, rgb: np.ndarray):
    rgb = np.ascontiguousarray(rgb, dtype=np.float32)
    _host_check(_lib.nh_write_pfm(path.encode(), _fptr(rgb), rgb.shape[1], rgb.shape[0]), "write_pfm")


def load_png(path: str) -> np.ndarray:
    w, h = _i32(), _i32()
    _host_check(_lib.nh_image_load_png(path.encode(), None, 0, C.byref(w), C.byref(h)), "load_png")
    out = np.zeros((h.value, w.value, 4), np.uint8)
    _host_check(_lib.nh_image_load_png(path.encode(), out.ctypes.data_as(C.POINTER(C.c_uint8)), out.nbytes,
                                       C.byref(w), C.byref(h)), "load_png")
    return out
```

Before: 8840 Msamples/s.

## Add reduced any-hit primitive list for flat shadow-ray traversal

On the host, a conservative geometric analysis over the camera origin and lens, the emitter faces and the wall planes marks which primitives can never block a shadow ray. Those primitives are left out of a second pair-record list appended to the flat BVH image. In the any-hit (shadow) path, the flat traversal reads per-leaf counts and a header flag to walk only that reduced list, and skips a leaf entirely when its list is empty. The feature is on by default through an NH_ANY_LIST environment knob and is exposed through new C and Python entry points. It costs a larger flat image and extra host analysis, and correctness rests on the analysis staying conservative under float rounding.

```diff
diff --git a/include/nori_hip.h b/include/nori_hip.h
--- a/include/nori_hip.h
+++ b/include/nori_hip.h
@@ -279,6 +279,7 @@
     uint64_t pair_kinds;
     uint64_t flat_trace;
     uint64_t shadow_masks;
+    uint64_t any_list;
 } nh_render_stats;
 
 typedef struct nh_scene nh_scene;
@@ -325,12 +326,17 @@
 int nh_shadow_masks(const nh_camera *camera, const float *records, int32_t n_records, const float *emit_faces,
                     int32_t n_emit_faces, const int32_t *blocks, int32_t n_blocks, uint64_t *emitter_mask,
                     uint64_t *masks, int32_t *built);
+int nh_shadow_any_word(const nh_camera *camera, const float *records, int32_t n_records, const float *emit_faces,
+                       int32_t n_emit_faces, uint64_t *word);
 
 int nh_pair_layout(const float *records, int32_t n_records, const int32_t *leaves, int32_t n_leaves, int32_t by_kind,
                    int32_t *slots, int32_t *leaf_pairs);
 
 int nh_flat_image(const float *records, int32_t n_records, const int32_t *leaves, int32_t n_leaves, const float *boxes,
                   int32_t allowed, float *image, int32_t image_cap_f4, int32_t *n_f4, int32_t *box_equal);
+int nh_flat_image_any(const float *records, int32_t n_records, const int32_t *leaves, int32_t n_leaves,
+                      const float *boxes, int32_t allowed, uint64_t any_word, float *image, int32_t image_cap_f4,
+                      int32_t *n_f4, int32_t *box_equal);
 
 int nh_framebuffer_to_rgb(const float *rgbw, int32_t width, int32_t height, int32_t border, float *rgb);
 int nh_write_pfm(const char *path, const float *rgb, int32_t width, int32_t height);
diff --git a/optix-renderer_amd/csrc/nh_ctx.h b/optix-renderer_amd/csrc/nh_ctx.h
--- a/optix-renderer_amd/csrc/nh_ctx.h
+++ b/optix-renderer_amd/csrc/nh_ctx.h
@@ -173,6 +173,7 @@
     bool pair_kinds = false;
     float4 *small_image_ref = nullptr;
     const float4 *flat_image = nullptr;
+    int flat_any_records = 0;
     nh_camera camera{};
     std::vector<float> h_prims;
     unsigned long long *pmask = nullptr;
diff --git a/optix-renderer_amd/csrc/nh_layout.h b/optix-renderer_amd/csrc/nh_layout.h
--- a/optix-renderer_amd/csrc/nh_layout.h
+++ b/optix-renderer_amd/csrc/nh_layout.h
@@ -12,7 +12,8 @@
 
 constexpr int kPairF4 = 6;
 constexpr int kFlatHeaderF4 = 6, kFlatMaxPairs = 16;
-constexpr int kFlatLeftEq = 1, kFlatRightEq = 2;
+constexpr int kFlatLeftEq = 1, kFlatRightEq = 2, kFlatAnyList = 4;
+constexpr int kFlatAnyOff = kFlatHeaderF4 + kPairF4 * kFlatMaxPairs;
 
 constexpr int kMaxStack = 128;
 
diff --git a/optix-renderer_amd/csrc/nh_pipeline.hip b/optix-renderer_amd/csrc/nh_pipeline.hip
--- a/optix-renderer_amd/csrc/nh_pipeline.hip
+++ b/optix-renderer_amd/csrc/nh_pipeline.hip
@@ -225,6 +225,7 @@
     const bool flat = p.rr && c->flat_image && c->pair_kinds && !j.stats && !c->disney;
     L.flat = flat ? c->flat_image : nullptr;
     c->stats.flat_trace = flat ? 1 : 0;
+    c->stats.any_list = flat ? (uint64_t)c->flat_any_records : 0;
     c->stats.fused_bounce = p.fused ? 1 : 0;
     c->stats.node_bytes = p.wide ? 16 * nhd::kWideF4 * (c->wide_w / 4) : 64;
     c->stats.lds_scene = small && !p.persistent && c->depth <= 16 ? 1 : 0;
@@ -840,6 +841,7 @@
     c->stats.shadow_masks = 0;
     c->stats.pair_kinds = 0;
     c->stats.flat_trace = 0;
+    c->stats.any_list = 0;
     c->stats.trace_fused = 0;
     c->stats.lds_scene = 0;
     c->stats.fused_bounce = 0;
diff --git a/optix-renderer_amd/csrc/nh_traverse.h b/optix-renderer_amd/csrc/nh_traverse.h
--- a/optix-renderer_amd/csrc/nh_traverse.h
+++ b/optix-renderer_amd/csrc/nh_traverse.h
@@ -587,15 +587,23 @@
     if (!box(h0, h1, near_root)) return false;
     const int eq = __float_as_int(h0.w);
     const bool two = __float_as_int(h1.w) == 2;
-    bool hl = true, hr = false;
+    int cl = __float_as_int(h2.w), cr = __float_as_int(h4.w);
+    const float4 *pl = fl + kFlatHeaderF4;
+    if constexpr (ANY) {
+        if (eq & kFlatAnyList) {
+            cl = __float_as_int(h3.w);
+            cr = __float_as_int(h5.w);
+            pl = fl + kFlatAnyOff;
+        }
+    }
+    bool hl = !ANY || cl != 0, hr = false;
     float nl = near_root, nr = near_root;
-    if (!(eq & kFlatLeftEq)) hl = box(h2, h3, nl);
-    if (two) {
+    if (hl && !(eq & kFlatLeftEq)) hl = box(h2, h3, nl);
+    if (two && (!ANY || cr != 0)) {
         hr = true;
         if (!(eq & kFlatRightEq)) hr = box(h4, h5, nr);
     }
-    const int cl = __float_as_int(h2.w), cr = __float_as_int(h4.w);
-    const float4 *pl = fl + kFlatHeaderF4, *pr = pl + kPairF4 * ((cl & 0xffff) + (cl >> 16));
+    const float4 *pr = pl + kPairF4 * ((cl & 0xffff) + (cl >> 16));
     Hit bl{INFINITY, 0.f, 0.f, -1}, br{INFINITY, 0.f, 0.f, -1};
     bool fl_found = false, fr_found = false, any_l = false, any_r = false;
     if (hl) any_l = flat_leaf<ANY, MASKED>(pl, cl & 0xffff, cl >> 16, o, d, mint, maxt, bl, fl_found, cand);
diff --git a/optix-renderer_amd/csrc/nh_upload.hip b/optix-renderer_amd/csrc/nh_upload.hip
--- a/optix-renderer_amd/csrc/nh_upload.hip
+++ b/optix-renderer_amd/csrc/nh_upload.hip
@@ -389,6 +389,7 @@
     if (c->h_emit_tris.size() != 9 * ef_tri.size()) c->h_emit_tris.clear();
     c->small_image = c->small_image_ref = nullptr;
     c->flat_image = nullptr;
+    c->flat_any_records = 0;
     c->pair_kinds = false;
     c->V.assign(d->V, d->V + 3 * nv);
     c->F.assign(d->F, d->F + 3 * (size_t)d->n_faces);
@@ -423,6 +424,7 @@
 static int build_small_image(nh_ctx *c, const nh::GpuBvh &g) {
     c->small_image = c->small_image_ref = nullptr;
     c->flat_image = nullptr;
+    c->flat_any_records = 0;
     c->pair_kinds = false;
     for (int &v : c->small_tab) v = 0;
     const size_t scene_bytes = 16 * (size_t)(c->n_node_f4 + c->n_prim_f4) + 8 * (size_t)c->n_leaves;
@@ -524,7 +526,13 @@
             std::memcpy(boxes + 12, boxes, 6 * sizeof(float));
         }
         const nh::PairLayout pl = nh::pair_layout(g.leaves.data(), c->n_leaves, g.prims.data(), n, true);
-        const nh::FlatImage fi = nh::flat_image(boxes, g.leaves.data(), c->n_leaves, g.prims.data(), n, pl, nh::flat_trace_knob());
+        uint64_t any_word = ~(uint64_t)0;
+        if (nh::any_list_knob() && n <= 64 && !c->h_emit_tris.empty())
+            any_word = nh::shadow_any_word(c->camera, g.prims.data(), n, c->h_emit_tris.data(), (int)(c->h_emit_tris.size() / 9));
+        const nh::FlatImage fi = nh::flat_image(boxes, g.leaves.data(), c->n_leaves, g.prims.data(), n, pl, nh::flat_trace_knob(),
+                                                any_word);
+        if (fi.flat && fi.any_list)
+            for (int k = 0; k < n; ++k) c->flat_any_records += (int)((any_word >> k) & 1);
         if (fi.flat) {
             const nh::f4 *dev = nullptr;
             if (int rc = upload(c, c->bvh_bufs, fi.data.data(), fi.data.size(), &dev)) return rc;
diff --git a/optix-renderer_amd/host/gpu_layout.cpp b/optix-renderer_amd/host/gpu_layout.cpp
--- a/optix-renderer_amd/host/gpu_layout.cpp
+++ b/optix-renderer_amd/host/gpu_layout.cpp
@@ -550,7 +550,7 @@
 }
 
 FlatImage flat_image(const float boxes[18], const i2 *leaves, int n_leaves, const f4 *prims, int n_records,
-                     const PairLayout &pl, bool allowed) {
+                     const PairLayout &pl, bool allowed, uint64_t any_word) {
     FlatImage out;
     if (!allowed || n_leaves < 1 || n_leaves > 2 || n_records < 1 || (int)pl.leaves.size() != n_leaves) return out;
     int n_pairs = 0;
@@ -567,30 +567,58 @@
         return f;
     };
     const float *root = boxes, *lb = n_leaves == 2 ? boxes + 6 : boxes, *rb = n_leaves == 2 ? boxes + 12 : boxes;
+    const uint64_t in_use = n_records < 64 ? ~(~(uint64_t)0 << n_records) : ~(uint64_t)0;
+    const bool any_list = n_records <= 64 && (any_word & in_use) != in_use;
+    std::vector<int2> any_slots[2];
+    int any_counts[2] = {0, 0};
+    if (any_list)
+        for (int l = 0; l < n_leaves; ++l) {
+            std::vector<int> kind[2];
+            for (int k = leaves[l].x; k < leaves[l].x + leaves[l].y; ++k) {
+                if (k < 0 || k >= n_records) return out;
+                if (!((any_word >> k) & 1)) continue;
+                int bits;
+                std::memcpy(&bits, &prims[3 * (size_t)k + 2].w, 4);
+                kind[bits & nhd::kPrimSphere ? 1 : 0].push_back(k);
+            }
+            for (const std::vector<int> &v : kind)
+                for (size_t i = 0; i < v.size(); i += 2)
+                    any_slots[l].push_back(make_int2(v[i], i + 1 < v.size() ? v[i + 1] : -1));
+            any_counts[l] = ((int)kind[0].size() + 1) / 2 | (((int)kind[1].size() + 1) / 2) << 16;
+        }
+    out.any_list = any_list;
     out.box_equal = n_leaves == 1 ? nhd::kFlatLeftEq
                                   : (same_bits(lb, root) ? nhd::kFlatLeftEq : 0) | (same_bits(rb, root) ? nhd::kFlatRightEq : 0);
-    out.data.reserve((size_t)nhd::kFlatHeaderF4 + (size_t)nhd::kPairF4 * n_pairs);
-    out.data.push_back(make_float4(root[0], root[1], root[2], as_float(out.box_equal)));
+    out.data.reserve((size_t)nhd::kFlatHeaderF4 + (size_t)nhd::kPairF4 * (any_list ? 2 * nhd::kFlatMaxPairs : n_pairs));
+    out.data.push_back(make_float4(root[0], root[1], root[2], as_float(out.box_equal | (any_list ? nhd::kFlatAnyList : 0))));
     out.data.push_back(make_float4(root[3], root[4], root[5], as_float(n_leaves)));
     out.data.push_back(make_float4(lb[0], lb[1], lb[2], as_float(pl.leaves[0].y)));
-    out.data.push_back(make_float4(lb[3], lb[4], lb[5], 0.f));
+    out.data.push_back(make_float4(lb[3], lb[4], lb[5], as_float(any_counts[0])));
     out.data.push_back(make_float4(rb[0], rb[1], rb[2], as_float(n_leaves == 2 ? pl.leaves[1].y : 0)));
-    out.data.push_back(make_float4(rb[3], rb[4], rb[5], 0.f));
+    out.data.push_back(make_float4(rb[3], rb[4], rb[5], as_float(any_counts[1])));
+    const auto pair_record = [&](int2 s) {
+        const int k = s.x, k1 = s.y < 0 ? k : s.y;
+        if (k < 0 || k >= n_records || k1 >= n_records) return false;
+        const float4 a = prims[3 * (size_t)k], b = prims[3 * (size_t)k + 1], c = prims[3 * (size_t)k + 2];
+        const float4 a1 = prims[3 * (size_t)k1], b1 = prims[3 * (size_t)k1 + 1], c1 = prims[3 * (size_t)k1 + 2];
+        out.data.push_back(make_float4(a.x, a1.x, a.y, a1.y));
+        out.data.push_back(make_float4(a.z, a1.z, a.w, a1.w));
+        out.data.push_back(make_float4(b.x - a.x, b1.x - a1.x, b.y - a.y, b1.y - a1.y));
+        out.data.push_back(make_float4(b.z - a.z, b1.z - a1.z, c.x - a.x, c1.x - a1.x));
+        out.data.push_back(make_float4(c.y - a.y, c1.y - a1.y, c.z - a.z, c1.z - a1.z));
+        out.data.push_back(make_float4(c.w, c1.w, as_float(k), as_float(k1)));
+        return true;
+    };
     for (int l = 0; l < n_leaves; ++l) {
         const int2 p = pl.leaves[(size_t)l];
-        for (int i = 0, n = (p.y & 0xffff) + (p.y >> 16); i < n; ++i) {
-            const int2 s = pl.slots[(size_t)(p.x + i)];
-            const int k = s.x, k1 = s.y < 0 ? k : s.y;
-            if (k < 0 || k >= n_records || k1 >= n_records) return FlatImage{};
-            const float4 a = prims[3 * (size_t)k], b = prims[3 * (size_t)k + 1], c = prims[3 * (size_t)k + 2];
-            const float4 a1 = prims[3 * (size_t)k1], b1 = prims[3 * (size_t)k1 + 1], c1 = prims[3 * (size_t)k1 + 2];
-            out.data.push_back(make_float4(a.x, a1.x, a.y, a1.y));
-            out.data.push_back(make_float4(a.z, a1.z, a.w, a1.w));
-            out.data.push_back(make_float4(b.x - a.x, b1.x - a1.x, b.y - a.y, b1.y - a1.y));
-            out.data.push_back(make_float4(b.z - a.z, b1.z - a1.z, c.x - a.x, c1.x - a1.x));
-            out.data.push_back(make_float4(c.y - a.y, c1.y - a1.y, c.z - a.z, c1.z - a1.z));
-            out.data.push_back(make_float4(c.w, c1.w, as_float(k), as_float(k1)));
-        }
+        for (int i = 0, n = (p.y & 0xffff) + (p.y >> 16); i < n; ++i)
+            if (!pair_record(pl.slots[(size_t)(p.x + i)])) return FlatImage{};
+    }
+    if (any_list) {
+        out.data.resize((size_t)nhd::kFlatHeaderF4 + (size_t)nhd::kPairF4 * nhd::kFlatMaxPairs, make_float4(0.f, 0.f, 0.f, 0.f));
+        for (int l = 0; l < n_leaves; ++l)
+            for (const int2 &s : any_slots[l])
+                if (!pair_record(s)) return FlatImage{};
     }
     out.flat = true;
     return out;
@@ -600,8 +628,9 @@
 
 extern "C" {
 
-int nh_flat_image(const float *records, int32_t n_records, const int32_t *leaves, int32_t n_leaves, const float *boxes,
-                  int32_t allowed, float *image, int32_t image_cap_f4, int32_t *n_f4, int32_t *box_equal) {
+int nh_flat_image_any(const float *records, int32_t n_records, const int32_t *leaves, int32_t n_leaves,
+                      const float *boxes, int32_t allowed, uint64_t any_word, float *image, int32_t image_cap_f4,
+                      int32_t *n_f4, int32_t *box_equal) {
     bool ok = n_records >= 0 && n_leaves >= 0 && (n_records == 0 || records) && (n_leaves == 0 || leaves) && boxes &&
               n_f4 && box_equal && image_cap_f4 >= 0 && (image_cap_f4 == 0 || image);
     std::vector<char> used((size_t)std::max(n_records, 0), 0);
@@ -620,7 +649,8 @@
     const nh::i2 *lv = reinterpret_cast<const nh::i2 *>(leaves);
     const nh::f4 *rec = reinterpret_cast<const nh::f4 *>(records);
     const nh::PairLayout pl = nh::pair_layout(lv, n_leaves, rec, n_records, true);
-    const nh::FlatImage fi = nh::flat_image(boxes, lv, n_leaves, rec, n_records, pl, allowed != 0 && nh::flat_trace_knob());
+    const nh::FlatImage fi = nh::flat_image(boxes, lv, n_leaves, rec, n_records, pl, allowed != 0 && nh::flat_trace_knob(),
+                                            nh::any_list_knob() ? any_word : ~(uint64_t)0);
     *n_f4 = fi.flat ? (int32_t)fi.data.size() : 0;
     *box_equal = fi.box_equal;
     if (fi.flat) {
@@ -631,6 +661,12 @@
         std::memcpy(image, fi.data.data(), fi.data.size() * sizeof(nh::f4));
     }
     return NH_OK;
+}
+
+int nh_flat_image(const float *records, int32_t n_records, const int32_t *leaves, int32_t n_leaves, const float *boxes,
+                  int32_t allowed, float *image, int32_t image_cap_f4, int32_t *n_f4, int32_t *box_equal) {
+    return nh_flat_image_any(records, n_records, leaves, n_leaves, boxes, allowed, ~(uint64_t)0, image, image_cap_f4, n_f4,
+                             box_equal);
 }
 
 int nh_pair_layout(const float *records, int32_t n_records, const int32_t *leaves, int32_t n_leaves, int32_t by_kind,
diff --git a/optix-renderer_amd/host/gpu_layout.h b/optix-renderer_amd/host/gpu_layout.h
--- a/optix-renderer_amd/host/gpu_layout.h
+++ b/optix-renderer_amd/host/gpu_layout.h
@@ -55,6 +55,8 @@
 bool primary_mask_in_front(const nh_camera &cam, const f4 *prims, int n_records, std::vector<char> &in_front);
 
 uint64_t shadow_emitter_mask(const f4 *prims, int n_records, const float *emit_faces, int n_faces);
+uint64_t shadow_any_word(const nh_camera &cam, const f4 *prims, int n_records, const float *emit_faces, int n_faces);
+bool any_list_knob();
 std::vector<float> shadow_emitter_faces(const nh_scene_desc &d);
 bool shadow_block_masks(const nh_camera &cam, const f4 *prims, int n_records, const float *emit_faces, int n_faces,
                         const int32_t *blocks, int n_blocks, std::vector<uint64_t> &masks);
@@ -66,11 +68,12 @@
 
 struct FlatImage {
     bool flat = false;
+    bool any_list = false;
     int box_equal = 0;
     std::vector<f4> data;
 };
 FlatImage flat_image(const float boxes[18], const i2 *leaves, int n_leaves, const f4 *prims, int n_records,
-                     const PairLayout &pl, bool allowed);
+                     const PairLayout &pl, bool allowed, uint64_t any_word = ~(uint64_t)0);
 bool flat_trace_knob();
 
 }
diff --git a/optix-renderer_amd/host/shadow_masks.cpp b/optix-renderer_amd/host/shadow_masks.cpp
--- a/optix-renderer_amd/host/shadow_masks.cpp
+++ b/optix-renderer_amd/host/shadow_masks.cpp
@@ -1,5 +1,6 @@
 #include <algorithm>
 #include <cmath>
+#include <cstdlib>
 #include <cstring>
 
 #include "gpu_layout.h"
@@ -48,6 +49,9 @@
     double sin_t;
     double len;
     double rho;
+    double s;
+    int side;
+    double reach;
     double grown;
     AABB box;
 };
@@ -64,9 +68,55 @@
     AABB scene, emit;
     double eps_o = 0, eta = 0, d_e = 0, m = 0;
     uint64_t emitter_word = ~(uint64_t)0;
+    uint64_t any_word = ~(uint64_t)0;
 };
 
-Analysis analyse(const f4 *prims, int n_records, const float *emit_faces, int n_faces) {
+const double kEpsD = 1e-4f;
+
+uint64_t supporting_walls(const Analysis &A, int n_records, const V3 *origin, double origin_radius) {
+    uint64_t keep = ~(uint64_t)0;
+    if (!A.ok) return keep;
+    AABB from = A.scene;
+    if (origin) {
+        from.add(V3{origin->x - origin_radius, origin->y - origin_radius, origin->z - origin_radius});
+        from.add(V3{origin->x + origin_radius, origin->y + origin_radius, origin->z + origin_radius});
+    }
+    if (!std::isfinite(from.lo.x + from.lo.y + from.lo.z + from.hi.x + from.hi.y + from.hi.z)) return keep;
+    double max_abs = 0;
+    for (const V3 &q : {from.lo, from.hi}) max_abs = std::max({max_abs, std::fabs(q.x), std::fabs(q.y), std::fabs(q.z)});
+    const double hit_round = 8.0 * kU * max_abs;
+    std::vector<V3> ends;
+    for (const Record &R : A.rec) {
+        if (!R.sphere) {
+            ends.insert(ends.end(), R.p, R.p + 3);
+            continue;
+        }
+        double far_d = 0;
+        for (int i = 0; i < 8; ++i) {
+            const V3 q{i & 1 ? from.hi.x : from.lo.x, i & 2 ? from.hi.y : from.lo.y, i & 4 ? from.hi.z : from.lo.z};
+            far_d = std::max(far_d, norm(q - R.p[0]) + R.r);
+        }
+        if (!(R.r > 0.0)) return keep;
+        const double g_hit = R.r + 64.0 * kU * far_d * far_d / R.r + hit_round;
+        for (int i = 0; i < 8; ++i)
+            ends.push_back(V3{R.p[0].x + (i & 1 ? g_hit : -g_hit), R.p[0].y + (i & 2 ? g_hit : -g_hit),
+                              R.p[0].z + (i & 4 ? g_hit : -g_hit)});
+    }
+    for (int k = 0; k < n_records; ++k) {
+        const Record &R = A.rec[(size_t)k];
+        if (R.sphere || !std::isfinite(R.rho)) continue;
+        double depth = 0;
+        for (const V3 &q : ends) depth = std::max(depth, -R.side * dot(R.n, q - R.p[0]));
+        const double eps_f = depth + hit_round;
+        const double rho_t = 8.0 * kU * A.d_e * (R.reach + 2.0 * A.d_e) / (R.s * R.sin_t);
+        if (!(R.s > 2.0 * rho_t) || !(kEpsD > 2.0 * (A.d_e * eps_f / R.s + rho_t + 4.0 * kU * A.d_e))) continue;
+        keep &= ~((uint64_t)1 << k);
+    }
+    return keep;
+}
+
+Analysis analyse(const f4 *prims, int n_records, const float *emit_faces, int n_faces, const V3 *origin = nullptr,
+                 double origin_radius = 0.0) {
     Analysis A;
     if (n_records <= 0 || n_records > 64 || n_faces <= 0 || !emit_faces) return A;
     double min_sin = 1.0, max_abs = 0.0;
@@ -150,6 +200,9 @@
         s -= A.eps_o;
         if (!one_side || !(s > 0.0) || !(32.0 * kU * reach <= s * R.sin_t)) continue;
         R.rho = 64.0 * kU * (reach + R.len + A.d_e) * A.d_e / (s * R.sin_t);
+        R.s = s;
+        R.side = side;
+        R.reach = reach;
     }
     A.ok = true;
     uint64_t word = n_records < 64 ? ~(uint64_t)0 << n_records : 0;
@@ -172,6 +225,20 @@
         if (!behind) word |= (uint64_t)1 << k;
     }
     A.emitter_word = word;
+    A.any_word = word & supporting_walls(A, n_records, origin, origin_radius);
+    for (int k = 0; k < n_records; ++k) {
+        const Record &R = A.rec[(size_t)k];
+        if (R.sphere || !((A.any_word >> k) & 1)) continue;
+        bool own = false;
+        for (const Face &F : A.faces) {
+            int hit = 0;
+            for (int i = 0; i < 3; ++i)
+                for (int j = 0; j < 3; ++j)
+                    hit += R.p[i].x == F.p[j].x && R.p[i].y == F.p[j].y && R.p[i].z == F.p[j].z;
+            own = own || hit >= 3;
+        }
+        if (!own) A.any_word = ~(uint64_t)0;
+    }
     return A;
 }
 
@@ -213,6 +280,19 @@
 
 uint64_t shadow_emitter_mask(const f4 *prims, int n_records, const float *emit_faces, int n_faces) {
     return analyse(prims, n_records, emit_faces, n_faces).emitter_word;
+}
+
+uint64_t shadow_any_word(const nh_camera &cam, const f4 *prims, int n_records, const float *emit_faces, int n_faces) {
+    const float *cw = cam.camera_to_world;
+    const V3 org{(double)cw[3] / cw[15], (double)cw[7] / cw[15], (double)cw[11] / cw[15]};
+    const double lens = std::fabs((double)cam.lens_radius);
+    if (!std::isfinite(org.x + org.y + org.z + lens)) return ~(uint64_t)0;
+    return analyse(prims, n_records, emit_faces, n_faces, &org, lens).any_word;
+}
+
+bool any_list_knob() {
+    const char *e = std::getenv("NH_ANY_LIST");
+    return !(e && e[0] == '0');
 }
 
 bool shadow_block_masks(const nh_camera &cam, const f4 *prims, int n_records, const float *emit_faces, int n_faces,
@@ -365,4 +445,14 @@
     return NH_OK;
 }
 
-}
+int nh_shadow_any_word(const nh_camera *camera, const float *records, int32_t n_records, const float *emit_faces,
+                       int32_t n_emit_faces, uint64_t *word) {
+    if (!camera || !word || n_records < 0 || (n_records > 0 && !records) || (n_emit_faces > 0 && !emit_faces)) {
+        nh::set_host_error("nh_shadow_any_word: invalid argument");
+        return NH_ERR_INVALID;
+    }
+    *word = nh::shadow_any_word(*camera, reinterpret_cast<const nh::f4 *>(records), n_records, emit_faces, n_emit_faces);
+    return NH_OK;
+}
+
+}
diff --git a/optix-renderer_amd/nori_hip.py b/optix-renderer_amd/nori_hip.py
--- a/optix-renderer_amd/nori_hip.py
+++ b/optix-renderer_amd/nori_hip.py
@@ -188,7 +188,7 @@
                                   "tail_coop_bounces", "bounce_cycles_load", "bounce_cycles_body",
                                   "bounce_cycles_shadow", "bounce_cycles_closest", "bounce_cycles_head",
                                   "bounce_cycles_store", "bounce_bounces", "bounce_traits", "primary_masks",
-                                  "pair_kinds", "flat_trace", "shadow_masks")]
+                                  "pair_kinds", "flat_trace", "shadow_masks", "any_list")]
 
 
 def _sig(name, res, *args):
@@ -225,6 +225,9 @@
      C.POINTER(C.c_uint64), C.POINTER(_i32))
 _sig("nh_pair_layout", _i32, _fp, _i32, C.POINTER(_i32), _i32, _i32, C.POINTER(_i32), C.POINTER(_i32))
 _sig("nh_flat_image", _i32, _fp, _i32, C.POINTER(_i32), _i32, _fp, _i32, _fp, _i32, C.POINTER(_i32), C.POINTER(_i32))
+_sig("nh_shadow_any_word", _i32, C.POINTER(nh_camera), _fp, _i32, _fp, _i32, C.POINTER(C.c_uint64))
+_sig("nh_flat_image_any", _i32, _fp, _i32, C.POINTER(_i32), _i32, _fp, _i32, C.c_uint64, _fp, _i32, C.POINTER(_i32),
+     C.POINTER(_i32))
 _sig("nh_framebuffer_to_rgb", _i32, _fp, _i32, _i32, _i32, _fp)
 _sig("nh_write_pfm", _i32, C.c_char_p, _fp, _i32, _i32)
 _sig("nh_image_load_png", _i32, C.c_char_p, C.POINTER(C.c_uint8), C.c_size_t, C.POINTER(_i32), C.POINTER(_i32))
@@ -874,15 +877,30 @@
     return slots, lp
 
 
-def flat_image(records: np.ndarray, leaves, boxes, allowed: bool = True):
+def shadow_any_word(camera: nh_camera, records: np.ndarray, emit_faces) -> int:
+    rec = np.ascontiguousarray(records, dtype=np.float32).reshape(-1, 12)
+    ef = np.zeros((0, 9), np.float32) if emit_faces is None else np.ascontiguousarray(emit_faces, np.float32).reshape(-1, 9)
+    word = C.c_uint64(0)
+    _host_check(_lib.nh_shadow_any_word(C.byref(camera), _fptr(rec), len(rec), _fptr(ef), len(ef), C.byref(word)),
+                "shadow_any_word")
+    return int(word.value)
+
+
+def flat_image(records: np.ndarray, leaves, boxes, allowed: bool = True, any_word: int | None = None):
     rec = np.ascontiguousarray(records, dtype=np.float32).reshape(-1, 12)
     lv = np.ascontiguousarray(leaves, dtype=np.int32).reshape(-1, 2)
     bx = np.ascontiguousarray(boxes, dtype=np.float32).ravel()
     assert bx.size == 18
-    cap = 6 + 6 * 16
+    cap = 6 + 6 * 16 * (1 if any_word is None else 2)
     img, n, eq = np.zeros((cap, 4), np.float32), _i32(0), _i32(0)
-    _host_check(_lib.nh_flat_image(_fptr(rec), len(rec), lv.ctypes.data_as(C.POINTER(_i32)), len(lv), _fptr(bx),
-                                   1 if allowed else 0, _fptr(img), cap, C.byref(n), C.byref(eq)), "flat_image")
+    ip = lv.ctypes.data_as(C.POINTER(_i32))
+    if any_word is None:
+        _host_check(_lib.nh_flat_image(_fptr(rec), len(rec), ip, len(lv), _fptr(bx), 1 if allowed else 0, _fptr(img), cap,
+                                       C.byref(n), C.byref(eq)), "flat_image")
+    else:
+        _host_check(_lib.nh_flat_image_any(_fptr(rec), len(rec), ip, len(lv), _fptr(bx), 1 if allowed else 0,
+                                           C.c_uint64(any_word & ((1 << 64) - 1)), _fptr(img), cap, C.byref(n),
+                                           C.byref(eq)), "flat_image_any")
     return (img[:n.value].copy() if n.value else None), int(eq.value)
 
 
```

Result: faster. 9567 Msamples/s (median of 6 runs) (+8.2%).
